# mihikamd/DP-GSAT

Measured on AMD Instinct MI355X. Metric: million edges/s (attn+sample+aggregate fwd+bwd), higher is better.
Workload: dtype f32

## Files before the change

dp_gsat_amd/_lib.py:

```python
from __future__ import annotations

import ctypes
import os
from ctypes import c_char_p, c_double, c_float, c_int, c_int32, c_int64, c_size_t, c_uint64, c_void_p

import torch

_HERE = os.path.dirname(os.path.abspath(__file__))
LIB_PATH = os.path.join(_HERE, "libgsat_hip.so")

P, I64, I32, F32, F64, SZ, INT, U64 = c_void_p, c_int64, c_int32, c_float, c_double, c_size_t, c_int, c_uint64

SIGNATURES = {
    "gsat_abi_version": (INT, []),
    "gsat_seed_next": (INT, [P, P, P]),
    "gsat_last_error": (c_char_p, []),
    "gsat_csr_workspace_bytes": (SZ, [I64, I64]),
    "gsat_rev_workspace_bytes": (SZ, [I64]),
    "gsat_build_csr": (INT, [P, P, I64, I64, P, P, P, P, P, SZ, P]),
    "gsat_reverse_edge_perm": (INT, [P, I64, I64, P, P, P, SZ, P]),
    "gsat_reverse_edge_perm_csr": (INT, [P, P, P, P, P, P, P, P, I64, I64, P, P, P]),
    "gsat_segment_ptr": (INT, [P, I64, I64, P, P, P]),
    "gsat_gather_i64": (INT, [P, I64, P, I64, P, P]),
    "gsat_row_chunks_workspace_bytes": (SZ, [I64]),
    "gsat_row_chunks": (INT, [P, I64, P, P, SZ, P]),
    "gsat_long_row_partial_floats": (SZ, [I64, I64]),
    "gsat_aggr_sum_fwd": (INT, [P, P, P, P, P, P, P, I64, I64, I64, F32, P, P, P, P]),
    "gsat_aggr_sum_bwd": (INT, [P, P, P, P, P, P, P, I64, I64, I64, F32, P, P, P, P, P, P]),
    "gsat_pna_fwd": (INT, [P, P, P, P, P, P, I64, I64, P, INT, P, INT, F32, F32, P, P]),
    "gsat_pna_bwd": (INT, [P, P, P, P, P, P, P, I64, I64, P, INT, P, INT, F32, F32, P, P, P, P, P]),
    "gsat_pna_long_row_floats": (SZ, [I64, I64, INT]),
    "gsat_pna_fwd_long": (INT, [P, P, P, P, P, P, I64, I64, I64, P, INT, P, INT, F32, F32, P, P, P, P]),
    "gsat_pna_bwd_long": (INT, [P, P, P, P, P, P, P, I64, I64, I64, P, INT, P, INT, F32, F32, P, P, P, P, P, P, P]),
    "gsat_pna_tile_plan": (INT, [I64, I64, P, P, P]),
    "gsat_pna_build_tiles": (INT, [P, P, P, P, P, I64, INT, INT, INT, P, P, P, P]),
    "gsat_pna_bwd_tiled": (INT, [P, P, P, P, P, P, P, I64, INT, INT, INT, P, P, I64, I64, I64, P, INT, P, INT, P, P, P, P, P, P, P]),
    "gsat_pna_fwd_compact": (INT, [P, P, P, P, P, I64, I64, P, INT, P, P, P]),
    "gsat_pna_post_fwd": (INT, [P, P, P, I64, I64, INT, P, I64, P, I64, P, P]),
    "gsat_pna_post_dw_workspace_floats": (SZ, [I64, I64, INT, I64]),
    "gsat_pna_post_dw": (INT, [P, P, P, I64, I64, INT, P, I64, P, P, SZ, P]),
    "gsat_pna_fwd_node_att": (INT, [P, P, P, P, I64, I64, P, INT, P, INT, F32, F32, P, P]),
    "gsat_pna_bwd_tiled_node_att": (INT, [P, P, P, P, P, P, I64, INT, INT, INT, P, P, I64, I64, I64, P, INT, P, INT, P, P, P, P, P, P, P, INT, P]),
    "gsat_csr_pair_workspace_bytes": (SZ, [I64, I64]),
    "gsat_build_csr_pair": (INT, [P, I64, I64] + [P] * 12 + [P, SZ, P]),
    "gsat_segment_ptr32": (INT, [P, I64, I64, P, P, P, P]),
    "gsat_bn_workspace_floats": (SZ, [I64, I64]),
    "gsat_bn_fwd": (INT, [P, P, P, P, P, I64, I64, INT, F32, F32, INT, P, P, P, P, P]),
    "gsat_bn_bwd": (INT, [P, P, P, P, P, P, I64, I64, INT, INT, P, P, P, P, P]),
    "gsat_bn_act_fwd": (INT, [P, P, P, P, P, I64, I64, INT, F32, F32, INT, P, F32, U64, P, P, P, P, P, P]),
    "gsat_bn_act_bwd": (INT, [P, P, P, P, P, P, I64, I64, INT, INT, F32, U64, P, P, P, P, P, P, P]),
    "gsat_bn_act_fwd_valid": (INT, [P, P, P, P, P, I64, I64, INT, F32, F32, INT, P, F32, U64, P, P, P, P, P, P, P]),
    "gsat_bn_act_bwd_valid": (INT, [P, P, P, P, P, P, I64, I64, INT, INT, F32, U64, P, P, P, P, P, P, P, P]),
    "gsat_bn_local_sum": (INT, [P, P, I64, I64, P, P, P]),
    "gsat_bn_apply_fwd": (INT, [P, P, P, P, P, I64, I64, INT, P, F32, U64, P, P, P]),
    "gsat_bn_local_bwd_sums": (INT, [P, P, P, P, P, P, I64, I64, INT, F32, U64, P, P, P, P, P]),
    "gsat_bn_apply_bwd": (INT, [P, P, P, P, P, P, P, P, I64, P, I64, I64, INT, F32, U64, P, P, P, P]),
    "gsat_relu_dropout_fwd": (INT, [P, I64, I64, F32, U64, P, P, P]),
    "gsat_relu_dropout_bwd": (INT, [P, P, I64, I64, F32, P, P]),
    "gsat_colsum_workspace_floats": (SZ, [I64]),
    "gsat_colsum": (INT, [P, I64, I64, P, P, P]),
    "gsat_embsum_fwd": (INT, [P, P, INT, P, I64, I64, P, P]),
    "gsat_onehot_rows": (INT, [P, P, INT, I64, I64, P, P]),
    "gsat_gemm_workspace_floats": (SZ, [INT, I64, I64, I64]),
    "gsat_gemm_plan": (INT, [INT, INT, INT, I64, I64, I64, INT, INT, I64, P]),
    "gsat_gemm_f32": (INT, [INT, INT, I64, I64, I64, P, I64, P, I64, P, I64, P, INT, P, SZ, P]),
    "gsat_gemm_bf16x3": (INT, [INT, INT, I64, I64, I64, P, I64, P, I64, P, I64, P, INT, P, SZ, P]),
    "gsat_attn_fwd_workspace_bytes": (SZ, [P]),
    "gsat_attn_fwd_kind": (I32, [P]),
    "gsat_attn_bwd_workspace_bytes": (SZ, [P]),
    "gsat_attn_fwd": (INT, [P, P]),
    "gsat_attn_bwd": (INT, [P, P, P]),
    "gsat_instance_norm_fwd": (INT, [P, P, P, P, I64, I64, I64, P, P, P]),
    "gsat_instance_norm_bwd": (INT, [P, P, P, P, P, P, I64, I64, I64, P, P, P]),
    "gsat_philox_keep_mask": (INT, [U64, I32, I64, I64, F32, P, P]),
    "gsat_philox_noise": (INT, [U64, I64, P, P]),
    "gsat_sample_fwd": (INT, [P, P, INT, F32, F32, I64, P, P]),
    "gsat_sample_bwd": (INT, [P, P, F32, I64, P, P]),
    "gsat_lift_fwd": (INT, [P, P, P, I64, P, P]),
    "gsat_lift_bwd": (INT, [P, P, P, P, P, P, P, P, I64, P, P]),
    "gsat_symmetrise": (INT, [P, P, P, I64, P, P]),
    "gsat_info_loss_fwd": (INT, [P, P, F32, I64, P, P, P]),
    "gsat_info_loss_bwd": (INT, [P, P, F32, P, I64, P, P]),
    "gsat_info_loss_valid_fwd": (INT, [P, P, F32, P, I64, P, P, P, P]),
    "gsat_info_loss_valid_bwd": (INT, [P, P, F32, P, P, I64, P, P, P]),
    "gsat_f1_sparsity_fwd": (INT, [P, P, I64, P, P, P, P, P]),
    "gsat_f1_sparsity_bwd": (INT, [P, P, P, P, I64, P, P, P]),
    "gsat_f1_sparsity_block_entries": (I64, []),
    "gsat_f1_sparsity_max_blocks": (I64, []),
    "gsat_collate_padded": (INT, [P, I64, P, P, P, I64, P, P, I64, I64, P, P, P, P, P, P]),
    "gsat_collate": (INT, [P, I64, P, P, P, I64, P, P, I64, I64, P, P, P, P, P]),
    "gsat_line_graph_pair_counts": (INT, [P, I64, P, P]),
    "gsat_line_graph": (INT, [P, P, P, I64, I64, P, P]),
    "gsat_narrow_i64": (INT, [P, I64, P, P]),
    "gsat_und_edges_workspace_bytes": (SZ, [I64]),
    "gsat_und_edges": (INT, [P, I64, I64, P, P, P, P, P, P, P, P, SZ, P]),
    "gsat_und_line_graph_counts": (INT, [P, P, P, P, I64, P, P]),
    "gsat_und_line_graph": (INT, [P, P, P, P, P, I64, I64, P, P]),
    "gsat_segment_pool_fwd": (INT, [P, P, I64, I64, INT, P, P]),
    "gsat_segment_pool_bwd": (INT, [P, P, I64, I64, INT, P, P]),
    "gsat_rank_edges_lds_cap": (I64, []),
    "gsat_rank_edges_workspace_bytes": (SZ, [I64]),
    "gsat_rank_edges": (INT, [P, P, P, P, I64, I64, I64, I64, INT, P, P, P, P, P, SZ, P]),
    "gsat_auroc_workspace_bytes": (SZ, [I64]),
    "gsat_auroc": (INT, [P, P, I64, P, P, SZ, P]),
    "gsat_delta_kl_workspace_bytes": (SZ, [I64]),
    "gsat_delta_kl": (INT, [P, P, I64, F64, P, P, SZ, P]),
    "gsat_auroc_tasks_workspace_bytes": (SZ, [I64, I64]),
    "gsat_auroc_tasks": (INT, [P, P, I64, I64, P, P, SZ, P]),
    "gsat_att_histogram": (INT, [P, P, I64, I64, F64, F64, P, P, P]),
    "gsat_subgraph_block_items": (I64, []),
    "gsat_subgraph_workspace_bytes": (SZ, [I64, I64]),
    "gsat_subgraph_index": (INT, [P, I64, I64, P, P, I64, P, INT, INT, INT, I64, I64, INT, P, P, P, P, P, P, P, P, SZ, P]),
    "gsat_gather_rows": (INT, [P, P, I64, I64, P, P]),
    "gsat_eval_log_append": (INT, [P] * 8 + [I64] * 4 + [P] * 8 + [I64] * 3 + [P]),
    "gsat_delta_kl_segments_chunk": (I64, []),
    "gsat_delta_kl_segments_workspace_bytes": (SZ, [I64, I64]),
    "gsat_delta_kl_segments": (INT, [P, P, P, I64, I64, I64, F64, P, P, SZ, P]),
}



class AttnArgs(ctypes.Structure):
    _fields_ = [("M", I64), ("N", I64), ("G", I64), ("H", I32), ("C1", I32), ("C2", I32), ("edge_mode", I32),
                ("training", I32), ("p_drop", F32), ("seed", U64),
                ("src", P), ("dst", P), ("seg_ptr", P), ("seg_order", P), ("row_seg", P),
                ("W1", P), ("b1", P), ("W2", P), ("b2", P), ("W3", P), ("b3", P),
                ("emb", P), ("mask1", P), ("mask2", P), ("u", P),
                ("P", P), ("Q", P), ("a1", P), ("h2", P), ("stats", P), ("logits", P), ("att", P),
                ("fwd_workspace", P), ("fwd_workspace_bytes", SZ), ("seed_dev", P), ("noise_philox", I32), ("fused", I32),
                ("node_ptr", P)]


class AttnGrads(ctypes.Structure):
    _fields_ = [("dlogits", P), ("datt", P), ("rowptr_src", P), ("eid_by_src", P), ("rowptr_dst", P), ("eid_by_dst", P),
                ("chunk_ptr_src", P), ("chunk_ptr_dst", P),
                ("demb", P), ("dW1", P), ("db1", P), ("dW2", P), ("db2", P), ("dW3", P), ("db3", P),
                ("workspace", P), ("workspace_bytes", SZ)]


_lib = None


class GsatHipError(RuntimeError):
    pass


def load():
    global _lib
    if _lib is not None:
        return _lib
    if not os.path.exists(LIB_PATH):
        raise GsatHipError(
            f"{LIB_PATH} not found: the HIP extension is required (no CPU fallback). "
            "Build it with `python -c 'import __graft_entry__ as g; g.build()'` or `make -C dp_gsat_amd/csrc`.")
    lib = ctypes.CDLL(LIB_PATH)
    for name, (res, args) in SIGNATURES.items():
        fn = getattr(lib, name)
        fn.restype = res
        fn.argtypes = args
    _lib = lib
    return lib


def ptr(t):
    if t is None:
        return None
    if not t.is_cuda:
        raise GsatHipError("dp_gsat_amd operators need ROCm (cuda) tensors: the HIP path has no CPU fallback")
    if not t.is_contiguous():
        raise GsatHipError("dp_gsat_amd operators need contiguous tensors")
    return t.data_ptr()


_raw_stream = getattr(torch._C, "_cuda_getCurrentRawStream", None)


def stream():
    if _raw_stream is not None:
        return _raw_stream(torch.cuda.current_device())
    return torch.cuda.current_stream().cuda_stream


def call(name, *args):
    lib = _lib if _lib is not None else load()
    rc = getattr(lib, name)(*args)
    if rc != 0:
        msg = lib.gsat_last_error()
        raise GsatHipError(f"{name} failed (code {rc}): {msg.decode() if msg else ''}")
    return rc
```

dp_gsat_amd/csrc/attn.hip:

```cpp
#include "common.h"
#include "attn_fused.h"
#include <cstdlib>

namespace gsat {

constexpr float IN_EPS = 1e-5f;
constexpr int SB = 256;
#ifndef GSAT_SB_LANES
#define GSAT_SB_LANES 16
#endif
constexpr int SB_LANES = GSAT_SB_LANES;
constexpr int SB_SLOTS = SB / SB_LANES;
constexpr int SB_RC = 2;

struct GemmWs { float* ptr; size_t floats; };
static int gemm_rm(hipStream_t stream, bool ta, bool tb, int64_t M, int64_t N, int64_t K, const float* A, int64_t lda, const float* B,
                   int64_t ldb, float beta, float* C, int64_t ldc, GemmWs ws = {nullptr, 0}, bool split_ok = false, SlabJob* defer = nullptr) {
    const char* env = getenv("GSAT_ATTN_BWD_SPLIT");
    const bool bwd_split = !(env && atoi(env) == 0);
    return gemm_f32(stream, ta, tb, M, N, K, A, lda, B, ldb, C, ldc, nullptr, beta != 0.f, ws.ptr, ws.floats, split_ok && bwd_split, defer);
}

template <bool EDGE>
struct PreAct {
    const float* P; const float* Q; const float* bias; const int32_t* src; const int32_t* dst; int C;
    __device__ __forceinline__ float4 load(int row, int c) const {
        float4 b = bias ? ld4(bias + c) : f4zero();
        float4 v;
        if (EDGE) {
            float4 p = ld4(P + (size_t)src[row] * C + c);
            float4 q = ld4(Q + (size_t)dst[row] * C + c);
            v = make_float4(p.x + q.x, p.y + q.y, p.z + q.z, p.w + q.w);
        } else {
            v = ld4(P + (size_t)row * C + c);
        }
        return make_float4(v.x + b.x, v.y + b.y, v.z + b.z, v.w + b.w);
    }
};

__device__ __forceinline__ float4 keep4(const float* mask, SeedRef sref, int layer, int row, int c, int C, float p, bool training) {
    if (!training || p <= 0.f) return make_float4(1.f, 1.f, 1.f, 1.f);
    if (mask) return ld4(mask + (size_t)row * C + c);
    return philox_keep4(sref.get(), layer, row, c, p);
}

__device__ __forceinline__ float4 slot_reduce(float4 v, float4 (*sm)[SB_LANES], int slot, int lane) {
    __syncthreads();
    sm[slot][lane] = v;
    __syncthreads();
    float4 r = f4zero();
    if (slot == 0) {
#pragma unroll
        for (int s = 0; s < SB_SLOTS; ++s) {
            float4 t = sm[s][lane];
            r.x += t.x; r.y += t.y; r.z += t.z; r.w += t.w;
        }
    }
    return r;
}

__device__ __forceinline__ void seg_slice(const int32_t* __restrict__ seg_ptr, int g, int* beg, int* end, float* inv_n) {
    const int b = seg_ptr[g], e = seg_ptr[g + 1];
    *inv_n = 1.f / (float)max(e - b, 1);
    const int Z = gridDim.z, z = blockIdx.z;
    if (Z > 1) {
        const int per = (e - b + Z - 1) / Z;
        *beg = min(e, b + z * per);
        *end = min(e, *beg + per);
    } else {
        *beg = b; *end = e;
    }
}

template <bool EDGE>
__global__ __launch_bounds__(SB) void k_seg_partial(PreAct<EDGE> pre, const int32_t* __restrict__ seg_ptr, const int32_t* __restrict__ order,
                                                    const float* __restrict__ mean , float* __restrict__ part) {
    __shared__ float4 sm[SB_SLOTS][SB_LANES];
    const int g = blockIdx.x;
    const int lane = threadIdx.x % SB_LANES, slot = threadIdx.x / SB_LANES;
    const int c = (blockIdx.y * SB_LANES + lane) * 4;
    const int C = pre.C;
    const bool on = c < C;
    int beg, end; float inv_n;
    seg_slice(seg_ptr, g, &beg, &end, &inv_n);
    float4 acc = f4zero();
    if (on) {
        const float4 mu = mean ? ld4(mean + (size_t)g * C + c) : f4zero();
        for (int r = beg + slot; r < end; r += SB_SLOTS) {
            float4 h = pre.load(order ? order[r] : r, c);
            if (mean) {
                float dx = h.x - mu.x, dy = h.y - mu.y, dz = h.z - mu.z, dw = h.w - mu.w;
                acc.x = fmaf(dx, dx, acc.x); acc.y = fmaf(dy, dy, acc.y); acc.z = fmaf(dz, dz, acc.z); acc.w = fmaf(dw, dw, acc.w);
            } else {
                acc.x += h.x; acc.y += h.y; acc.z += h.z; acc.w += h.w;
            }
        }
    }
    float4 tot = slot_reduce(acc, sm, slot, lane);
    if (slot == 0 && on) st4(part + ((size_t)g * gridDim.z + blockIdx.z) * C + c, tot);
}

__global__ void k_zcombine(const float* __restrict__ part, const int32_t* __restrict__ seg_ptr, int G, int Z, int C, int mode,
                           float* __restrict__ out) {
    const int64_t i = (int64_t)blockIdx.x * blockDim.x + threadIdx.x;
    if (i >= (int64_t)G * C) return;
    const int g = (int)(i / C), c = (int)(i % C);
    float acc = 0.f;
    for (int z = 0; z < Z; ++z) acc += part[((size_t)g * Z + z) * C + c];
    const float inv_n = 1.f / (float)max(seg_ptr[g + 1] - seg_ptr[g], 1);
    out[i] = mode == 0 ? acc : mode == 1 ? acc * inv_n : 1.f / sqrtf(acc * inv_n + IN_EPS);
}

template <bool EDGE, bool APPLY>
__global__ __launch_bounds__(SB) void k_seg_stats(PreAct<EDGE> pre, const int32_t* __restrict__ seg_ptr,
                                                  const int32_t* __restrict__ order, float* __restrict__ mean_out,
                                                  float* __restrict__ rstd_out, const float* __restrict__ mask = nullptr,
                                                  SeedRef seed = SeedRef{0, nullptr}, int layer = 0, float p = 0.f, int training = 0,
                                                  float* __restrict__ act_out = nullptr) {
    __shared__ float4 sm[SB_SLOTS][SB_LANES];
    __shared__ float4 bc[SB_LANES];
    const int g = blockIdx.x;
    const int lane = threadIdx.x % SB_LANES, slot = threadIdx.x / SB_LANES;
    const int c = (blockIdx.y * SB_LANES + lane) * 4;
    const int C = pre.C;
    const bool on = c < C;
    const int beg = seg_ptr[g], end = seg_ptr[g + 1];
    const float inv_n = 1.f / (float)max(end - beg, 1);
    float4 hc[SB_RC];
    int mc[SB_RC];
#pragma unroll
    for (int i = 0; i < SB_RC; ++i) {
        const int r = beg + slot + i * SB_SLOTS;
        mc[i] = (r < end) ? (order ? order[r] : r) : -1;
    }
#pragma unroll
    for (int i = 0; i < SB_RC; ++i) hc[i] = (on && mc[i] >= 0) ? pre.load(mc[i], c) : f4zero();
    const int rest = beg + slot + SB_RC * SB_SLOTS;
    float4 acc = f4zero();
    if (on) {
#pragma unroll
        for (int i = 0; i < SB_RC; ++i)
            if (mc[i] >= 0) { acc.x += hc[i].x; acc.y += hc[i].y; acc.z += hc[i].z; acc.w += hc[i].w; }
        for (int r = rest; r < end; r += SB_SLOTS) {
            float4 h = pre.load(order ? order[r] : r, c);
            acc.x += h.x; acc.y += h.y; acc.z += h.z; acc.w += h.w;
        }
    }
    float4 tot = slot_reduce(acc, sm, slot, lane);
    if (slot == 0) bc[lane] = make_float4(tot.x * inv_n, tot.y * inv_n, tot.z * inv_n, tot.w * inv_n);
    __syncthreads();
    const float4 mu = bc[lane];
    acc = f4zero();
    if (on) {
#pragma unroll
        for (int i = 0; i < SB_RC; ++i)
            if (mc[i] >= 0) {
                float dx = hc[i].x - mu.x, dy = hc[i].y - mu.y, dz = hc[i].z - mu.z, dw = hc[i].w - mu.w;
                acc.x = fmaf(dx, dx, acc.x); acc.y = fmaf(dy, dy, acc.y); acc.z = fmaf(dz, dz, acc.z); acc.w = fmaf(dw, dw, acc.w);
            }
        for (int r = rest; r < end; r += SB_SLOTS) {
            float4 h = pre.load(order ? order[r] : r, c);
            float dx = h.x - mu.x, dy = h.y - mu.y, dz = h.z - mu.z, dw = h.w - mu.w;
            acc.x = fmaf(dx, dx, acc.x); acc.y = fmaf(dy, dy, acc.y); acc.z = fmaf(dz, dz, acc.z); acc.w = fmaf(dw, dw, acc.w);
        }
    }
    tot = slot_reduce(acc, sm, slot, lane);
    float4 rs = make_float4(1.f / sqrtf(tot.x * inv_n + IN_EPS), 1.f / sqrtf(tot.y * inv_n + IN_EPS),
                            1.f / sqrtf(tot.z * inv_n + IN_EPS), 1.f / sqrtf(tot.w * inv_n + IN_EPS));
    if (slot == 0 && on) {
        st4(mean_out + (size_t)g * C + c, mu);
        st4(rstd_out + (size_t)g * C + c, rs);
    }
    if (APPLY) {
        if (slot == 0) bc[lane] = rs;
        __syncthreads();
        rs = bc[lane];
        const float sc = (training && p > 0.f) ? 1.f / (1.f - p) : 1.f;
        if (on) {
#pragma unroll
            for (int i = 0; i < SB_RC; ++i)
                if (mc[i] >= 0) {
                    const int m = mc[i];
                    const float4 h = hc[i];
                    const float4 k = keep4(mask, seed, layer, m, c, C, p, training != 0);
                    st4(act_out + (size_t)m * C + c,
                        make_float4(fmaxf((h.x - mu.x) * rs.x, 0.f) * k.x * sc, fmaxf((h.y - mu.y) * rs.y, 0.f) * k.y * sc,
                                    fmaxf((h.z - mu.z) * rs.z, 0.f) * k.z * sc, fmaxf((h.w - mu.w) * rs.w, 0.f) * k.w * sc));
                }
            for (int r = rest; r < end; r += SB_SLOTS) {
                const int m = order ? order[r] : r;
                const float4 h = pre.load(m, c);
                const float4 k = keep4(mask, seed, layer, m, c, C, p, training != 0);
                st4(act_out + (size_t)m * C + c,
                    make_float4(fmaxf((h.x - mu.x) * rs.x, 0.f) * k.x * sc, fmaxf((h.y - mu.y) * rs.y, 0.f) * k.y * sc,
                                fmaxf((h.z - mu.z) * rs.z, 0.f) * k.z * sc, fmaxf((h.w - mu.w) * rs.w, 0.f) * k.w * sc));
            }
        }
    }
}

template <bool EDGE, bool RELU>
__global__ void k_norm_apply(PreAct<EDGE> pre, const int32_t* __restrict__ row_seg, const float* __restrict__ mean,
                             const float* __restrict__ rstd, const float* __restrict__ mask, SeedRef seed, int layer,
                             float p, int training, int64_t M, float* __restrict__ out) {
    const int C = pre.C, C4 = C >> 2;
    const float sc = (training && p > 0.f) ? 1.f / (1.f - p) : 1.f;
    for (int64_t i = (int64_t)blockIdx.x * blockDim.x + threadIdx.x; i < M * C4; i += (int64_t)gridDim.x * blockDim.x) {
        const int m = (int)(i / C4), c = (int)(i % C4) * 4;
        const int g = row_seg[m];
        float4 h = pre.load(m, c);
        float4 mu = ld4(mean + (size_t)g * C + c), rs = ld4(rstd + (size_t)g * C + c);
        float4 y = make_float4((h.x - mu.x) * rs.x, (h.y - mu.y) * rs.y, (h.z - mu.z) * rs.z, (h.w - mu.w) * rs.w);
        if (RELU) {
            float4 k = keep4(mask, seed, layer, m, c, C, p, training != 0);
            y = make_float4(fmaxf(y.x, 0.f) * k.x * sc, fmaxf(y.y, 0.f) * k.y * sc, fmaxf(y.z, 0.f) * k.z * sc, fmaxf(y.w, 0.f) * k.w * sc);
        }
        st4(out + (size_t)m * C + c, y);
    }
}

template <int LPR>
__global__ __launch_bounds__(256) void k_head_fwd(const float* __restrict__ h2, const float* __restrict__ b2,
                                                  const int32_t* __restrict__ row_seg, const float* __restrict__ mean,
                                                  const float* __restrict__ rstd, const float* __restrict__ mask, SeedRef seed,
                                                  float p, int training, const float* __restrict__ w3, const float* __restrict__ b3,
                                                  const float* __restrict__ u, int noise_philox, int64_t M, int C, float* __restrict__ logits,
                                                  float* __restrict__ att) {
    const int lane = threadIdx.x % LPR;
    const float sc = (training && p > 0.f) ? 1.f / (1.f - p) : 1.f;
    PreAct<false> pre{h2, nullptr, b2, nullptr, nullptr, C};
    for (int64_t m = ((int64_t)blockIdx.x * blockDim.x + threadIdx.x) / LPR; m < M; m += (int64_t)gridDim.x * blockDim.x / LPR) {
        const int g = row_seg[m];
        float acc = 0.f;
        for (int c = lane * 4; c < C; c += LPR * 4) {
            float4 h = pre.load((int)m, c);
            float4 mu = ld4(mean + (size_t)g * C + c), rs = ld4(rstd + (size_t)g * C + c);
            float4 k = keep4(mask, seed, 2, (int)m, c, C, p, training != 0);
            float4 w = ld4(w3 + c);
            acc = fmaf(fmaxf((h.x - mu.x) * rs.x, 0.f) * k.x * sc, w.x, acc);
            acc = fmaf(fmaxf((h.y - mu.y) * rs.y, 0.f) * k.y * sc, w.y, acc);
            acc = fmaf(fmaxf((h.z - mu.z) * rs.z, 0.f) * k.z * sc, w.z, acc);
            acc = fmaf(fmaxf((h.w - mu.w) * rs.w, 0.f) * k.w * sc, w.w, acc);
        }
        acc = group_sum<LPR>(acc);
        if (lane == 0) {
            const float z = acc + b3[0];
            logits[m] = z;
            if (att) {
                float t = z;
                if (training && (u || noise_philox)) {
                    const float uu = u ? u[m] : philox_noise_u(seed.get(), (int)m);
                    t = z + (logf(uu) - logf(1.0f - uu));
                }
                att[m] = 1.f / (1.f + expf(-t));
            }
        }
    }
}

__global__ __launch_bounds__(256) void k_dz(const float* __restrict__ dlogits, const float* __restrict__ datt, const float* __restrict__ att,
                                            int64_t M, float* __restrict__ dz, float* __restrict__ zero_a, int na, float* __restrict__ zero_b, int nb,
                                            float* __restrict__ block_sum = nullptr ) {
    int64_t m = (int64_t)blockIdx.x * blockDim.x + threadIdx.x;
    const int64_t total = (int64_t)gridDim.x * blockDim.x;
    for (int64_t i = m; i < na; i += total) zero_a[i] = 0.f;
    for (int64_t i = m; i < nb; i += total) zero_b[i] = 0.f;
    float v = 0.f;
    if (m < M) {
        v = dlogits ? dlogits[m] : 0.f;
        if (datt) { float a = att[m]; v = fmaf(datt[m], a * (1.f - a), v); }
        dz[m] = v;
    }
    if (block_sum) {
        __shared__ float ws[4];
        const float w = group_sum<64>(v);
        if ((threadIdx.x & 63) == 0) ws[threadIdx.x >> 6] = w;
        __syncthreads();
        if (threadIdx.x == 0) block_sum[blockIdx.x] = ((ws[0] + ws[1]) + ws[2]) + ws[3];
    }
}

struct DzSrc {
    const float* dz;
    const float *dlogits, *datt, *att;
    __device__ __forceinline__ float get(int m) const {
        if (dz) return dz[m];
        float v = dlogits ? dlogits[m] : 0.f;
        if (datt) { const float a = att[m]; v = fmaf(datt[m], a * (1.f - a), v); }
        return v;
    }
};

template <bool APPLY>
__global__ __launch_bounds__(SB) void k_head_bwd_stats(const float* __restrict__ h2, const float* __restrict__ b2,
                                                       const int32_t* __restrict__ seg_ptr, const int32_t* __restrict__ order,
                                                       const float* __restrict__ mean, const float* __restrict__ rstd,
                                                       const float* __restrict__ mask, SeedRef seed, float p, int training,
                                                       const float* __restrict__ w3, const DzSrc dzs, int C,
                                                       float* __restrict__ S1, float* __restrict__ S2, float* __restrict__ dw3p,
                                                       float* __restrict__ dh2 = nullptr) {
    __shared__ float4 sm[SB_SLOTS][SB_LANES];
    __shared__ float4 bc1[SB_LANES], bc2[SB_LANES];
    const int g = blockIdx.x;
    const int lane = threadIdx.x % SB_LANES, slot = threadIdx.x / SB_LANES;
    const int c = (blockIdx.y * SB_LANES + lane) * 4;
    const bool on = c < C;
    int beg, end; float inv_n;
    seg_slice(seg_ptr, g, &beg, &end, &inv_n);
    if (gridDim.z > 1) inv_n = 1.f;
    const size_t orow = gridDim.z > 1 ? (size_t)g * gridDim.z + blockIdx.z : (size_t)g;
    const float sc = (training && p > 0.f) ? 1.f / (1.f - p) : 1.f;
    PreAct<false> pre{h2, nullptr, b2, nullptr, nullptr, C};
    float4 a1 = f4zero(), a2 = f4zero(), a3 = f4zero();
    if (on) {
        const float4 mu = ld4(mean + (size_t)g * C + c), rs = ld4(rstd + (size_t)g * C + c), w = ld4(w3 + c);
        for (int r = beg + slot; r < end; r += SB_SLOTS) {
            const int m = order ? order[r] : r;
            const float d = dzs.get(m);
            float4 h = pre.load(m, c);
            float4 k = keep4(mask, seed, 2, m, c, C, p, training != 0);
            float4 y = make_float4((h.x - mu.x) * rs.x, (h.y - mu.y) * rs.y, (h.z - mu.z) * rs.z, (h.w - mu.w) * rs.w);
            float4 dy = make_float4(y.x > 0.f ? d * w.x * k.x * sc : 0.f, y.y > 0.f ? d * w.y * k.y * sc : 0.f,
                                    y.z > 0.f ? d * w.z * k.z * sc : 0.f, y.w > 0.f ? d * w.w * k.w * sc : 0.f);
            a1.x += dy.x; a1.y += dy.y; a1.z += dy.z; a1.w += dy.w;
            a2.x = fmaf(dy.x, y.x, a2.x); a2.y = fmaf(dy.y, y.y, a2.y); a2.z = fmaf(dy.z, y.z, a2.z); a2.w = fmaf(dy.w, y.w, a2.w);
            a3.x = fmaf(d, fmaxf(y.x, 0.f) * k.x * sc, a3.x); a3.y = fmaf(d, fmaxf(y.y, 0.f) * k.y * sc, a3.y);
            a3.z = fmaf(d, fmaxf(y.z, 0.f) * k.z * sc, a3.z); a3.w = fmaf(d, fmaxf(y.w, 0.f) * k.w * sc, a3.w);
        }
    }
    float4 t1 = slot_reduce(a1, sm, slot, lane);
    float4 t2 = slot_reduce(a2, sm, slot, lane);
    float4 t3 = slot_reduce(a3, sm, slot, lane);
    t1 = make_float4(t1.x * inv_n, t1.y * inv_n, t1.z * inv_n, t1.w * inv_n);
    t2 = make_float4(t2.x * inv_n, t2.y * inv_n, t2.z * inv_n, t2.w * inv_n);
    if (slot == 0 && on) {
        st4(S1 + orow * C + c, t1);
        st4(S2 + orow * C + c, t2);
        st4(dw3p + orow * C + c, t3);
    }
    if (APPLY) {
        if (slot == 0) { bc1[lane] = t1; bc2[lane] = t2; }
        __syncthreads();
        if (!on) return;
        const float4 s1 = bc1[lane], s2 = bc2[lane];
        const float4 mu = ld4(mean + (size_t)g * C + c), rs = ld4(rstd + (size_t)g * C + c), w = ld4(w3 + c);
        for (int r = beg + slot; r < end; r += SB_SLOTS) {
            const int m = order ? order[r] : r;
            const float d = dzs.get(m);
            const float4 h = pre.load(m, c);
            const float4 k = keep4(mask, seed, 2, m, c, C, p, training != 0);
            const float4 y = make_float4((h.x - mu.x) * rs.x, (h.y - mu.y) * rs.y, (h.z - mu.z) * rs.z, (h.w - mu.w) * rs.w);
            const float4 dy = make_float4(y.x > 0.f ? d * w.x * k.x * sc : 0.f, y.y > 0.f ? d * w.y * k.y * sc : 0.f,
                                          y.z > 0.f ? d * w.z * k.z * sc : 0.f, y.w > 0.f ? d * w.w * k.w * sc : 0.f);
            st4(dh2 + (size_t)m * C + c, make_float4(rs.x * (dy.x - s1.x - y.x * s2.x), rs.y * (dy.y - s1.y - y.y * s2.y),
                                                      rs.z * (dy.z - s1.z - y.z * s2.z), rs.w * (dy.w - s1.w - y.w * s2.w)));
        }
    }
}

__global__ void k_dh2(const float* __restrict__ h2, const float* __restrict__ b2, const int32_t* __restrict__ row_seg,
                      const float* __restrict__ mean, const float* __restrict__ rstd, const float* __restrict__ mask, SeedRef seed,
                      float p, int training, const float* __restrict__ w3, const float* __restrict__ dz,
                      const float* __restrict__ S1, const float* __restrict__ S2, int64_t M, int C, float* __restrict__ dh2) {
    const int C4 = C >> 2;
    const float sc = (training && p > 0.f) ? 1.f / (1.f - p) : 1.f;
    PreAct<false> pre{h2, nullptr, b2, nullptr, nullptr, C};
    for (int64_t i = (int64_t)blockIdx.x * blockDim.x + threadIdx.x; i < M * C4; i += (int64_t)gridDim.x * blockDim.x) {
        const int m = (int)(i / C4), c = (int)(i % C4) * 4;
        const int g = row_seg[m];
        const float d = dz[m];
        float4 h = pre.load(m, c);
        float4 mu = ld4(mean + (size_t)g * C + c), rs = ld4(rstd + (size_t)g * C + c), w = ld4(w3 + c);
        float4 k = keep4(mask, seed, 2, m, c, C, p, training != 0);
        float4 s1 = ld4(S1 + (size_t)g * C + c), s2 = ld4(S2 + (size_t)g * C + c);
        float4 y = make_float4((h.x - mu.x) * rs.x, (h.y - mu.y) * rs.y, (h.z - mu.z) * rs.z, (h.w - mu.w) * rs.w);
        float4 dy = make_float4(y.x > 0.f ? d * w.x * k.x * sc : 0.f, y.y > 0.f ? d * w.y * k.y * sc : 0.f,
                                y.z > 0.f ? d * w.z * k.z * sc : 0.f, y.w > 0.f ? d * w.w * k.w * sc : 0.f);
        st4(dh2 + (size_t)m * C + c, make_float4(rs.x * (dy.x - s1.x - y.x * s2.x), rs.y * (dy.y - s1.y - y.y * s2.y),
                                                  rs.z * (dy.z - s1.z - y.z * s2.z), rs.w * (dy.w - s1.w - y.w * s2.w)));
    }
}

template <bool APPLY, bool EDGE>
__global__ __launch_bounds__(SB) void k_l1_bwd_stats(float* __restrict__ da1, const float* __restrict__ a1,
                                                     const int32_t* __restrict__ seg_ptr, const int32_t* __restrict__ order,
                                                     float sc, int C, float* __restrict__ S1, float* __restrict__ S2,
                                                     PreAct<EDGE> pre = PreAct<EDGE>{}, const float* __restrict__ mean = nullptr,
                                                     const float* __restrict__ rstd = nullptr) {
    __shared__ float4 sm[SB_SLOTS][SB_LANES];
    __shared__ float4 bc1[SB_LANES], bc2[SB_LANES];
    const int g = blockIdx.x;
    const int lane = threadIdx.x % SB_LANES, slot = threadIdx.x / SB_LANES;
    const int c = (blockIdx.y * SB_LANES + lane) * 4;
    const bool on = c < C;
    int beg, end; float inv_n;
    seg_slice(seg_ptr, g, &beg, &end, &inv_n);
    if (gridDim.z > 1) inv_n = 1.f;
    const size_t orow = gridDim.z > 1 ? (size_t)g * gridDim.z + blockIdx.z : (size_t)g;
    const float inv_sc = 1.f / sc;
    float4 s1 = f4zero(), s2 = f4zero();
    float4 dcache[SB_RC], acache[SB_RC], hcache[SB_RC];
    int mc[SB_RC];
#pragma unroll
    for (int i = 0; i < SB_RC; ++i) {
        const int r = beg + slot + i * SB_SLOTS;
        mc[i] = (r < end && on) ? (order ? order[r] : r) : -1;
    }
#pragma unroll
    for (int i = 0; i < SB_RC; ++i) {
        dcache[i] = mc[i] >= 0 ? ld4(da1 + (size_t)mc[i] * C + c) : f4zero();
        acache[i] = mc[i] >= 0 ? ld4(a1 + (size_t)mc[i] * C + c) : f4zero();
        if (APPLY) hcache[i] = mc[i] >= 0 ? pre.load(mc[i], c) : f4zero();
    }
    const int rest = beg + slot + SB_RC * SB_SLOTS;
#define GSAT_L1_DY(D4, A4)                                                                                                         \
    const float4 dy = make_float4((A4).x > 0.f ? (D4).x * sc : 0.f, (A4).y > 0.f ? (D4).y * sc : 0.f,                                \
                                  (A4).z > 0.f ? (D4).z * sc : 0.f, (A4).w > 0.f ? (D4).w * sc : 0.f);
#define GSAT_L1_ACC(D4, A4)                                                                                                        \
    {                                                                                                                              \
        GSAT_L1_DY(D4, A4)                                                                                                         \
        s1.x += dy.x; s1.y += dy.y; s1.z += dy.z; s1.w += dy.w;                                                                    \
        s2.x = fmaf(dy.x, (A4).x * inv_sc, s2.x); s2.y = fmaf(dy.y, (A4).y * inv_sc, s2.y);                                          \
        s2.z = fmaf(dy.z, (A4).z * inv_sc, s2.z); s2.w = fmaf(dy.w, (A4).w * inv_sc, s2.w);                                          \
    }
    if (on) {
#pragma unroll
        for (int i = 0; i < SB_RC; ++i)
            if (mc[i] >= 0) GSAT_L1_ACC(dcache[i], acache[i])
        for (int r = rest; r < end; r += SB_SLOTS) {
            const int m = order ? order[r] : r;
            const float4 d = ld4(da1 + (size_t)m * C + c), a = ld4(a1 + (size_t)m * C + c);
            GSAT_L1_ACC(d, a)
        }
    }
#undef GSAT_L1_ACC
    float4 t1 = slot_reduce(s1, sm, slot, lane);
    float4 t2 = slot_reduce(s2, sm, slot, lane);
    t1 = make_float4(t1.x * inv_n, t1.y * inv_n, t1.z * inv_n, t1.w * inv_n);
    t2 = make_float4(t2.x * inv_n, t2.y * inv_n, t2.z * inv_n, t2.w * inv_n);
    if (slot == 0 && on) {
        st4(S1 + orow * C + c, t1);
        st4(S2 + orow * C + c, t2);
    }
    if (APPLY) {
        if (slot == 0) { bc1[lane] = t1; bc2[lane] = t2; }
        __syncthreads();
        if (!on) return;
        const float4 q1 = bc1[lane], q2 = bc2[lane];
        const float4 mu = ld4(mean + (size_t)g * C + c), rs = ld4(rstd + (size_t)g * C + c);
#define GSAT_L1_OUT(M_, H4, D4, A4)                                                                                                \
        {                                                                                                                          \
            const float4 y = make_float4(((H4).x - mu.x) * rs.x, ((H4).y - mu.y) * rs.y, ((H4).z - mu.z) * rs.z, ((H4).w - mu.w) * rs.w); \
            GSAT_L1_DY(D4, A4)                                                                                                     \
            st4(da1 + (size_t)(M_) * C + c, make_float4(rs.x * (dy.x - q1.x - y.x * q2.x), rs.y * (dy.y - q1.y - y.y * q2.y),        \
                                                         rs.z * (dy.z - q1.z - y.z * q2.z), rs.w * (dy.w - q1.w - y.w * q2.w)));     \
        }
#pragma unroll
        for (int i = 0; i < SB_RC; ++i)
            if (mc[i] >= 0) GSAT_L1_OUT(mc[i], hcache[i], dcache[i], acache[i])
        for (int r = rest; r < end; r += SB_SLOTS) {
            const int m = order ? order[r] : r;
            const float4 h = pre.load(m, c);
            const float4 d = ld4(da1 + (size_t)m * C + c), a = ld4(a1 + (size_t)m * C + c);
            GSAT_L1_OUT(m, h, d, a)
        }
#undef GSAT_L1_OUT
    }
#undef GSAT_L1_DY
}

template <bool EDGE>
__global__ void k_dh1(PreAct<EDGE> pre, const int32_t* __restrict__ row_seg, const float* __restrict__ mean,
                      const float* __restrict__ rstd, const float* __restrict__ a1, float sc, const float* __restrict__ S1,
                      const float* __restrict__ S2, int64_t M, float* __restrict__ da1_inout) {
    const int C = pre.C, C4 = C >> 2;
    for (int64_t i = (int64_t)blockIdx.x * blockDim.x + threadIdx.x; i < M * C4; i += (int64_t)gridDim.x * blockDim.x) {
        const int m = (int)(i / C4), c = (int)(i % C4) * 4;
        const int g = row_seg[m];
        float4 h = pre.load(m, c);
        float4 mu = ld4(mean + (size_t)g * C + c), rs = ld4(rstd + (size_t)g * C + c);
        float4 y = make_float4((h.x - mu.x) * rs.x, (h.y - mu.y) * rs.y, (h.z - mu.z) * rs.z, (h.w - mu.w) * rs.w);
        float4 d = ld4(da1_inout + (size_t)m * C + c), a = ld4(a1 + (size_t)m * C + c);
        float4 dy = make_float4(a.x > 0.f ? d.x * sc : 0.f, a.y > 0.f ? d.y * sc : 0.f, a.z > 0.f ? d.z * sc : 0.f, a.w > 0.f ? d.w * sc : 0.f);
        float4 s1 = ld4(S1 + (size_t)g * C + c), s2 = ld4(S2 + (size_t)g * C + c);
        st4(da1_inout + (size_t)m * C + c, make_float4(rs.x * (dy.x - s1.x - y.x * s2.x), rs.y * (dy.y - s1.y - y.y * s2.y),
                                                        rs.z * (dy.z - s1.z - y.z * s2.z), rs.w * (dy.w - s1.w - y.w * s2.w)));
    }
}

__global__ __launch_bounds__(SB) void k_in_bwd_stats(const float* __restrict__ y, const float* __restrict__ dy,
                                                     const int32_t* __restrict__ seg_ptr, const int32_t* __restrict__ order, int C,
                                                     float* __restrict__ S1, float* __restrict__ S2) {
    __shared__ float4 sm[SB_SLOTS][SB_LANES];
    const int g = blockIdx.x;
    const int lane = threadIdx.x % SB_LANES, slot = threadIdx.x / SB_LANES;
    const int c = (blockIdx.y * SB_LANES + lane) * 4;
    const bool on = c < C;
    int beg, end; float inv_n;
    seg_slice(seg_ptr, g, &beg, &end, &inv_n);
    if (gridDim.z > 1) inv_n = 1.f;
    const size_t orow = gridDim.z > 1 ? (size_t)g * gridDim.z + blockIdx.z : (size_t)g;
    float4 s1 = f4zero(), s2 = f4zero();
    if (on)
        for (int r = beg + slot; r < end; r += SB_SLOTS) {
            const int m = order ? order[r] : r;
            float4 d = ld4(dy + (size_t)m * C + c), v = ld4(y + (size_t)m * C + c);
            s1.x += d.x; s1.y += d.y; s1.z += d.z; s1.w += d.w;
            s2.x = fmaf(d.x, v.x, s2.x); s2.y = fmaf(d.y, v.y, s2.y); s2.z = fmaf(d.z, v.z, s2.z); s2.w = fmaf(d.w, v.w, s2.w);
        }
    float4 t1 = slot_reduce(s1, sm, slot, lane);
    float4 t2 = slot_reduce(s2, sm, slot, lane);
    if (slot == 0 && on) {
        st4(S1 + orow * C + c, make_float4(t1.x * inv_n, t1.y * inv_n, t1.z * inv_n, t1.w * inv_n));
        st4(S2 + orow * C + c, make_float4(t2.x * inv_n, t2.y * inv_n, t2.z * inv_n, t2.w * inv_n));
    }
}

__global__ void k_in_bwd_apply(const float* __restrict__ y, const float* __restrict__ dy, const int32_t* __restrict__ row_seg,
                               const float* __restrict__ rstd, const float* __restrict__ S1, const float* __restrict__ S2,
                               int64_t M, int C, float* __restrict__ dx) {
    const int C4 = C >> 2;
    for (int64_t i = (int64_t)blockIdx.x * blockDim.x + threadIdx.x; i < M * C4; i += (int64_t)gridDim.x * blockDim.x) {
        const int m = (int)(i / C4), c = (int)(i % C4) * 4;
        const int g = row_seg[m];
        float4 v = ld4(y + (size_t)m * C + c), d = ld4(dy + (size_t)m * C + c);
        float4 rs = ld4(rstd + (size_t)g * C + c), s1 = ld4(S1 + (size_t)g * C + c), s2 = ld4(S2 + (size_t)g * C + c);
        st4(dx + (size_t)m * C + c, make_float4(rs.x * (d.x - s1.x - v.x * s2.x), rs.y * (d.y - s1.y - v.y * s2.y),
                                                 rs.z * (d.z - s1.z - v.z * s2.z), rs.w * (d.w - s1.w - v.w * s2.w)));
    }
}

__global__ __launch_bounds__(SB) void k_colsum(const float* __restrict__ x, int64_t R, int C, int64_t rows_per_block,
                                               float* __restrict__ out) {
    __shared__ float4 sm[SB_SLOTS][SB_LANES];
    const int lane = threadIdx.x % SB_LANES, slot = threadIdx.x / SB_LANES;
    const int c = (blockIdx.x * SB_LANES + lane) * 4;
    const int64_t beg = (int64_t)blockIdx.y * rows_per_block, end = min(R, beg + rows_per_block);
    float4 acc = f4zero();
    if (c + 3 < C) {
        for (int64_t r = beg + slot; r < end; r += SB_SLOTS) {
            float4 v = ld4(x + (size_t)r * C + c);
            acc.x += v.x; acc.y += v.y; acc.z += v.z; acc.w += v.w;
        }
    } else if (c < C) {
        for (int64_t r = beg + slot; r < end; r += SB_SLOTS) {
            const float* p = x + (size_t)r * C + c;
            acc.x += p[0];
            if (c + 1 < C) acc.y += p[1];
            if (c + 2 < C) acc.z += p[2];
        }
    }
    float4 t = slot_reduce(acc, sm, slot, lane);
    if (slot == 0 && c < C) {
        float* o = out + (size_t)blockIdx.y * C + c;
        o[0] = t.x;
        if (c + 1 < C) o[1] = t.y;
        if (c + 2 < C) o[2] = t.z;
        if (c + 3 < C) o[3] = t.w;
    }
}

constexpr int FIN_T = 1024, FIN_SLOTS = FIN_T / SB_LANES;
__global__ __launch_bounds__(FIN_T) void k_head_bwd_finish(const float* __restrict__ dw3p, const float* __restrict__ dz_part, int64_t G, int ndz, int C,
                                                           float* __restrict__ dW3, float* __restrict__ db3) {
    __shared__ float4 sm[FIN_SLOTS][SB_LANES];
    const int lane = threadIdx.x % SB_LANES, slot = threadIdx.x / SB_LANES;
    const int ctiles = (C + 4 * SB_LANES - 1) / (4 * SB_LANES);
    float4 acc = f4zero();
    if ((int)blockIdx.x < ctiles) {
        const int c = (blockIdx.x * SB_LANES + lane) * 4;
        if (c < C) {
            int64_t g = slot;
            for (; g + 7 * FIN_SLOTS < G; g += 8 * FIN_SLOTS) {
                float4 v[8];
#pragma unroll
                for (int j = 0; j < 8; ++j) v[j] = ld4(dw3p + (size_t)(g + j * FIN_SLOTS) * C + c);
#pragma unroll
                for (int j = 0; j < 8; ++j) { acc.x += v[j].x; acc.y += v[j].y; acc.z += v[j].z; acc.w += v[j].w; }
            }
            for (; g < G; g += FIN_SLOTS) { const float4 v = ld4(dw3p + (size_t)g * C + c); acc.x += v.x; acc.y += v.y; acc.z += v.z; acc.w += v.w; }
        }
    } else {
        for (int i = threadIdx.x; i < ndz; i += FIN_T) acc.x += dz_part[i];
    }
    sm[slot][lane] = acc;
    __syncthreads();
    if (slot == 0) {
        float4 r = f4zero();
        for (int s_ = 0; s_ < FIN_SLOTS; ++s_) { const float4 t = sm[s_][lane]; r.x += t.x; r.y += t.y; r.z += t.z; r.w += t.w; }
        if ((int)blockIdx.x < ctiles) {
            const int c = (blockIdx.x * SB_LANES + lane) * 4;
            if (c < C) st4(dW3 + c, r);
        } else {
            sm[0][lane] = r;
        }
    }
    if ((int)blockIdx.x >= ctiles) {
        __syncthreads();
        if (threadIdx.x == 0) {
            float r = 0.f;
            for (int l = 0; l < SB_LANES; ++l) r += sm[0][l].x;
            db3[0] = r;
        }
    }
}

__global__ void k_philox_noise(uint64_t seed, int64_t M, float* __restrict__ u) {
    const int64_t m = (int64_t)blockIdx.x * blockDim.x + threadIdx.x;
    if (m < M) u[m] = philox_noise_u(seed, (int)m);
}

__global__ void k_philox_mask(uint64_t seed, int layer, int64_t M, int C, float p, float* __restrict__ keep) {
    const int C4 = C >> 2;
    for (int64_t i = (int64_t)blockIdx.x * blockDim.x + threadIdx.x; i < M * C4; i += (int64_t)gridDim.x * blockDim.x) {
        const int m = (int)(i / C4), c = (int)(i % C4) * 4;
        st4(keep + (size_t)m * C + c, keep4(nullptr, SeedRef{seed, nullptr}, layer, m, c, C, p, true));
    }
}

static inline int ew_blocks(int64_t work_items) {
    int64_t nb = ceil_div(work_items, 256);
    if (nb > 256 * 32) nb = 256 * 32;
    return (int)std::max<int64_t>(nb, 1);
}

static int colsum(hipStream_t stream, const float* x, int64_t R, int C, float* out, float* scratch ) {
    if (C <= 0) return GSAT_OK;
    const int ctiles = (int)ceil_div(C, 4 * SB_LANES);
    if (R <= 0) { GSAT_CHECK_HIP(gsat::zero_async(out, sizeof(float) * C, stream)); return GSAT_OK; }
    int64_t RB = std::min<int64_t>(256, ceil_div(R, 64));
    if (RB <= 1) {
        k_colsum<<<dim3(ctiles, 1), SB, 0, stream>>>(x, R, C, R, out);
    } else {
        int64_t rpb = ceil_div(R, RB);
        RB = ceil_div(R, rpb);
        k_colsum<<<dim3(ctiles, (unsigned)RB), SB, 0, stream>>>(x, R, C, rpb, scratch);
        k_colsum<<<dim3(ctiles, 1), SB, 0, stream>>>(scratch, RB, C, RB, out);
    }
    GSAT_LAUNCH_CHECK();
    return GSAT_OK;
}

static inline int seg_slices(int64_t rows, int64_t G) {
    const int64_t avg = rows / std::max<int64_t>(G, 1);
    return (int)std::max<int64_t>(1, std::min<int64_t>(64, ceil_div(avg, 4096)));
}

template <bool EDGE>
static int launch_seg_stats(hipStream_t stream, PreAct<EDGE> pre, const int32_t* seg_ptr, const int32_t* order, int64_t G, int Z,
                            float* mean, float* rstd, float* part) {
    if (G <= 0) return GSAT_OK;
    const int C = pre.C;
    const dim3 grid((unsigned)G, (unsigned)ceil_div(C, 4 * SB_LANES), (unsigned)Z);
    if (Z == 1) {
        k_seg_stats<EDGE, false><<<grid, SB, 0, stream>>>(pre, seg_ptr, order, mean, rstd);
    } else {
        GSAT_REQUIRE(part, GSAT_ERR_WORKSPACE, "segmented statistics need a workspace for sliced segments");
        const unsigned cb = (unsigned)ceil_div(G * C, 256);
        k_seg_partial<EDGE><<<grid, SB, 0, stream>>>(pre, seg_ptr, order, nullptr, part);
        k_zcombine<<<cb, 256, 0, stream>>>(part, seg_ptr, (int)G, Z, C, 1, mean);
        k_seg_partial<EDGE><<<grid, SB, 0, stream>>>(pre, seg_ptr, order, mean, part);
        k_zcombine<<<cb, 256, 0, stream>>>(part, seg_ptr, (int)G, Z, C, 2, rstd);
    }
    GSAT_LAUNCH_CHECK();
    return GSAT_OK;
}

static size_t attn_gemm_ws_w2(const gsat_attn_args* a) { return align_up(gemm_workspace_floats(a->C2, a->C1, a->M, true), 64); }
static size_t attn_gemm_ws_w1(const gsat_attn_args* a) { return align_up(gemm_workspace_floats(a->C1, a->H, a->N, true), 64); }
static size_t attn_gemm_ws_floats(const gsat_attn_args* a) { return attn_gemm_ws_w2(a) + (a->edge_mode ? 2 : 1) * attn_gemm_ws_w1(a); }

static int check_args(const gsat_attn_args* a, const char* who) {
    GSAT_REQUIRE(a, GSAT_ERR_ARG, "%s: null args", who);
    GSAT_REQUIRE(a->M >= 0 && a->N >= 0 && a->G >= 0 && a->M < (1ll << 31) && a->N < (1ll << 31), GSAT_ERR_ARG, "%s: bad extents", who);
    GSAT_REQUIRE(a->H > 0 && a->C1 > 0 && a->C2 > 0 && a->H % 4 == 0 && a->C1 % 4 == 0 && a->C2 % 4 == 0, GSAT_ERR_UNSUPPORTED,
                 "%s: H, C1, C2 must be positive multiples of 4 (got %d, %d, %d)", who, a->H, a->C1, a->C2);
    GSAT_REQUIRE(a->p_drop >= 0.f && a->p_drop < 1.f, GSAT_ERR_ARG, "%s: dropout p must be in [0,1)", who);
    if (a->M == 0) return GSAT_OK;
    GSAT_REQUIRE(a->emb && a->W1 && a->b1 && a->W2 && a->b2 && a->W3 && a->b3 && a->seg_ptr && a->row_seg, GSAT_ERR_ARG, "%s: null input", who);
    GSAT_REQUIRE(a->P && a->h2 && a->stats && a->logits, GSAT_ERR_ARG, "%s: null output/saved buffer", who);
    if (a->edge_mode) GSAT_REQUIRE(a->src && a->dst && a->Q, GSAT_ERR_ARG, "%s: edge mode needs src, dst, Q", who);
    else GSAT_REQUIRE(a->M == a->N, GSAT_ERR_ARG, "%s: node mode needs M == N", who);
    return GSAT_OK;
}

}

using namespace gsat;

extern "C" {

size_t gsat_colsum_workspace_floats(int64_t C) { return (size_t)256 * (size_t)(C > 0 ? C : 0); }

int gsat_colsum(const float* x, int64_t R, int64_t C, float* out, float* workspace, void* stream) {
    GSAT_REQUIRE(R >= 0 && C >= 0 && C < (1ll << 31), GSAT_ERR_ARG, "gsat_colsum: bad extents");
    if (C == 0) return GSAT_OK;
    GSAT_REQUIRE(out && (x || R == 0) && workspace, GSAT_ERR_ARG, "gsat_colsum: null pointer");
    return colsum((hipStream_t)stream, x, R, (int)C, out, workspace);
}


int gsat_attn_fwd(const gsat_attn_args* a, void* stream_) {
    hipStream_t stream = (hipStream_t)stream_;
    int rc = check_args(a, "gsat_attn_fwd");
    if (rc) return rc;
    if (a->M == 0) return GSAT_OK;
    {
        FusedGeom fg;
        if (attn_fused_eligible(a, &fg)) return attn_fused_fwd(stream, a, fg);
    }
    GSAT_REQUIRE(a->a1, GSAT_ERR_ARG, "gsat_attn_fwd: the staged pipeline needs the a1 buffer");
    const int64_t M = a->M, N = a->N, G = a->G;
    const int H = a->H, C1 = a->C1, C2 = a->C2;
    float* mean1 = a->stats;
    float* rstd1 = mean1 + (size_t)G * C1;
    float* mean2 = rstd1 + (size_t)G * C1;
    float* rstd2 = mean2 + (size_t)G * C2;
    if (a->edge_mode) {
        if ((rc = gemm_rm(stream, false, true, N, C1, H, a->emb, H, a->W1, 2 * H, 0.f, a->P, C1))) return rc;
        if ((rc = gemm_rm(stream, false, true, N, C1, H, a->emb, H, a->W1 + H, 2 * H, 0.f, a->Q, C1))) return rc;
    } else {
        if ((rc = gemm_rm(stream, false, true, N, C1, H, a->emb, H, a->W1, H, 0.f, a->P, C1))) return rc;
    }
    const int Z = seg_slices(M, G);
    float* part = nullptr;
    if (Z > 1) {
        const size_t need = (size_t)G * Z * std::max(C1, C2) * sizeof(float);
        GSAT_REQUIRE(a->fwd_workspace && a->fwd_workspace_bytes >= need, GSAT_ERR_WORKSPACE, "gsat_attn_fwd: workspace %zu < %zu", a->fwd_workspace_bytes, need);
        part = static_cast<float*>(a->fwd_workspace);
    }
    const dim3 sgrid((unsigned)G, (unsigned)ceil_div(C1, 4 * SB_LANES), 1);
    const SeedRef sref{a->seed, a->seed_dev};
    if (a->edge_mode) {
        PreAct<true> pre{a->P, a->Q, a->b1, a->src, a->dst, C1};
        if (Z == 1 && G > 0) {
            k_seg_stats<true, true><<<sgrid, SB, 0, stream>>>(pre, a->seg_ptr, a->seg_order, mean1, rstd1, a->mask1, sref, 1, a->p_drop, a->training, a->a1);
        } else {
            if ((rc = launch_seg_stats<true>(stream, pre, a->seg_ptr, a->seg_order, G, Z, mean1, rstd1, part))) return rc;
            k_norm_apply<true, true><<<ew_blocks(M * (C1 / 4)), 256, 0, stream>>>(pre, a->row_seg, mean1, rstd1, a->mask1, sref, 1, a->p_drop, a->training, M, a->a1);
        }
    } else {
        PreAct<false> pre{a->P, nullptr, a->b1, nullptr, nullptr, C1};
        if (Z == 1 && G > 0) {
            k_seg_stats<false, true><<<sgrid, SB, 0, stream>>>(pre, a->seg_ptr, a->seg_order, mean1, rstd1, a->mask1, sref, 1, a->p_drop, a->training, a->a1);
        } else {
            if ((rc = launch_seg_stats<false>(stream, pre, a->seg_ptr, a->seg_order, G, Z, mean1, rstd1, part))) return rc;
            k_norm_apply<false, true><<<ew_blocks(M * (C1 / 4)), 256, 0, stream>>>(pre, a->row_seg, mean1, rstd1, a->mask1, sref, 1, a->p_drop, a->training, M, a->a1);
        }
    }
    GSAT_LAUNCH_CHECK();
    if ((rc = gemm_rm(stream, false, true, M, C2, C1, a->a1, C1, a->W2, C1, 0.f, a->h2, C2))) return rc;
    {
        PreAct<false> pre{a->h2, nullptr, a->b2, nullptr, nullptr, C2};
        if ((rc = launch_seg_stats<false>(stream, pre, a->seg_ptr, a->seg_order, G, Z, mean2, rstd2, part))) return rc;
    }
    const int q = C2 / 4;
    const int lpr = q <= 4 ? 4 : q <= 8 ? 8 : q <= 16 ? 16 : q <= 32 ? 32 : 64;
    const int nb = (int)std::min<int64_t>(ceil_div(M, 256 / lpr), 256 * 32);
#define HEAD(L) k_head_fwd<L><<<nb, 256, 0, stream>>>(a->h2, a->b2, a->row_seg, mean2, rstd2, a->mask2, SeedRef{a->seed, a->seed_dev}, a->p_drop, a->training, a->W3, a->b3, a->u, a->noise_philox, M, C2, a->logits, a->att)
    switch (lpr) { case 4: HEAD(4); break; case 8: HEAD(8); break; case 16: HEAD(16); break; case 32: HEAD(32); break; default: HEAD(64); break; }
#undef HEAD
    GSAT_LAUNCH_CHECK();
    return GSAT_OK;
}

size_t gsat_attn_fwd_workspace_bytes(const gsat_attn_args* a) {
    if (!a) return 0;
    FusedGeom fg;
    if (attn_fused_eligible(a, &fg)) return fused_ws_bytes(fg, a->G);
    const int Z = seg_slices(a->M, a->G);
    return Z > 1 ? (size_t)a->G * Z * std::max(a->C1, a->C2) * sizeof(float) : 0;
}

int gsat_attn_fwd_kind(const gsat_attn_args* a) {
    if (!a) return 0;
    FusedGeom fg;
    if (!attn_fused_eligible(a, &fg)) return 0;
    return fg.x6 ? 2 : 1;
}

size_t gsat_attn_bwd_workspace_bytes(const gsat_attn_args* a) {
    if (!a) return 0;
    const size_t M = (size_t)a->M, N = (size_t)a->N, G = (size_t)a->G, C1 = a->C1, C2 = a->C2;
    const size_t cmax = C1 > C2 ? C1 : C2;
    size_t b = 0;
    b += align_up((M > G ? M : G) * 4, 256);
    b += align_up(M * C2 * 4, 256);
    b += align_up(M * C1 * 4, 256);
    b += 2 * align_up(G * C1 * 4, 256);
    b += 3 * align_up(G * C2 * 4, 256);
    b += align_up(256 * cmax * 4, 256);
    { const size_t Z = seg_slices(a->M, a->G); if (Z > 1) b += 3 * align_up(G * Z * cmax * 4, 256); }
    if (a->edge_mode) b += 2 * align_up(N * C1 * 4, 256) + align_up(gsat_long_row_partial_floats(a->M, a->C1) * 4, 256);
    b += align_up(attn_gemm_ws_floats(a) * 4, 256);
    if (attn_fused_bwd_eligible(a)) b += align_up(attn_fused_bwd_ws_bytes(a), 256);
    b += align_up(std::max(dual_gemm_ws_bytes(1, a->C2, a->C1, a->C1), dual_gemm_ws_bytes(2, a->C1, a->H, a->H)), 256);
    return b + 1024;
}

int gsat_attn_bwd(const gsat_attn_args* a, const gsat_attn_grads* gr, void* stream_) {
    hipStream_t stream = (hipStream_t)stream_;
    int rc = check_args(a, "gsat_attn_bwd");
    if (rc) return rc;
    GSAT_REQUIRE(gr && gr->demb && gr->dW1 && gr->db1 && gr->dW2 && gr->db2 && gr->dW3 && gr->db3, GSAT_ERR_ARG, "gsat_attn_bwd: null gradient output");
    const int64_t M = a->M, N = a->N, G = a->G;
    const int H = a->H, C1 = a->C1, C2 = a->C2;
    const int C0 = a->edge_mode ? 2 * H : H;
    if (M == 0) {
        GSAT_CHECK_HIP(gsat::zero_async(gr->demb, sizeof(float) * N * H, stream));
        GSAT_CHECK_HIP(gsat::zero_async(gr->dW1, sizeof(float) * C1 * C0, stream));
        GSAT_CHECK_HIP(gsat::zero_async(gr->db1, sizeof(float) * C1, stream));
        GSAT_CHECK_HIP(gsat::zero_async(gr->dW2, sizeof(float) * C2 * C1, stream));
        GSAT_CHECK_HIP(gsat::zero_async(gr->db2, sizeof(float) * C2, stream));
        GSAT_CHECK_HIP(gsat::zero_async(gr->dW3, sizeof(float) * C2, stream));
        GSAT_CHECK_HIP(gsat::zero_async(gr->db3, sizeof(float), stream));
        return GSAT_OK;
    }
    GSAT_REQUIRE(gr->dlogits || gr->datt, GSAT_ERR_ARG, "gsat_attn_bwd: need dlogits and/or datt");
    GSAT_REQUIRE(!gr->datt || a->att, GSAT_ERR_ARG, "gsat_attn_bwd: datt given but att was not saved");
    if (a->edge_mode) GSAT_REQUIRE(gr->rowptr_src && gr->eid_by_src && gr->rowptr_dst && gr->eid_by_dst, GSAT_ERR_ARG, "gsat_attn_bwd: edge mode needs both CSRs");
    Arena ar(gr->workspace, gr->workspace_bytes);
    float* dz = ar.take<float>(std::max<int64_t>(M, G));
    float* dh2 = ar.take<float>((size_t)M * C2);
    float* da1 = ar.take<float>((size_t)M * C1);
    float* S1p = ar.take<float>((size_t)G * C1);
    float* S2p = ar.take<float>((size_t)G * C1);
    float* S1 = ar.take<float>((size_t)G * C2);
    float* S2 = ar.take<float>((size_t)G * C2);
    float* dw3p = ar.take<float>((size_t)G * C2);
    float* scratch = ar.take<float>((size_t)256 * std::max(C1, C2));
    const int Z = seg_slices(M, G);
    float *zp1 = nullptr, *zp2 = nullptr, *zp3 = nullptr;
    if (Z > 1) {
        const size_t n = (size_t)G * Z * std::max(C1, C2);
        zp1 = ar.take<float>(n); zp2 = ar.take<float>(n); zp3 = ar.take<float>(n);
    }
    float *dP = nullptr, *dQ = nullptr;
    float* lpart = nullptr;
    if (a->edge_mode) {
        dP = ar.take<float>((size_t)N * C1);
        dQ = ar.take<float>((size_t)N * C1);
        lpart = ar.take<float>(gsat_long_row_partial_floats(M, C1));
    }
    GemmWs gws{nullptr, attn_gemm_ws_w2(a)}, gws1{nullptr, attn_gemm_ws_w1(a)}, gws1b{nullptr, a->edge_mode ? attn_gemm_ws_w1(a) : 0};
    gws.ptr = ar.take<float>(gws.floats);
    gws1.ptr = ar.take<float>(gws1.floats);
    gws1b.ptr = ar.take<float>(gws1b.floats);
    SlabJob jobs[3] = {};
    const size_t dws_bytes = std::max(dual_gemm_ws_bytes(1, C2, C1, C1), dual_gemm_ws_bytes(2, C1, H, H));
    char* dws = ar.take<char>(dws_bytes);
    const bool fused_bwd = attn_fused_bwd_eligible(a) && seg_slices(M, G) == 1;
    const size_t fws_bytes = fused_bwd ? attn_fused_bwd_ws_bytes(a) : 0;
    char* fws = fused_bwd ? ar.take<char>(fws_bytes) : nullptr;
    GSAT_REQUIRE(ar.ok(), GSAT_ERR_WORKSPACE, "gsat_attn_bwd: workspace %zu < %zu", gr->workspace_bytes, ar.off);
    float* mean1 = a->stats;
    float* rstd1 = mean1 + (size_t)G * C1;
    float* mean2 = rstd1 + (size_t)G * C1;
    float* rstd2 = mean2 + (size_t)G * C2;
    const float sc = (a->training && a->p_drop > 0.f) ? 1.f / (1.f - a->p_drop) : 1.f;

    const dim3 g2((unsigned)G, (unsigned)ceil_div(C2, 4 * SB_LANES), (unsigned)Z), g1((unsigned)G, (unsigned)ceil_div(C1, 4 * SB_LANES), (unsigned)Z);
    if (fused_bwd) {
        if ((rc = attn_fused_bwd(stream, a, gr, da1, fws, fws_bytes))) return rc;
    } else {
    const char* env_m = getenv("GSAT_ATTN_BWD_MERGED");
    const bool merged = Z == 1 && G > 0 && !(env_m && atoi(env_m) == 0);
    const unsigned dzb = (unsigned)ceil_div(M, 256);
    float* dzpart = scratch;
    const bool part_ok = (size_t)dzb <= (size_t)256 * std::max(C1, C2);
    k_dz<<<dzb, 256, 0, stream>>>(gr->dlogits, gr->datt, a->att, M, dz, gr->db1, (int)C1, gr->db2, (int)C2, (merged && part_ok) ? dzpart : nullptr);
    GSAT_LAUNCH_CHECK();
    if (!(merged && part_ok) && (rc = colsum(stream, dz, M, 1, gr->db3, scratch))) return rc;
    if (Z == 1)
        k_head_bwd_stats<true><<<g2, SB, 0, stream>>>(a->h2, a->b2, a->seg_ptr, a->seg_order, mean2, rstd2, a->mask2, SeedRef{a->seed, a->seed_dev}, a->p_drop,
                                                      a->training, a->W3, DzSrc{dz, nullptr, nullptr, nullptr}, C2, S1, S2, dw3p, dh2);
    else
        k_head_bwd_stats<false><<<g2, SB, 0, stream>>>(a->h2, a->b2, a->seg_ptr, a->seg_order, mean2, rstd2, a->mask2, SeedRef{a->seed, a->seed_dev}, a->p_drop,
                                                       a->training, a->W3, DzSrc{dz, nullptr, nullptr, nullptr}, C2, zp1, zp2, zp3);
    if (merged && part_ok)
        k_head_bwd_finish<<<(unsigned)ceil_div(C2, 4 * SB_LANES) + 1, FIN_T, 0, stream>>>(dw3p, dzpart, G, (int)dzb, C2, gr->dW3, gr->db3);
    if (Z > 1) {
        const unsigned cb = (unsigned)ceil_div(G * C2, 256);
        k_zcombine<<<cb, 256, 0, stream>>>(zp1, a->seg_ptr, (int)G, Z, C2, 1, S1);
        k_zcombine<<<cb, 256, 0, stream>>>(zp2, a->seg_ptr, (int)G, Z, C2, 1, S2);
        k_zcombine<<<cb, 256, 0, stream>>>(zp3, a->seg_ptr, (int)G, Z, C2, 0, dw3p);
    }
    GSAT_LAUNCH_CHECK();
    if (!(merged && part_ok) && (rc = colsum(stream, dw3p, G, C2, gr->dW3, scratch))) return rc;
    if (Z > 1) {
        k_dh2<<<ew_blocks(M * (C2 / 4)), 256, 0, stream>>>(a->h2, a->b2, a->row_seg, mean2, rstd2, a->mask2, SeedRef{a->seed, a->seed_dev}, a->p_drop, a->training,
                                                           a->W3, dz, S1, S2, M, C2, dh2);
        GSAT_LAUNCH_CHECK();
    }
    if (dual_gemm_ok(1, M, C2, C1, C1)) {
        if ((rc = dual_gemm(stream, 1, M, C2, C1, C1, dh2, C2, a->a1, C1, a->W2, C1, da1, C1, 0, gr->dW2, C1, dws, dws_bytes))) return rc;
    } else {
        if ((rc = gemm_rm(stream, true, false, C2, C1, M, dh2, C2, a->a1, C1, 0.f, gr->dW2, C1, gws, true, &jobs[0]))) return rc;
        if ((rc = gemm_rm(stream, false, false, M, C1, C2, dh2, C2, a->W2, C1, 0.f, da1, C1, GemmWs{nullptr, 0}, true))) return rc;
    }
    if (Z == 1) {
        if (a->edge_mode) {
            PreAct<true> pre1{a->P, a->Q, a->b1, a->src, a->dst, C1};
            k_l1_bwd_stats<true, true><<<g1, SB, 0, stream>>>(da1, a->a1, a->seg_ptr, a->seg_order, sc, C1, S1p, S2p, pre1, mean1, rstd1);
        } else {
            PreAct<false> pre1{a->P, nullptr, a->b1, nullptr, nullptr, C1};
            k_l1_bwd_stats<true, false><<<g1, SB, 0, stream>>>(da1, a->a1, a->seg_ptr, a->seg_order, sc, C1, S1p, S2p, pre1, mean1, rstd1);
        }
    } else {
        k_l1_bwd_stats<false, false><<<g1, SB, 0, stream>>>(da1, a->a1, a->seg_ptr, a->seg_order, sc, C1, zp1, zp2);
    }
    if (Z > 1) {
        const unsigned cb = (unsigned)ceil_div(G * C1, 256);
        k_zcombine<<<cb, 256, 0, stream>>>(zp1, a->seg_ptr, (int)G, Z, C1, 1, S1p);
        k_zcombine<<<cb, 256, 0, stream>>>(zp2, a->seg_ptr, (int)G, Z, C1, 1, S2p);
    }
    GSAT_LAUNCH_CHECK();
    }
    if (a->edge_mode) {
        if (Z > 1) {
            PreAct<true> pre{a->P, a->Q, a->b1, a->src, a->dst, C1};
            k_dh1<true><<<ew_blocks(M * (C1 / 4)), 256, 0, stream>>>(pre, a->row_seg, mean1, rstd1, a->a1, sc, S1p, S2p, M, da1);
            GSAT_LAUNCH_CHECK();
        }
        if ((rc = aggr_sum_fwd_impl(stream, da1, nullptr, nullptr, nullptr, gr->rowptr_src, gr->eid_by_src, nullptr, N, M, C1, 0.f, dP,
                                    gr->chunk_ptr_src, lpart))) return rc;
        if ((rc = aggr_sum_fwd_impl(stream, da1, nullptr, nullptr, nullptr, gr->rowptr_dst, gr->eid_by_dst, nullptr, N, M, C1, 0.f, dQ,
                                    gr->chunk_ptr_dst, lpart))) return rc;
        if (dual_gemm_ok(2, N, C1, H, H)) {
            if ((rc = dual_gemm(stream, 2, N, C1, H, H, dP, C1, a->emb, H, a->W1, 2 * H, gr->demb, H, 0, gr->dW1, 2 * H, dws, dws_bytes))) return rc;
            if ((rc = dual_gemm(stream, 2, N, C1, H, H, dQ, C1, a->emb, H, a->W1 + H, 2 * H, gr->demb, H, 1, gr->dW1 + H, 2 * H, dws, dws_bytes))) return rc;
        } else {
        if ((rc = gemm_rm(stream, false, false, N, H, C1, dP, C1, a->W1, 2 * H, 0.f, gr->demb, H, GemmWs{nullptr, 0}, true))) return rc;
        if ((rc = gemm_rm(stream, false, false, N, H, C1, dQ, C1, a->W1 + H, 2 * H, 1.f, gr->demb, H, GemmWs{nullptr, 0}, true))) return rc;
        if ((rc = gemm_rm(stream, true, false, C1, H, N, dP, C1, a->emb, H, 0.f, gr->dW1, 2 * H, gws1, true, &jobs[1]))) return rc;
        if ((rc = gemm_rm(stream, true, false, C1, H, N, dQ, C1, a->emb, H, 0.f, gr->dW1 + H, 2 * H, gws1b, true, &jobs[2]))) return rc;
        }
    } else {
        if (Z > 1) {
            PreAct<false> pre{a->P, nullptr, a->b1, nullptr, nullptr, C1};
            k_dh1<false><<<ew_blocks(M * (C1 / 4)), 256, 0, stream>>>(pre, a->row_seg, mean1, rstd1, a->a1, sc, S1p, S2p, M, da1);
            GSAT_LAUNCH_CHECK();
        }
        if (dual_gemm_ok(2, N, C1, H, H)) {
            if ((rc = dual_gemm(stream, 2, N, C1, H, H, da1, C1, a->emb, H, a->W1, H, gr->demb, H, 0, gr->dW1, H, dws, dws_bytes))) return rc;
        } else {
        if ((rc = gemm_rm(stream, false, false, N, H, C1, da1, C1, a->W1, H, 0.f, gr->demb, H, GemmWs{nullptr, 0}, true))) return rc;
        if ((rc = gemm_rm(stream, true, false, C1, H, N, da1, C1, a->emb, H, 0.f, gr->dW1, H, gws1, true, &jobs[1]))) return rc;
        }
    }
    return slab_reduce_jobs(stream, jobs, 3);
}

int gsat_instance_norm_fwd(const float* x, const int32_t* seg_ptr, const int32_t* seg_order, const int32_t* row_seg, int64_t M,
                           int64_t G, int64_t C, float* y, float* stats, void* stream_) {
    hipStream_t stream = (hipStream_t)stream_;
    GSAT_REQUIRE(M >= 0 && G >= 0 && C > 0 && C % 4 == 0 && M < (1ll << 31), GSAT_ERR_UNSUPPORTED, "gsat_instance_norm_fwd: C must be a positive multiple of 4");
    if (M == 0 || G == 0) return GSAT_OK;
    GSAT_REQUIRE(x && seg_ptr && row_seg && y && stats, GSAT_ERR_ARG, "gsat_instance_norm_fwd: null pointer");
    float* mean = stats;
    float* rstd = stats + (size_t)G * C;
    PreAct<false> pre{x, nullptr, nullptr, nullptr, nullptr, (int)C};
    k_seg_stats<false, false><<<dim3((unsigned)G, (unsigned)ceil_div(C, 4 * SB_LANES), 1), SB, 0, stream>>>(pre, seg_ptr, seg_order, mean, rstd);
    k_norm_apply<false, false><<<ew_blocks(M * (C / 4)), 256, 0, stream>>>(pre, row_seg, mean, rstd, nullptr, SeedRef{0, nullptr}, 0, 0.f, 0, M, y);
    GSAT_LAUNCH_CHECK();
    return GSAT_OK;
}

int gsat_instance_norm_bwd(const float* y, const float* dy, const float* stats, const int32_t* seg_ptr, const int32_t* seg_order,
                           const int32_t* row_seg, int64_t M, int64_t G, int64_t C, float* dx, float* workspace, void* stream_) {
    hipStream_t stream = (hipStream_t)stream_;
    GSAT_REQUIRE(M >= 0 && G >= 0 && C > 0 && C % 4 == 0 && M < (1ll << 31), GSAT_ERR_UNSUPPORTED, "gsat_instance_norm_bwd: C must be a positive multiple of 4");
    if (M == 0 || G == 0) return GSAT_OK;
    GSAT_REQUIRE(y && dy && stats && seg_ptr && row_seg && dx && workspace, GSAT_ERR_ARG, "gsat_instance_norm_bwd: null pointer");
    float* S1 = workspace;
    float* S2 = workspace + (size_t)G * C;
    k_in_bwd_stats<<<dim3((unsigned)G, (unsigned)ceil_div(C, 4 * SB_LANES), 1), SB, 0, stream>>>(y, dy, seg_ptr, seg_order, (int)C, S1, S2);
    k_in_bwd_apply<<<ew_blocks(M * (C / 4)), 256, 0, stream>>>(y, dy, row_seg, stats + (size_t)G * C, S1, S2, M, (int)C, dx);
    GSAT_LAUNCH_CHECK();
    return GSAT_OK;
}

int gsat_philox_noise(uint64_t seed, int64_t M, float* u, void* stream_) {
    hipStream_t stream = (hipStream_t)stream_;
    GSAT_REQUIRE(M >= 0 && M < (1ll << 31), GSAT_ERR_ARG, "gsat_philox_noise: bad M");
    if (M == 0) return GSAT_OK;
    GSAT_REQUIRE(u, GSAT_ERR_ARG, "gsat_philox_noise: null pointer");
    k_philox_noise<<<(unsigned)ceil_div(M, 256), 256, 0, stream>>>(seed, M, u);
    GSAT_LAUNCH_CHECK();
    return GSAT_OK;
}

int gsat_philox_keep_mask(uint64_t seed, int32_t layer, int64_t M, int64_t C, float p_drop, float* keep, void* stream_) {
    hipStream_t stream = (hipStream_t)stream_;
    GSAT_REQUIRE(M >= 0 && C > 0 && C % 4 == 0 && M < (1ll << 31), GSAT_ERR_UNSUPPORTED, "gsat_philox_keep_mask: C must be a positive multiple of 4");
    if (M == 0) return GSAT_OK;
    GSAT_REQUIRE(keep, GSAT_ERR_ARG, "gsat_philox_keep_mask: null pointer");
    k_philox_mask<<<ew_blocks(M * (C / 4)), 256, 0, stream>>>(seed, layer, M, (int)C, p_drop, keep);
    GSAT_LAUNCH_CHECK();
    return GSAT_OK;
}

}
```

dp_gsat_amd/csrc/attn_fused.h:

```cpp
#pragma once
#include "common.h"

namespace gsat {

constexpr int F_GT = 16;

struct FusedGeom {
    int H, C1, C2, C2p;
    int CH, NCH;
    int S1, S2;
    int NCB2;
    int NRB, RM, RX;
    int LDX, LDU, LDT, LDH, SW;
    int offU, offT, offS, offMeta;
    int lds_bytes;
    int pqg;
    int x6;
};

struct FTile { int row0, nrows, g0, ng, node0, nnodes, flags, pad; };
size_t attn_plan_bytes(int64_t G);
bool attn_plan_ok(int64_t G);
int attn_plan_launch(hipStream_t stream, const int32_t* seg_ptr, const int32_t* node_ptr, int64_t G, int RM, int RX, FTile* tiles, int* counters);

bool fused_geometry(int H, int C1, int C2, bool edge, FusedGeom* out, bool pqg = false);
size_t fused_ws_bytes(const FusedGeom& g, int64_t G);
bool attn_fused_eligible(const gsat_attn_args* a, FusedGeom* g);
int attn_fused_fwd(hipStream_t stream, const gsat_attn_args* a, const FusedGeom& g);

bool attn_fused_bwd_eligible(const gsat_attn_args* a);
size_t attn_fused_bwd_ws_bytes(const gsat_attn_args* a);
int attn_fused_bwd(hipStream_t stream, const gsat_attn_args* a, const gsat_attn_grads* gr, float* dh1, void* ws, size_t ws_bytes);

bool dual_gemm_ok(int mode, int64_t R, int KA, int KY, int NO);
size_t dual_gemm_ws_bytes(int mode, int KA, int KY, int NO);
int dual_gemm(hipStream_t stream, int mode, int64_t R, int KA, int KY, int NO, const float* A, int lda, const float* Y, int ldy, const float* W,
              int ldw, float* OUT, int ldo, int accumulate, float* DW, int lddw, void* ws, size_t ws_bytes);

#ifdef __HIPCC__
__device__ __forceinline__ float4 keep4f(const float* mask, SeedRef sref, int layer, int row, int c, int C, float p, bool training) {
    if (!training || p <= 0.f) return make_float4(1.f, 1.f, 1.f, 1.f);
    if (mask) return ld4(mask + (size_t)row * C + c);
    return philox_keep4(sref.get(), layer, row, c, p);
}
#endif

}
```

dp_gsat_amd/csrc/attn_fused.hip:

```cpp
#include "common.h"
#include "attn_fused.h"
#include <algorithm>
#include <cstdlib>

namespace gsat {

typedef float f32x16 __attribute__((ext_vector_type(16)));

constexpr int FT = 512;
constexpr int F_RMAX = 128;
constexpr float F_EPS = 1e-5f;


static inline int ceil32(int v) { return (v + 31) / 32 * 32; }

bool fused_geometry(int H, int C1, int C2, bool edge, FusedGeom* out, bool pqg) {
    if (H < 8 || H > 256 || H % 8 || C1 < 4 || C1 % 4 || C2 < 4 || C2 % 4 || C2 > 256 || C1 > 2048) return false;
    for (int nrb = 2; nrb >= 1; --nrb) {
        FusedGeom g{};
        g.H = H; g.C1 = C1; g.C2 = C2; g.C2p = ceil32(C2);
        g.CH = edge ? 64 : 128;
        g.NCH = (C1 + g.CH - 1) / g.CH;
        g.S1 = H / 8; g.S2 = g.CH / 8;
        g.NCB2 = g.C2p / 32;
// ... 197 lines not shown
#pragma unroll
        for (int j = 0; j < 4; ++j) {
            if (s + j < S) {
                b[(j + 3) & 3] = bp[64 * min(s + j + 3, S - 1)];
                const float4 x0 = ld4(a0 + 4 * (s + j));
                float4 x1 = f4zero();
                if (NA > 1) x1 = ld4(a1 + 4 * (s + j));
                const float4 w = b[j];
                acc0 = GSAT_MFMA(x0.x, w.x, acc0);
                if (NA > 1) acc1 = GSAT_MFMA(x1.x, w.x, acc1);
                acc0 = GSAT_MFMA(x0.y, w.y, acc0);
                if (NA > 1) acc1 = GSAT_MFMA(x1.y, w.y, acc1);
                acc0 = GSAT_MFMA(x0.z, w.z, acc0);
                if (NA > 1) acc1 = GSAT_MFMA(x1.z, w.z, acc1);
                acc0 = GSAT_MFMA(x0.w, w.w, acc0);
                if (NA > 1) acc1 = GSAT_MFMA(x1.w, w.w, acc1);
            }
        }
    }
}

typedef __attribute__((ext_vector_type(8))) __bf16 fbf16x8;
typedef __attribute__((ext_vector_type(4))) unsigned fu32x4;
#define GSAT_MFMA_B(a, b, c) __builtin_amdgcn_mfma_f32_32x32x16_bf16((a), (b), (c), 0, 0, 0)

__device__ __forceinline__ void split3(const float4 lo4, const float4 hi4, fbf16x8& p0, fbf16x8& p1, fbf16x8& p2) {
    const float x[8] = {lo4.x, lo4.y, lo4.z, lo4.w, hi4.x, hi4.y, hi4.z, hi4.w};
    fu32x4 a, b, c;
#pragma unroll
    for (int e = 0; e < 4; ++e) {
        const unsigned u0 = __builtin_bit_cast(unsigned, x[2 * e]), u1 = __builtin_bit_cast(unsigned, x[2 * e + 1]);
        const float r0 = x[2 * e] - __builtin_bit_cast(float, u0 & 0xFFFF0000u), r1 = x[2 * e + 1] - __builtin_bit_cast(float, u1 & 0xFFFF0000u);
        const unsigned v0 = __builtin_bit_cast(unsigned, r0), v1 = __builtin_bit_cast(unsigned, r1);
        const float s0 = r0 - __builtin_bit_cast(float, v0 & 0xFFFF0000u), s1 = r1 - __builtin_bit_cast(float, v1 & 0xFFFF0000u);
        a[e] = __builtin_amdgcn_perm(u1, u0, 0x07060302u);
        b[e] = __builtin_amdgcn_perm(v1, v0, 0x07060302u);
        c[e] = __builtin_amdgcn_perm(__builtin_bit_cast(unsigned, s1), __builtin_bit_cast(unsigned, s0), 0x07060302u);
    }
    p0 = __builtin_bit_cast(fbf16x8, a); p1 = __builtin_bit_cast(fbf16x8, b); p2 = __builtin_bit_cast(fbf16x8, c);
}

template <int NA>
__device__ __forceinline__ void mma_run_x6(f32x16& acc0, f32x16& acc1, const float* a0, const float* a1, const uint4* __restrict__ bp, const int S) {
    uint4 b[3][3];
#pragma unroll
    for (int p = 0; p < 3; ++p) { b[0][p] = bp[p * 64]; b[1][p] = bp[(3 * min(1, S - 1) + p) * 64]; }
    for (int s = 0; s < S; s += 3) {
#pragma unroll
        for (int j = 0; j < 3; ++j) {
            if (s + j < S) {
                const int sn = min(s + j + 2, S - 1);
#pragma unroll
                for (int p = 0; p < 3; ++p) b[(j + 2) % 3][p] = bp[(3 * sn + p) * 64];
                const fbf16x8 y0 = __builtin_bit_cast(fbf16x8, b[j][0]), y1 = __builtin_bit_cast(fbf16x8, b[j][1]), y2 = __builtin_bit_cast(fbf16x8, b[j][2]);
                fbf16x8 x0, x1, x2;
                split3(ld4(a0 + 16 * (s + j)), ld4(a0 + 16 * (s + j) + 4), x0, x1, x2);
                acc0 = GSAT_MFMA_B(x2, y0, acc0);
                acc0 = GSAT_MFMA_B(x0, y2, acc0);
                acc0 = GSAT_MFMA_B(x1, y1, acc0);
                acc0 = GSAT_MFMA_B(x1, y0, acc0);
                acc0 = GSAT_MFMA_B(x0, y1, acc0);
                acc0 = GSAT_MFMA_B(x0, y0, acc0);
                if (NA > 1) {
                    split3(ld4(a1 + 16 * (s + j)), ld4(a1 + 16 * (s + j) + 4), x0, x1, x2);
                    acc1 = GSAT_MFMA_B(x2, y0, acc1);
                    acc1 = GSAT_MFMA_B(x0, y2, acc1);
                    acc1 = GSAT_MFMA_B(x1, y1, acc1);
                    acc1 = GSAT_MFMA_B(x1, y0, acc1);
                    acc1 = GSAT_MFMA_B(x0, y1, acc1);
                    acc1 = GSAT_MFMA_B(x0, y0, acc1);
                }
            }
        }
    }
}

__device__ __forceinline__ void acc_zero(f32x16& a) {
#pragma unroll
    for (int r = 0; r < 16; ++r) a[r] = 0.f;
}

__device__ __forceinline__ float4 f4add(float4 a, float4 b) { return make_float4(a.x + b.x, a.y + b.y, a.z + b.z, a.w + b.w); }

__device__ float4 slow_pq4(const float* __restrict__ emb_row, const float* __restrict__ W1, int K1, int koff, int col, int C1, int H) {
    float r[4] = {0.f, 0.f, 0.f, 0.f};
    for (int j = 0; j < 4; ++j) {
        if (col + j >= C1) break;
        const float* w = W1 + (size_t)(col + j) * K1 + koff;
        float acc = 0.f;
        for (int k = 0; k < H; ++k) acc = fmaf(emb_row[k], w[k], acc);
        r[j] = acc;
    }
    return make_float4(r[0], r[1], r[2], r[3]);
}

__device__ __forceinline__ void lds_barrier() { asm volatile("s_waitcnt lgkmcnt(0)\n\ts_barrier" ::: "memory"); }

template <int RC>
__device__ __forceinline__ void column_stats(const float* col, const int LD, float bias, int b, int e, float* mean, float* rstd) {
    const float inv_n = 1.f / (float)max(e - b, 1);
    const float* p = col + b * LD;
    const int lastoff = max(e - 1 - b, 0) * LD;
    float v[RC];
#pragma unroll
    for (int j = 0; j < RC; ++j) v[j] = p[min(j * LD, lastoff)];
#pragma unroll
    for (int j = 0; j < RC; ++j) v[j] = (b + j < e) ? v[j] + bias : 0.f;
    float s0 = 0.f, s1 = 0.f, s2 = 0.f, s3 = 0.f;
#pragma unroll
    for (int j = 0; j < RC; j += 4) { s0 += v[j]; s1 += v[j + 1]; s2 += v[j + 2]; s3 += v[j + 3]; }
    float s;
    const int n = e - b;
    for (int r0 = RC; r0 < n; r0 += 16) {
        float w[16];
#pragma unroll
        for (int j = 0; j < 16; ++j) w[j] = p[min((r0 + j) * LD, lastoff)];
#pragma unroll
        for (int j = 0; j < 16; j += 4) {
            s0 += (r0 + j < n) ? w[j] + bias : 0.f; s1 += (r0 + j + 1 < n) ? w[j + 1] + bias : 0.f;
            s2 += (r0 + j + 2 < n) ? w[j + 2] + bias : 0.f; s3 += (r0 + j + 3 < n) ? w[j + 3] + bias : 0.f;
        }
    }
    s = (s0 + s1) + (s2 + s3);
    const float mu = s * inv_n;
    float q0 = 0.f, q1 = 0.f, q2 = 0.f, q3 = 0.f;
#pragma unroll
    for (int j = 0; j < RC; j += 4) {
        const float d0 = (b + j < e) ? v[j] - mu : 0.f, d1 = (b + j + 1 < e) ? v[j + 1] - mu : 0.f;
        const float d2 = (b + j + 2 < e) ? v[j + 2] - mu : 0.f, d3 = (b + j + 3 < e) ? v[j + 3] - mu : 0.f;
        q0 = fmaf(d0, d0, q0); q1 = fmaf(d1, d1, q1); q2 = fmaf(d2, d2, q2); q3 = fmaf(d3, d3, q3);
    }
    for (int r0 = RC; r0 < n; r0 += 16) {
        float w[16];
#pragma unroll
        for (int j = 0; j < 16; ++j) w[j] = p[min((r0 + j) * LD, lastoff)];
#pragma unroll
        for (int j = 0; j < 16; j += 4) {
            const float d0 = (r0 + j < n) ? (w[j] + bias) - mu : 0.f, d1 = (r0 + j + 1 < n) ? (w[j + 1] + bias) - mu : 0.f;
            const float d2 = (r0 + j + 2 < n) ? (w[j + 2] + bias) - mu : 0.f, d3 = (r0 + j + 3 < n) ? (w[j + 3] + bias) - mu : 0.f;
            q0 = fmaf(d0, d0, q0); q1 = fmaf(d1, d1, q1); q2 = fmaf(d2, d2, q2); q3 = fmaf(d3, d3, q3);
        }
    }
    const float q = (q0 + q1) + (q2 + q3);
    *mean = mu;
    *rstd = 1.f / sqrtf(q * inv_n + F_EPS);
}

struct FusedArgs {
    const float *emb, *W1, *b1, *b2, *w3, *b3;
    const float4 *Wp1, *Wp2;
    const int32_t *src, *dst, *seg_ptr, *order;
    const float *mask1, *mask2, *u;
    float *P, *Q, *a1, *h2, *stats, *logits, *att;
    const FTile* tiles;
    int* counters;
    int64_t M, N, G;
    SeedRef seed;
    float p;
    int training, noise_philox;
    FusedGeom g;
};

template <bool EDGE, int NRB, int NCB2W, bool X6, bool PQG>
__global__ __launch_bounds__(FT, 2) void k_attn_fused_fwd(const FusedArgs A) {
    extern __shared__ __attribute__((aligned(16))) float lds[];
    const FusedGeom& g = A.g;
    constexpr int CH = EDGE ? 64 : 128, LDT = CH + 4, LDU = 2 * CH + 4, S2 = CH / 8;
    const int H = g.H, C1 = g.C1, C2 = g.C2, LDX = g.LDX, LDH = g.LDH, SW = g.SW;
    float* const X = lds;
    float* const U = lds + g.offU;
    float* const T = lds + g.offT;
    float* const H2 = lds;
    float* const sMean = lds + g.offS;
    int* const meta = reinterpret_cast<int*>(lds + g.offMeta);
    int* const sGptr = meta;
    int* const sRowG = meta + 32;
    int* const sRowId = sRowG + F_RMAX;
    int* const sSrcL = sRowId + F_RMAX;
    int* const sDstL = sSrcL + F_RMAX;
    int* const sCtl = sDstL + F_RMAX;
    float* const sB2 = reinterpret_cast<float*>(sCtl + 16);
    float* const sW3 = sB2 + g.C2p;
    float* const sB1 = sW3 + g.C2p;
    const int tid = threadIdx.x, lane = tid & 63, wave = tid >> 6;
    const int cw = wave & 3, rw = wave >> 2, c = lane & 31, h = lane >> 5;
    const int RM = 64 * NRB;
    const int64_t G = A.G;
    float* const mean1 = A.stats;
    float* const rstd1 = mean1 + (size_t)G * C1;
    float* const mean2 = rstd1 + (size_t)G * C1;
    float* const rstd2 = mean2 + (size_t)G * C2;
    const float sc = (A.training && A.p > 0.f) ? 1.f / (1.f - A.p) : 1.f;
    const bool train = A.training != 0;
    const int ntiles = A.counters[0];
    const int K1 = EDGE ? 2 * H : H;
    const int H4 = H >> 2, C24 = C2 >> 2;
    constexpr int CH4 = CH / 4;

    for (int i = tid; i < g.C2p; i += FT) { sB2[i] = i < C2 ? A.b2[i] : 0.f; sW3[i] = i < C2 ? A.w3[i] : 0.f; }
    for (int i = tid; i < g.NCH * g.CH; i += FT) sB1[i] = i < C1 ? A.b1[i] : 0.f;
#ifdef GSAT_FUSED_STAMPS
    long long stamp[14] = {0, 0, 0, 0, 0, 0, 0, 0, 0, 0, 0, 0, 0, 0};
    long long tlast = __builtin_amdgcn_s_memtime();
#define STAMP(i) do { if (tid == 0) { const long long n_ = __builtin_amdgcn_s_memtime(); stamp[i] += n_ - tlast; tlast = n_; } } while (0)
#else
#define STAMP(i)
#endif
    FTile nxt = A.tiles[min((int)blockIdx.x, max(ntiles - 1, 0))];
    for (int t = blockIdx.x; t < ntiles; t += gridDim.x) {
        lds_barrier();
        const FTile tl = nxt;
        nxt = A.tiles[min(t + (int)gridDim.x, ntiles - 1)];
        const bool big = (tl.flags & 1) != 0;
        const int nslab_m = big ? (tl.nrows + RM - 1) / RM : 1;
        if (tid <= tl.ng) sGptr[tid] = A.seg_ptr[tl.g0 + tid] - tl.row0;
        if (tid == 0) sCtl[1] = 0;

        auto load_x = [&](int x0, int nx) {
            const int fill = min((nx + 31) & ~31, EDGE ? g.RX : RM);
            for (int i0 = tid; i0 < fill * H4; i0 += 4 * FT) {
                float4 v[4];
#pragma unroll
                for (int u = 0; u < 4; ++u) {
                    const int i = min(i0 + u * FT, fill * H4 - 1), r = i / H4, q = i - r * H4;
                    v[u] = ld4(A.emb + (size_t)(x0 + min(r, nx - 1)) * H + 4 * q);
                }
#pragma unroll
                for (int u = 0; u < 4; ++u) {
                    const int i = i0 + u * FT, r = i / H4, q = i - r * H4;
                    if (i < fill * H4) st4(X + r * LDX + 4 * q, r < nx ? v[u] : f4zero());
                }
            }
        };
        auto gemm1 = [&](int kc, int nx) {
            f32x16 acc0, acc1;
            acc_zero(acc0); acc_zero(acc1);
            const float4* bp = A.Wp1 + ((size_t)(kc * 4 + cw) * g.S1) * 64 + lane;
            const uint4* bx = reinterpret_cast<const uint4*>(A.Wp1) + ((size_t)(kc * 4 + cw) * (H / 16)) * 192 + lane;
            if (EDGE) {
                const int rb = rw;
                if (rb * 32 < nx) {
                    if (X6) mma_run_x6<1>(acc0, acc1, X + (rb * 32 + c) * LDX + 8 * h, nullptr, bx, H / 16);
                    else mma_run<1>(acc0, acc1, X + (rb * 32 + c) * LDX + h * (H / 2), nullptr, bp, g.S1);
                    float* const o = U + (rb * 32 + 4 * h) * LDU + cw * 32 + c;
#pragma unroll
                    for (int r = 0; r < 16; ++r) o[((r & 3) + 8 * (r >> 2)) * LDU] = acc0[r];
                }
            } else {
                const int rb0 = rw * NRB;
                const int na = min(NRB, (nx - rb0 * 32 + 31) / 32);
                if (na > 0) {
                    if (X6) {
                        const float* a0 = X + (rb0 * 32 + c) * LDX + 8 * h;
                        if (NRB > 1 && na > 1) mma_run_x6<2>(acc0, acc1, a0, a0 + 32 * LDX, bx, H / 16);
                        else mma_run_x6<1>(acc0, acc1, a0, nullptr, bx, H / 16);
                    } else {
                    const float* a0 = X + (rb0 * 32 + c) * LDX + h * (H / 2);
                    if (NRB > 1 && na > 1) mma_run<2>(acc0, acc1, a0, a0 + 32 * LDX, bp, g.S1);
                    else mma_run<1>(acc0, acc1, a0, nullptr, bp, g.S1);
                    }
                    float* const o = T + (rb0 * 32 + 4 * h) * LDT + cw * 32 + c;
#pragma unroll
                    for (int r = 0; r < 16; ++r) o[((r & 3) + 8 * (r >> 2)) * LDT] = acc0[r];
                    if (NRB > 1 && na > 1) {
#pragma unroll
                        for (int r = 0; r < 16; ++r) o[(32 + (r & 3) + 8 * (r >> 2)) * LDT] = acc1[r];
                    }
                }
            }
        };
        auto gemm1_global = [&](int kc, int x0g, int nx) {
            f32x16 acc0, acc1;
            acc_zero(acc0); acc_zero(acc1);
            const float4* bp = A.Wp1 + ((size_t)(kc * 4 + cw) * g.S1) * 64 + lane;
            const uint4* bx = reinterpret_cast<const uint4*>(A.Wp1) + ((size_t)(kc * 4 + cw) * (H / 16)) * 192 + lane;
            const int rbA = rw, rbB = rw + 2;
            const int na = (rbA * 32 < nx ? 1 : 0) + ((NRB > 1 && rbB * 32 < nx) ? 1 : 0);
            if (na <= 0) return;
            if (X6) {
                const float* a0 = X + (rbA * 32 + c) * LDX + 8 * h;
                if (na > 1) mma_run_x6<2>(acc0, acc1, a0, a0 + 64 * LDX, bx, H / 16);
                else mma_run_x6<1>(acc0, acc1, a0, nullptr, bx, H / 16);
            } else {
                const float* a0 = X + (rbA * 32 + c) * LDX + h * (H / 2);
                if (na > 1) mma_run<2>(acc0, acc1, a0, a0 + 64 * LDX, bp, g.S1);
                else mma_run<1>(acc0, acc1, a0, nullptr, bp, g.S1);
            }
            const int col128 = cw * 32 + c, ch = kc * CH + (col128 & (CH - 1));
            if (ch >= C1) return;
            int c1o = C1;
            asm volatile("" : "+s"(c1o));
            float* const pA = (col128 >= CH ? A.Q : A.P) + ch + (size_t)(x0g + rbA * 32 + 4 * h) * C1;
#pragma unroll
            for (int r = 0; r < 16; ++r) {
                const int rr = (r & 3) + 8 * (r >> 2);
                if (rbA * 32 + 4 * h + rr < nx) pA[rr * c1o] = acc0[r];
            }
            if (na > 1) {
                float* const pB = pA + (size_t)64 * C1;
#pragma unroll
                for (int r = 0; r < 16; ++r) {
                    const int rr = (r & 3) + 8 * (r >> 2);
                    if (rbB * 32 + 4 * h + rr < nx) pB[rr * c1o] = acc1[r];
                }
            }
        };
// ... 69 lines not shown
                }, bMean, bRstd, mean1, rstd1);
            } else {
                big_stats(C1, [&](int r, int col) { return A.P[(size_t)(tl.row0 + r) * C1 + col] + A.b1[col]; }, bMean, bRstd, mean1, rstd1);
            }
        }

        for (int sl = 0; sl < nslab_m; ++sl) {
            const int r0 = sl * RM;
            const int nr = big ? min(RM, tl.nrows - r0) : tl.nrows;
            const int nrp = (nr + 31) & ~31;
            lds_barrier();
            if (!big) load_x(EDGE ? tl.node0 : tl.row0, EDGE ? tl.nnodes : tl.nrows);
            for (int r = tid; r < RM; r += FT) {
                if (r < nr) {
                    const int gr = tl.row0 + r0 + r;
                    const int m = EDGE ? (A.order ? A.order[gr] : gr) : gr;
                    sRowId[r] = m;
                    if (EDGE) {
                        const int s = A.src[m], d = A.dst[m];
                        const int sl_ = s - tl.node0, dl_ = d - tl.node0;
                        sSrcL[r] = (!big && (unsigned)sl_ < (unsigned)tl.nnodes) ? sl_ : -(s + 1);
                        sDstL[r] = (!big && (unsigned)dl_ < (unsigned)tl.nnodes) ? dl_ : -(d + 1);
                        if (!big && ((unsigned)sl_ >= (unsigned)tl.nnodes || (unsigned)dl_ >= (unsigned)tl.nnodes)) sCtl[1] = 1;
                    }
                    int gl = 0;
                    if (!big) {
#pragma unroll
                        for (int k = 1; k < F_GT; ++k) gl += (k < tl.ng && sGptr[k] <= r) ? 1 : 0;
                    }
                    sRowG[r] = gl;
                }
            }
            f32x16 acc2[NCB2W][NRB];
#pragma unroll
            for (int j = 0; j < NCB2W; ++j)
#pragma unroll
                for (int i = 0; i < NRB; ++i) acc_zero(acc2[j][i]);
            lds_barrier();
            STAMP(0);
            if (PQG && !big) {
                for (int kc = 0; kc < g.NCH; ++kc) gemm1_global(kc, tl.node0, tl.nnodes);
                __syncthreads();
                STAMP(1);
            }

            for (int kc = 0; kc < g.NCH; ++kc) {
                if (!big && !PQG) {
                    gemm1(kc, EDGE ? tl.nnodes : tl.nrows);
                    lds_barrier();
                    STAMP(1);
                    save_pq(kc, EDGE ? tl.node0 : tl.row0, EDGE ? tl.nnodes : tl.nrows);
                    STAMP(10);
                }
                if (PQG) {
                    constexpr int GB = 2;
                    for (int i0 = tid; i0 < nrp * CH4; i0 += GB * FT) {
                        float4 pv[GB], qv[GB];
#pragma unroll
                        for (int u = 0; u < GB; ++u) {
                            const int i = min(i0 + u * FT, nrp * CH4 - 1), r = min(i / CH4, nr - 1), q = i - (i / CH4) * CH4;
                            const int col = min(kc * CH + 4 * q, C1 - 4);
                            const int sl_ = sSrcL[r], dl_ = sDstL[r];
                            const int sg = sl_ >= 0 ? tl.node0 + sl_ : -sl_ - 1, dg = dl_ >= 0 ? tl.node0 + dl_ : -dl_ - 1;
                            pv[u] = ld4(A.P + (size_t)sg * C1 + col);
                            qv[u] = ld4(A.Q + (size_t)dg * C1 + col);
                        }
#pragma unroll
                        for (int u = 0; u < GB; ++u) {
                            const int i = i0 + u * FT;
                            if (i < nrp * CH4) {
                                const int r = i / CH4, q = i - r * CH4, col = kc * CH + 4 * q;
                                st4(T + r * LDT + 4 * q, (r < nr && col < C1) ? f4add(pv[u], qv[u]) : f4zero());
                            }
                        }
                    }
                    if (!big && sCtl[1] != 0) {
                        for (int i = tid; i < nr * CH4; i += FT) {
                            const int r = i / CH4, q = i - r * CH4, col = kc * CH + 4 * q;
                            const int sl_ = sSrcL[r], dl_ = sDstL[r];
                            if ((sl_ < 0 || dl_ < 0) && col < C1) {
                                const float4 p4 = sl_ >= 0 ? ld4(A.P + (size_t)(tl.node0 + sl_) * C1 + col) : slow_pq4(A.emb + (size_t)(-sl_ - 1) * H, A.W1, K1, 0, col, C1, H);
                                const float4 q4 = dl_ >= 0 ? ld4(A.Q + (size_t)(tl.node0 + dl_) * C1 + col) : slow_pq4(A.emb + (size_t)(-dl_ - 1) * H, A.W1, K1, H, col, C1, H);
                                st4(T + r * LDT + 4 * q, f4add(p4, q4));
                            }
                        }
                    }
                    lds_barrier();
                    STAMP(2);
                } else if (EDGE || big) {
                    for (int i = tid; i < nrp * CH4; i += FT) {
                        const int r = i / CH4, q = i - r * CH4;
                        float4 v = f4zero();
                        const int col = kc * CH + 4 * q;
                        if (r < nr && col < C1) {
                            if (EDGE) {
                                const int s = sSrcL[r], d = sDstL[r];
                                float4 p4, q4;
                                if (big) {
                                    p4 = ld4(A.P + (size_t)(-s - 1) * C1 + col);
                                    q4 = ld4(A.Q + (size_t)(-d - 1) * C1 + col);
                                } else {
                                    p4 = s >= 0 ? ld4(U + s * LDU + 4 * q) : slow_pq4(A.emb + (size_t)(-s - 1) * H, A.W1, K1, 0, col, C1, H);
                                    q4 = d >= 0 ? ld4(U + d * LDU + CH + 4 * q) : slow_pq4(A.emb + (size_t)(-d - 1) * H, A.W1, K1, H, col, C1, H);
                                }
                                v = f4add(p4, q4);
                            } else {
                                v = ld4(A.P + (size_t)sRowId[r] * C1 + col);
                            }
                        }
                        st4(T + r * LDT + 4 * q, v);
                    }
                    lds_barrier();
                    STAMP(2);
                }
                if (!big) {
                    constexpr int nslot = FT / CH;
                    const int cc = tid % CH, slot = tid / CH;
                    const int col = kc * CH + cc;
                    const float bias = sB1[col];
                    for (int gl = slot; gl < tl.ng; gl += nslot) {
                        float mu, rs;
                        column_stats<32>(T + cc, LDT, bias, sGptr[gl], sGptr[gl + 1], &mu, &rs);
                        sMean[gl * SW + cc] = mu;
                        sMean[(F_GT + gl) * SW + cc] = rs;
                        if (col < C1) { mean1[(size_t)(tl.g0 + gl) * C1 + col] = mu; rstd1[(size_t)(tl.g0 + gl) * C1 + col] = rs; }
                    }
                    STAMP(11);
                    lds_barrier();
                    STAMP(3);
                }
                constexpr int AB = (NRB == 2 && NCB2W == 2) ? 2 : 4;
                for (int i0 = tid; i0 < nr * CH4; i0 += AB * FT) {
                    float4 hv[AB], mu[AB], rs[AB], bb[AB];
                    int mm[AB], rr[AB], qq[AB];
#pragma unroll
                    for (int u = 0; u < AB; ++u) {
                        const int i = min(i0 + u * FT, nr * CH4 - 1);
                        rr[u] = i / CH4; qq[u] = i - rr[u] * CH4;
                        hv[u] = ld4(T + rr[u] * LDT + 4 * qq[u]);
                        bb[u] = ld4(sB1 + kc * CH + 4 * qq[u]);
                        mm[u] = sRowId[rr[u]];
                        if (big) { mu[u] = ld4(bMean + min(kc * CH + 4 * qq[u], C1 - 4)); rs[u] = ld4(bRstd + min(kc * CH + 4 * qq[u], C1 - 4)); }
                        else { const int gl = sRowG[rr[u]]; mu[u] = ld4(sMean + gl * SW + 4 * qq[u]); rs[u] = ld4(sMean + (F_GT + gl) * SW + 4 * qq[u]); }
                    }
#pragma unroll
                    for (int u = 0; u < AB; ++u) {
                        const int col = kc * CH + 4 * qq[u];
                        if (i0 + u * FT < nr * CH4 && col < C1) {
                            const float4 x = f4add(hv[u], bb[u]);
                            const float4 k = keep4f(A.mask1, A.seed, 1, mm[u], col, C1, A.p, train);
                            const float4 y = make_float4(fmaxf((x.x - mu[u].x) * rs[u].x, 0.f) * k.x * sc, fmaxf((x.y - mu[u].y) * rs[u].y, 0.f) * k.y * sc,
                                                         fmaxf((x.z - mu[u].z) * rs[u].z, 0.f) * k.z * sc, fmaxf((x.w - mu[u].w) * rs[u].w, 0.f) * k.w * sc);
                            st4(T + rr[u] * LDT + 4 * qq[u], y);
                            if (A.a1) st4(A.a1 + (size_t)mm[u] * C1 + col, y);
                        }
                    }
                }
                lds_barrier();
                STAMP(4);
                {
                    const int rb0 = rw * NRB;
                    const int na = min(NRB, (nr - rb0 * 32 + 31) / 32);
                    if (na > 0) {
                        const float* a0 = T + (rb0 * 32 + c) * LDT + (X6 ? 8 * h : h * (CH / 2));
#pragma unroll
                        for (int j = 0; j < NCB2W; ++j) {
                            const int cb2 = cw + 4 * j;
                            if (cb2 < g.NCB2) {
                                if (X6) {
                                    const uint4* bx = reinterpret_cast<const uint4*>(A.Wp2) + ((size_t)(kc * g.NCB2 + cb2) * (CH / 16)) * 192 + lane;
                                    if (NRB > 1 && na > 1) mma_run_x6<2>(acc2[j][0], acc2[j][NRB - 1], a0, a0 + 32 * LDT, bx, CH / 16);
                                    else mma_run_x6<1>(acc2[j][0], acc2[j][NRB - 1], a0, nullptr, bx, CH / 16);
                                } else {
                                const float4* bp = A.Wp2 + ((size_t)(kc * g.NCB2 + cb2) * S2) * 64 + lane;
                                if (NRB > 1 && na > 1) mma_run<2>(acc2[j][0], acc2[j][NRB - 1], a0, a0 + 32 * LDT, bp, S2);
                                else mma_run<1>(acc2[j][0], acc2[j][NRB - 1], a0, nullptr, bp, S2);
                                }
                            }
                        }
                    }
                }
                lds_barrier();
                STAMP(5);
            }
            {
                const int rb0 = rw * NRB;
#pragma unroll
                for (int j = 0; j < NCB2W; ++j) {
                    const int cb2 = cw + 4 * j;
                    if (cb2 < g.NCB2) {
#pragma unroll
                        for (int i = 0; i < NRB; ++i) {
                            if ((rb0 + i) * 32 < nrp) {
#pragma unroll
                                for (int r = 0; r < 16; ++r) {
                                    const int row = (rb0 + i) * 32 + (r & 3) + 8 * (r >> 2) + 4 * h;
                                    H2[row * LDH + cb2 * 32 + c] = acc2[j][i][r];
                                }
                            }
                        }
                    }
                }
            }
            lds_barrier();
            for (int i = tid; i < nr * C24; i += FT) {
                const int r = i / C24, q = i - r * C24;
                st4(A.h2 + (size_t)sRowId[r] * C2 + 4 * q, ld4(H2 + r * LDH + 4 * q));
            }
            STAMP(6);
            if (big) continue;
            {
                const int cc = tid % g.C2p, slot = tid / g.C2p, nslot = FT / g.C2p;
                if (slot < nslot) {
                    const float bias = sB2[cc];
                    for (int gl = slot; gl < tl.ng; gl += nslot) {
                        float mu, rs;
                        column_stats<32>(H2 + cc, LDH, bias, sGptr[gl], sGptr[gl + 1], &mu, &rs);
                        sMean[gl * SW + cc] = mu;
                        sMean[(F_GT + gl) * SW + cc] = rs;
                        if (cc < C2) { mean2[(size_t)(tl.g0 + gl) * C2 + cc] = mu; rstd2[(size_t)(tl.g0 + gl) * C2 + cc] = rs; }
                    }
                }
            }
            lds_barrier();
            STAMP(7);
            {
                constexpr int TPR = FT / (64 * NRB);
                const int r = tid / TPR, part = tid % TPR;
                float acc = 0.f;
                int m = 0;
                if (r < nr) {
                    m = sRowId[r];
                    const int gl = sRowG[r];
                    for (int q = part; q < C24; q += TPR) {
                        const float4 hv = f4add(ld4(H2 + r * LDH + 4 * q), ld4(sB2 + 4 * q));
                        const float4 mu = ld4(sMean + gl * SW + 4 * q), rs = ld4(sMean + (F_GT + gl) * SW + 4 * q);
                        const float4 k = keep4f(A.mask2, A.seed, 2, m, 4 * q, C2, A.p, train);
                        const float4 w = ld4(sW3 + 4 * q);
                        acc = fmaf(fmaxf((hv.x - mu.x) * rs.x, 0.f) * k.x * sc, w.x, acc);
                        acc = fmaf(fmaxf((hv.y - mu.y) * rs.y, 0.f) * k.y * sc, w.y, acc);
                        acc = fmaf(fmaxf((hv.z - mu.z) * rs.z, 0.f) * k.z * sc, w.z, acc);
                        acc = fmaf(fmaxf((hv.w - mu.w) * rs.w, 0.f) * k.w * sc, w.w, acc);
                    }
                }
                acc = group_sum<TPR>(acc);
                if (part == 0 && r < nr) {
                    const float z = acc + A.b3[0];
                    A.logits[m] = z;
                    if (A.att) {
                        float tt = z;
                        if (train && (A.u || A.noise_philox)) {
                            const float uu = A.u ? A.u[m] : philox_noise_u(A.seed.get(), m);
                            tt = z + (logf(uu) - logf(1.0f - uu));
                        }
                        A.att[m] = 1.f / (1.f + expf(-tt));
                    }
                }
            }
            STAMP(8);
        }
        if (big) {
            __syncthreads();
            big_stats(C2, [&](int r, int col) {
                const int gr = tl.row0 + r;
                const int m = EDGE ? (A.order ? A.order[gr] : gr) : gr;
                return A.h2[(size_t)m * C2 + col] + A.b2[col];
            }, bMean, bRstd, mean2, rstd2);
            constexpr int TPR = 4;
            for (int rbase = 0; rbase < tl.nrows; rbase += FT / TPR) {
                const int r = rbase + tid / TPR, part = tid % TPR;
                float acc = 0.f;
                int m = 0;
                if (r < tl.nrows) {
                    const int gr = tl.row0 + r;
                    m = EDGE ? (A.order ? A.order[gr] : gr) : gr;
                    for (int q = part; q < C24; q += TPR) {
                        const float4 hv = f4add(ld4(A.h2 + (size_t)m * C2 + 4 * q), ld4(A.b2 + 4 * q));
                        const float4 mu = ld4(bMean + 4 * q), rs = ld4(bRstd + 4 * q);
                        const float4 k = keep4f(A.mask2, A.seed, 2, m, 4 * q, C2, A.p, train);
                        const float4 w = ld4(A.w3 + 4 * q);
                        acc = fmaf(fmaxf((hv.x - mu.x) * rs.x, 0.f) * k.x * sc, w.x, acc);
                        acc = fmaf(fmaxf((hv.y - mu.y) * rs.y, 0.f) * k.y * sc, w.y, acc);
                        acc = fmaf(fmaxf((hv.z - mu.z) * rs.z, 0.f) * k.z * sc, w.z, acc);
                        acc = fmaf(fmaxf((hv.w - mu.w) * rs.w, 0.f) * k.w * sc, w.w, acc);
                    }
                }
                acc = group_sum<TPR>(acc);
                if (part == 0 && r < tl.nrows) {
                    const float z = acc + A.b3[0];
                    A.logits[m] = z;
                    if (A.att) {
                        float tt = z;
                        if (train && (A.u || A.noise_philox)) {
                            const float uu = A.u ? A.u[m] : philox_noise_u(A.seed.get(), m);
                            tt = z + (logf(uu) - logf(1.0f - uu));
                        }
                        A.att[m] = 1.f / (1.f + expf(-tt));
                    }
                }
            }
        }
    }
#ifdef GSAT_FUSED_STAMPS
    STAMP(9);
    if (tid == 0) {
        unsigned long long* o = reinterpret_cast<unsigned long long*>(A.counters + 16);
        for (int i = 0; i < 14; ++i) atomicAdd(o + i, (unsigned long long)stamp[i]);
        atomicAdd(o + 14, 1ull);
    }
#endif
}

template <bool EDGE, int NRB, int NCB2W, bool X6 = false, bool PQG = false>
static int launch_fused(hipStream_t stream, const FusedArgs& fa, int grid) {
    static size_t allowed = 64 * 1024;
    const size_t lds = (size_t)fa.g.lds_bytes;
    if (lds > allowed) {
        GSAT_CHECK_HIP(hipFuncSetAttribute((const void*)k_attn_fused_fwd<EDGE, NRB, NCB2W, X6, PQG>, hipFuncAttributeMaxDynamicSharedMemorySize, (int)lds));
        allowed = lds;
    }
    k_attn_fused_fwd<EDGE, NRB, NCB2W, X6, PQG><<<grid, FT, lds, stream>>>(fa);
    GSAT_LAUNCH_CHECK();
    return GSAT_OK;
}

size_t attn_plan_bytes(int64_t G) { return align_up((size_t)(G + 1 + (G + 63) / 64 * 64) * sizeof(FTile), 256); }
bool attn_plan_ok(int64_t G) { return G > 0 && G <= (int64_t)PLAN_MAX_SB * 64; }
int attn_plan_launch(hipStream_t stream, const int32_t* seg_ptr, const int32_t* node_ptr, int64_t G, int RM, int RX, FTile* tiles, int* counters) {
    k_attn_plan<<<1, PLAN_T, 0, stream>>>(seg_ptr, node_ptr, (int)G, RM, RX, tiles, counters);
    GSAT_LAUNCH_CHECK();
    return GSAT_OK;
}

bool attn_fused_eligible(const gsat_attn_args* a, FusedGeom* g) {
    const char* env = getenv("GSAT_ATTN_FUSED");
    const int want = a->fused != 0 ? a->fused : (env ? (atoi(env) != 0 ? 1 : -1) : 0);
    if (want < 0) return false;
    if (a->M <= 0 || a->G <= 0 || a->G > (int64_t)PLAN_MAX_SB * 64) return false;
    if (!a->edge_mode && a->seg_order) return false;
    if (a->edge_mode && !a->node_ptr) return false;
    {
        const char* ep = getenv("GSAT_ATTN_FUSED_PQG");
        const bool pqg = a->edge_mode && !(ep && atoi(ep) == 0);
        if (!(pqg && fused_geometry(a->H, a->C1, a->C2, true, g, true) && g->NRB == 2) && !fused_geometry(a->H, a->C1, a->C2, a->edge_mode != 0, g, false)) return false;
    }
    {
        const char* ex = getenv("GSAT_ATTN_FUSED_X6");
        g->x6 = (!(ex && atoi(ex) == 0) && a->H % 16 == 0 && g->NRB == 2 && g->NCB2 <= 4) ? 1 : 0;
    }
    if (a->M > a->G * (int64_t)(2 * g->RM)) return false;
    if (want == 0 && (a->edge_mode || !g->x6 || a->M < 32768)) return false;
    return true;
}

int attn_fused_fwd(hipStream_t stream, const gsat_attn_args* a, const FusedGeom& g) {
    const size_t need = fused_ws_bytes(g, a->G);
    GSAT_REQUIRE(a->fwd_workspace && a->fwd_workspace_bytes >= need, GSAT_ERR_WORKSPACE, "gsat_attn_fwd: workspace %zu < %zu (fused path)",
                 a->fwd_workspace_bytes, need);
    char* w = static_cast<char*>(a->fwd_workspace);
    int* counters = reinterpret_cast<int*>(w); w += 256;
    FTile* tiles = reinterpret_cast<FTile*>(w); w += align_up((size_t)(a->G + 1 + (a->G + 63) / 64 * 64) * sizeof(FTile), 256);
    float4* Wp1 = reinterpret_cast<float4*>(w); w += align_up((size_t)g.NCH * 4 * g.S1 * 64 * 24, 256);
    float4* Wp2 = reinterpret_cast<float4*>(w);
    const int64_t nflt4 = (int64_t)g.NCH * 4 * g.S1 * 64 + (int64_t)g.NCH * g.NCB2 * g.S2 * 64;
    const int pack_blocks = (int)std::min<int64_t>(ceil_div(nflt4, PLAN_T), 512);
    const int32_t* node_ptr = a->edge_mode ? a->node_ptr : a->seg_ptr;
    k_attn_prep<<<1 + pack_blocks, PLAN_T, 0, stream>>>(a->W1, a->W2, g, a->edge_mode, a->seg_ptr, node_ptr, (int)a->G, tiles, counters, Wp1, Wp2);
    GSAT_LAUNCH_CHECK();
    FusedArgs fa{};
    fa.emb = a->emb; fa.W1 = a->W1; fa.b1 = a->b1; fa.b2 = a->b2; fa.w3 = a->W3; fa.b3 = a->b3;
    fa.Wp1 = Wp1; fa.Wp2 = Wp2;
    fa.src = a->src; fa.dst = a->dst; fa.seg_ptr = a->seg_ptr; fa.order = a->seg_order;
    fa.mask1 = a->mask1; fa.mask2 = a->mask2; fa.u = a->u;
    fa.P = a->P; fa.Q = a->Q; fa.a1 = a->a1; fa.h2 = a->h2; fa.stats = a->stats; fa.logits = a->logits; fa.att = a->att;
    fa.tiles = tiles; fa.counters = counters;
    fa.M = a->M; fa.N = a->N; fa.G = a->G;
    fa.seed = SeedRef{a->seed, a->seed_dev};
    fa.p = a->p_drop; fa.training = a->training; fa.noise_philox = a->noise_philox;
    fa.g = g;
    static int cus = 0;
    if (!cus) {
        int dev = 0;
        hipDeviceProp_t prop;
        GSAT_CHECK_HIP(hipGetDevice(&dev));
        GSAT_CHECK_HIP(hipGetDeviceProperties(&prop, dev));
        cus = prop.multiProcessorCount > 0 ? prop.multiProcessorCount : 256;
    }
    const int grid = (int)std::min<int64_t>(cus, a->G);
    const bool e = a->edge_mode != 0;
    const int ncbw = g.NCB2 > 4 ? 2 : 1;
#define GO(E, R, W) return launch_fused<E, R, W>(stream, fa, grid)
    if (e && g.pqg) {
        if (g.x6) return launch_fused<true, 2, 1, true, true>(stream, fa, grid);
        if (ncbw == 2) return launch_fused<true, 2, 2, false, true>(stream, fa, grid);
        return launch_fused<true, 2, 1, false, true>(stream, fa, grid);
    }
    if (g.x6) { if (e) return launch_fused<true, 2, 1, true>(stream, fa, grid); return launch_fused<false, 2, 1, true>(stream, fa, grid); }
    if (e) { if (g.NRB == 2) { if (ncbw == 2) GO(true, 2, 2); GO(true, 2, 1); } if (ncbw == 2) GO(true, 1, 2); GO(true, 1, 1); }
    if (g.NRB == 2) { if (ncbw == 2) GO(false, 2, 2); GO(false, 2, 1); }
    if (ncbw == 2) GO(false, 1, 2);
    GO(false, 1, 1);
#undef GO
}

}
```

dp_gsat_amd/ops.py:

```python
from __future__ import annotations

import os
from typing import Optional

import torch

from ._lib import call, ptr, stream
from .graph_index import BatchIndex


def _f32c(t: Optional[torch.Tensor]) -> Optional[torch.Tensor]:
    if t is None:
        return None
    if isinstance(t, LiftedAttention):
        raise TypeError("LiftedAttention reached an autograd Function: pass dp_gsat_amd.ops.edge_tensor(att) instead")
    if t.dtype != torch.float32:
        raise TypeError("dp_gsat_amd kernels compute in fp32; got " + str(t.dtype))
    return t.contiguous()


def _flat_att(att: Optional[torch.Tensor], E: int) -> Optional[torch.Tensor]:
    if att is None:
        return None
    if isinstance(att, LiftedAttention):
# ... 187 lines not shown
        out = torch.empty(N, S * A * F, dtype=torch.float32, device=x.device)
        hubs = index.long_rows_nowait[0]
        if hubs is not None:
            call("gsat_pna_fwd_long", ptr(x), ptr(attf), ptr(edge_emb), ptr(index.rowptr_dst), ptr(index.src_by_dst), ptr(index.eid_by_dst),
                 N, index.E, H, a_arr, A, s_arr, S, float(avg_lin), float(avg_log), ptr(out), ptr(hubs),
                 ptr(index.pna_partial(H, edge_emb is not None)), stream())
        else:
            call("gsat_pna_fwd", ptr(x), ptr(attf), ptr(edge_emb), ptr(index.rowptr_dst), ptr(index.src_by_dst),
                 ptr(index.eid_by_dst), N, H, a_arr, A, s_arr, S, float(avg_lin), float(avg_log), ptr(out), stream())
        ctx.save_for_backward(x, attf, edge_emb)
        ctx.index = index
        ctx.cfg = (tuple(aggr_codes), tuple(scaler_codes), float(avg_lin), float(avg_log))
        ctx.att_shape = None if att is None else att.shape
        return (out, x_in) if passthrough else out

    @staticmethod
    def _forward_node_att(ctx, x, node_att, index, aggr_codes, scaler_codes, avg_lin, avg_log):
        import ctypes
        N, H = x.shape
        if N != index.N or node_att.numel() != N:
            raise ValueError(f"x / node attention have {N} / {node_att.numel()} rows but the index was built for {index.N} nodes")
        na = _f32c(node_att).view(-1)
        A, S = len(aggr_codes), len(scaler_codes)
        a_arr = (ctypes.c_int32 * A)(*aggr_codes)
        s_arr = (ctypes.c_int32 * S)(*scaler_codes)
        out = torch.empty(N, S * A * 2 * H, dtype=torch.float32, device=x.device)
        call("gsat_pna_fwd_node_att", ptr(x), ptr(na), ptr(index.rowptr_dst), ptr(index.src_by_dst), N, H, a_arr, A, s_arr, S,
             float(avg_lin), float(avg_log), ptr(out), stream())
        ctx.save_for_backward(x, na)
        ctx.index, ctx.node_att = index, True
        ctx.cfg = (tuple(aggr_codes), tuple(scaler_codes), float(avg_lin), float(avg_log))
        ctx.att_shape = node_att.shape
        return out

    @staticmethod
    def _backward_node_att(ctx, dout, dx_add=None):
        import ctypes
        x, na = ctx.saved_tensors
        index = ctx.index
        aggr_codes, scaler_codes, _, _ = ctx.cfg
        dout = _f32c(dout)
        N, H = x.shape
        A, S = len(aggr_codes), len(scaler_codes)
        a_arr = (ctypes.c_int32 * A)(*aggr_codes)
        s_arr = (ctypes.c_int32 * S)(*scaler_codes)
        dev = x.device
        need_att = ctx.needs_input_grad[8]
        tile_ptr, T, rows_nominal, rows_cap, edges_cap, spill = index.pna_tiles(H)
        dmsg = torch.empty(max(index.E, 1), H, dtype=torch.float32, device=dev)[: index.E]
        dw = torch.empty(max(index.E, 1), dtype=torch.float32, device=dev) if need_att else None
        dna, acc, ret = None, 0, None
        if need_att:
            if ctx.lifted is not None:
                dna, acc, ret = ctx.lifted._shared_dna(N, dev)
            else:
                dna = ret = torch.empty(N, dtype=torch.float32, device=dev)
        dx = torch.empty_like(x)
        call("gsat_pna_bwd_tiled_node_att", ptr(x), ptr(na), ptr(dout), ptr(index.rowptr_dst), ptr(index.src_by_dst), ptr(tile_ptr), T,
             rows_nominal, rows_cap, edges_cap, ptr(index.rowptr_src), ptr(index.slot_dst_of_srcslot), N, index.E, H, a_arr, A, s_arr, S,
             ptr(spill[1:]), ptr(spill[:1]), ptr(dx), ptr(dmsg), ptr(dna), ptr(dw), ptr(dx_add), acc, stream())
        return dx, None, None, None, None, None, None, None, (ret.view(ctx.att_shape) if ret is not None else None), None, None

    @staticmethod
    def backward(ctx, dout, dx_add=None):
        import ctypes
        dx_add = None if dx_add is None else _f32c(dx_add)
        if dout is None:
            return dx_add, None, None, None, None, None, None, None, None, None, None
        if ctx.node_att:
            return PnaAggregate._backward_node_att(ctx, dout, dx_add)
        x, attf, edge_emb = ctx.saved_tensors
        index = ctx.index
        aggr_codes, scaler_codes, avg_lin, avg_log = ctx.cfg
        dout = _f32c(dout)
        N, H = x.shape
        A, S = len(aggr_codes), len(scaler_codes)
        a_arr = (ctypes.c_int32 * A)(*aggr_codes)
        s_arr = (ctypes.c_int32 * S)(*scaler_codes)
        need_att = attf is not None and ctx.needs_input_grad[1]
        need_ee = edge_emb is not None and ctx.needs_input_grad[2]
        dev = x.device
        dmsg = torch.empty(max(index.E, 1), H, dtype=torch.float32, device=dev)[: index.E]
        datt = torch.empty(index.E, dtype=torch.float32, device=dev) if need_att else None
        tiles = None
        hubs = index.long_rows_nowait[0]
        from .graph_index import sync_free
        if (edge_emb is None and _FIXED_PNA.get((aggr_codes, scaler_codes)) and os.environ.get("GSAT_PNA_TILED", "1") != "0"
                and (hubs is None or sync_free())):
            tiles = index.pna_tiles(H) or None
        if tiles is not None:
            tile_ptr, T, rows_nominal, rows_cap, edges_cap, spill = tiles
            dx = torch.empty_like(x)
            call("gsat_pna_bwd_tiled", ptr(x), ptr(attf), ptr(dout), ptr(index.rowptr_dst), ptr(index.src_by_dst), ptr(index.eid_by_dst),
                 ptr(tile_ptr), T, rows_nominal, rows_cap, edges_cap, ptr(index.rowptr_src), ptr(index.slot_dst_of_srcslot), N, index.E, H,
                 a_arr, A, s_arr, S, ptr(spill[1:]), ptr(spill[:1]), ptr(dx), ptr(dmsg), ptr(datt), ptr(dx_add), stream())
            return dx, (datt.view(ctx.att_shape) if need_att else None), None, None, None, None, None, None, None, None, None
        dx_self = torch.empty_like(x)
        dee = torch.empty_like(edge_emb) if need_ee else None
        if hubs is not None:
            call("gsat_pna_bwd_long", ptr(x), ptr(attf), ptr(edge_emb), ptr(dout), ptr(index.rowptr_dst), ptr(index.src_by_dst),
                 ptr(index.eid_by_dst), N, index.E, H, a_arr, A, s_arr, S, avg_lin, avg_log, ptr(dx_self), ptr(dmsg), ptr(datt),
                 ptr(dee), ptr(hubs), ptr(index.pna_partial(H, edge_emb is not None)), stream())
        else:
            call("gsat_pna_bwd", ptr(x), ptr(attf), ptr(edge_emb), ptr(dout), ptr(index.rowptr_dst), ptr(index.src_by_dst),
                 ptr(index.eid_by_dst), N, H, a_arr, A, s_arr, S, avg_lin, avg_log, ptr(dx_self), ptr(dmsg), ptr(datt),
                 ptr(dee), stream())
        dx = torch.empty_like(x)
        call("gsat_aggr_sum_fwd", ptr(dmsg), ptr(dx_self), None, None, ptr(index.rowptr_src),
             ptr(index.slot_dst_of_srcslot), None, N, index.E, H, 1.0, ptr(dx),
             ptr(index.long_rows[1]), ptr(index.partial(H)) if index.long_rows[1] is not None else None, stream())
        if dx_add is not None:
            dx = dx + dx_add
        return dx, (datt.view(ctx.att_shape) if need_att else None), dee, None, None, None, None, None, None, None, None


def pna_aggregate(x, index, att, edge_emb, aggregators, scalers, avg_deg, passthrough: bool = False):
    a = [AGGREGATOR_CODES[k] for k in aggregators]
    s = [SCALER_CODES[k] for k in scalers]
    if isinstance(att, LiftedAttention):
        if (edge_emb is None and att.index is index and _FIXED_PNA.get((tuple(a), tuple(s))) and index.long_rows_nowait[0] is None
                and os.environ.get("GSAT_PNA_TILED", "1") != "0" and os.environ.get("GSAT_NODE_ATT_LIFT", "0") != "1"
                and att._edge is None and index.pna_tiles(x.shape[1])):
            return PnaAggregate.apply(x, None, None, index, a, s, avg_deg["lin"], avg_deg["log"], att.shared_node_att, passthrough, att)
        att = att.edge()
    return PnaAggregate.apply(x, att, edge_emb, index, a, s, avg_deg["lin"], avg_deg["log"], None, passthrough)


def _attn_args(emb, params, index, segments, edge_mode, training, p, seed, mask1, mask2, u, bufs, seed_dev=None, noise_philox=False):
    from ._lib import AttnArgs
    W1, b1, W2, b2, W3, b3 = params
    N, H = emb.shape
    C1, C2 = W1.shape[0], W2.shape[0]
    a = AttnArgs()
    if edge_mode:
        eptr, order, _, eg32 = segments.edge_segments
        a.M, a.seg_ptr, a.seg_order, a.row_seg = index.E, ptr(eptr), ptr(order), ptr(eg32)
        a.src, a.dst = ptr(index.src32), ptr(index.dst32)
    else:
        a.M, a.seg_ptr, a.seg_order, a.row_seg = N, ptr(segments.node_ptr), None, ptr(segments.node_seg32)
        a.src, a.dst = None, None
    a.N, a.G, a.H, a.C1, a.C2 = N, segments.G, H, C1, C2
    a.edge_mode, a.training, a.p_drop, a.seed = int(edge_mode), int(training), float(p), int(seed) & ((1 << 64) - 1)
    a.W1, a.b1, a.W2, a.b2, a.W3, a.b3 = ptr(W1), ptr(b1), ptr(W2), ptr(b2), ptr(W3), ptr(b3)
    a.emb, a.mask1, a.mask2, a.u = ptr(emb), ptr(mask1), ptr(mask2), ptr(u)
    P, Q, a1, h2, stats, logits, att = bufs
    a.P, a.Q, a.a1, a.h2, a.stats, a.logits, a.att = ptr(P), ptr(Q), ptr(a1), ptr(h2), ptr(stats), ptr(logits), ptr(att)
    a.seed_dev = ptr(seed_dev)
    a.noise_philox = int(bool(noise_philox) and u is None)
    a.fused = 0
    a.node_ptr = ptr(segments.node_ptr)
    return a


class ExtractorAttention(torch.autograd.Function):

    last_forward_kind = 0

    @staticmethod
    def forward(ctx, emb, W1, b1, W2, b2, W3, b3, index, segments, edge_mode, training, p, seed, mask1, mask2, u, seed_dev=None, noise_philox=False):
        import ctypes
        ctx.set_materialize_grads(False)
        emb = _f32c(emb)
        params = tuple(_f32c(t) for t in (W1, b1, W2, b2, W3, b3))
        mask1, mask2 = _f32c(mask1), _f32c(mask2)
        u = None if u is None else _f32c(u).view(-1)
        N, H = emb.shape
        C1, C2 = params[0].shape[0], params[2].shape[0]
        C0 = 2 * H if edge_mode else H
        if params[0].shape[1] != C0 or params[2].shape[1] != C1 or tuple(params[4].shape) != (1, C2):
            raise ValueError("extractor weight shapes do not match the embedding width")
        if N != index.N:
            raise ValueError(f"emb has {N} rows but the index was built for {index.N} nodes")
        M = index.E if edge_mode else N
        for m_, c_ in ((mask1, C1), (mask2, C2)):
            if m_ is not None and tuple(m_.shape) != (M, c_):
                raise ValueError("dropout keep-mask has the wrong shape")
        if u is not None and u.numel() != M:
            raise ValueError("noise tensor has the wrong number of entries")
        dev, f32 = emb.device, torch.float32
        G = segments.G
        P = torch.empty(N, C1, dtype=f32, device=dev)
        Q = torch.empty(N, C1, dtype=f32, device=dev) if edge_mode else None
        a1 = torch.empty(M, C1, dtype=f32, device=dev)
        h2 = torch.empty(M, C2, dtype=f32, device=dev)
        stats = torch.empty(max(G, 1) * (2 * C1 + 2 * C2), dtype=f32, device=dev)
        logits = torch.empty(M, 1, dtype=f32, device=dev)
        att = torch.empty(M, 1, dtype=f32, device=dev)
        bufs = (P, Q, a1, h2, stats, logits, att)
        args = _attn_args(emb, params, index, segments, edge_mode, training, p, seed, mask1, mask2, u, bufs, seed_dev, noise_philox)
        from ._lib import load
        fws_bytes = int(load().gsat_attn_fwd_workspace_bytes(ctypes.byref(args)))
        ExtractorAttention.last_forward_kind = int(load().gsat_attn_fwd_kind(ctypes.byref(args)))
        if fws_bytes:
            fws = torch.empty(fws_bytes, dtype=torch.uint8, device=dev)
            args.fwd_workspace, args.fwd_workspace_bytes = ptr(fws), fws_bytes
        call("gsat_attn_fwd", ctypes.byref(args), stream())
        ctx.save_for_backward(emb, *params, P, Q if Q is not None else emb.new_empty(0), a1, h2, stats, att,
                              mask1 if mask1 is not None else emb.new_empty(0),
                              mask2 if mask2 is not None else emb.new_empty(0),
                              u if u is not None else emb.new_empty(0))
        ctx.meta = (index, segments, bool(edge_mode), bool(training), float(p), int(seed),
                    mask1 is not None, mask2 is not None, u is not None)
        ctx.seed_dev = seed_dev
        return logits, att

    @staticmethod
    def backward(ctx, dlogits, datt):
        import ctypes
        from ._lib import AttnGrads, load
        (emb, W1, b1, W2, b2, W3, b3, P, Q, a1, h2, stats, att, mask1, mask2, u) = ctx.saved_tensors
        index, segments, edge_mode, training, p, seed, has_m1, has_m2, has_u = ctx.meta
        params = (W1, b1, W2, b2, W3, b3)
        logits_dummy = att
        bufs = (P, Q if edge_mode else None, a1, h2, stats, logits_dummy, att)
        args = _attn_args(emb, params, index, segments, edge_mode, training, p, seed, mask1 if has_m1 else None,
                          mask2 if has_m2 else None, u if has_u else None, bufs, ctx.seed_dev)
        g = AttnGrads()
        dlogits = None if dlogits is None else _f32c(dlogits)
        datt = None if datt is None else _f32c(datt)
        g.dlogits, g.datt = ptr(dlogits), ptr(datt)
        if edge_mode:
            g.rowptr_src, g.eid_by_src = ptr(index.rowptr_src), ptr(index.eid_by_src)
            g.rowptr_dst, g.eid_by_dst = ptr(index.rowptr_dst), ptr(index.eid_by_dst)
            g.chunk_ptr_dst, g.chunk_ptr_src = (ptr(t) for t in index.long_rows)
        demb = torch.empty_like(emb)
        grads = [torch.empty_like(t) for t in params]
        g.demb = ptr(demb)
        g.dW1, g.db1, g.dW2, g.db2, g.dW3, g.db3 = (ptr(t) for t in grads)
        ws_bytes = int(load().gsat_attn_bwd_workspace_bytes(ctypes.byref(args)))
        ws = torch.empty(ws_bytes, dtype=torch.uint8, device=emb.device)
        g.workspace, g.workspace_bytes = ptr(ws), ws_bytes
        call("gsat_attn_bwd", ctypes.byref(args), ctypes.byref(g), stream())
        return (demb, *grads, None, None, None, None, None, None, None, None, None, None, None)


def new_seed() -> int:
    return int(torch.empty((), dtype=torch.int64).random_().item())


_DEVICE_SEEDS = {}


def device_seed(device) -> torch.Tensor:
    if os.environ.get("GSAT_DEVICE_SEEDS", "1") == "0":
        return torch.empty(1, dtype=torch.int64, device=device).random_()
    capturing = torch.cuda.is_current_stream_capturing()
    ent = _DEVICE_SEEDS.get(str(device))
    if ent is None:
        if capturing:
            return torch.empty(1, dtype=torch.int64, device=device).random_()
        ent = [torch.tensor([new_seed(), 0], dtype=torch.int64, device=device), torch.initial_seed()]
        _DEVICE_SEEDS[str(device)] = ent
    elif ent[1] != torch.initial_seed() and not capturing:
        ent[0].copy_(torch.tensor([new_seed(), 0], dtype=torch.int64))
        ent[1] = torch.initial_seed()
    out = torch.empty(1, dtype=torch.int64, device=device)
    call("gsat_seed_next", ptr(ent[0]), ptr(out), stream())
    return out


def device_seed_state(device) -> Optional[torch.Tensor]:
    ent = _DEVICE_SEEDS.get(str(device))
    return None if ent is None else ent[0]


class Sample(torch.autograd.Function):

    @staticmethod
    def forward(ctx, logits, noise, mode: int, temp: float, eps: float):
        z = _f32c(logits)
        nz = None if noise is None else _f32c(noise)
        att = torch.empty_like(z)
        call("gsat_sample_fwd", ptr(z), ptr(nz), int(mode), float(temp), float(eps), z.numel(), ptr(att), stream())
        ctx.save_for_backward(att)
        ctx.temp = float(temp)
        return att

    @staticmethod
    def backward(ctx, datt):
        (att,) = ctx.saved_tensors
        datt = _f32c(datt)
        dz = torch.empty_like(att)
        call("gsat_sample_bwd", ptr(att), ptr(datt), ctx.temp, att.numel(), ptr(dz), stream())
        return dz, None, None, None, None


class Lift(torch.autograd.Function):

    @staticmethod
    def forward(ctx, node_att, index: BatchIndex):
        a = _f32c(node_att)
        if a.numel() != index.N:
            raise ValueError("node attention must have one entry per node")
        out = torch.empty(index.E, 1, dtype=torch.float32, device=a.device)
        call("gsat_lift_fwd", ptr(a), ptr(index.src32), ptr(index.dst32), index.E, ptr(out), stream())
        ctx.save_for_backward(a)
        ctx.index = index
        return out

    @staticmethod
    def backward(ctx, dout):
        (a,) = ctx.saved_tensors
        ix = ctx.index
        dout = _f32c(dout)
        da = torch.empty_like(a)
        call("gsat_lift_bwd", ptr(a), ptr(dout), ptr(ix.rowptr_src), ptr(ix.dst_by_src), ptr(ix.eid_by_src),
             ptr(ix.rowptr_dst), ptr(ix.src_by_dst), ptr(ix.eid_by_dst), ix.N, ptr(da), stream())
        return da, None


class Symmetrise(torch.autograd.Function):

    @staticmethod
    def forward(ctx, att, rev, flag=None):
        a = _f32c(att)
        out = torch.empty_like(a)
        call("gsat_symmetrise", ptr(a), ptr(rev), ptr(flag), a.numel(), ptr(out), stream())
        ctx.save_for_backward(rev, flag if flag is not None else rev.new_empty(0))
        ctx.has_flag = flag is not None
        return out

    @staticmethod
    def backward(ctx, dout):
        rev, flag = ctx.saved_tensors
        d = _f32c(dout)
        da = torch.empty_like(d)
        call("gsat_symmetrise", ptr(d), ptr(rev), ptr(flag if ctx.has_flag else None), d.numel(), ptr(da), stream())
        return da, None, None


class InfoLoss(torch.autograd.Function):

    @staticmethod
    def forward(ctx, att, r, m_valid=None, r_dev=None):
        a = _f32c(att)
        r_vec = _f32c(r.detach()) if isinstance(r, torch.Tensor) else None
        r_scalar = 0.0 if r_vec is not None else float(r)
        if r_vec is not None and r_vec.numel() != a.numel():
            raise ValueError("tensor prior must have one entry per attention value")
        out = torch.empty((), dtype=torch.float32, device=a.device)
        partial = torch.empty(1024, dtype=torch.float32, device=a.device)
        if m_valid is None:
            if r_dev is not None:
                raise ValueError("a device r needs the count-aware info loss (m_valid)")
            call("gsat_info_loss_fwd", ptr(a), ptr(r_vec), r_scalar, a.numel(), ptr(partial), ptr(out), stream())
        else:
            if r_dev is not None and (r_vec is not None or r_dev.dtype != torch.float32 or r_dev.numel() != 1):
                raise ValueError("r_dev must be one float32 on the device, without a tensor prior")
            call("gsat_info_loss_valid_fwd", ptr(a), ptr(r_vec), r_scalar, ptr(r_dev), a.numel(), ptr(m_valid), ptr(partial), ptr(out), stream())
        ctx.save_for_backward(a, r_vec if r_vec is not None else a.new_empty(0))
        ctx.r_scalar, ctx.has_vec = r_scalar, r_vec is not None
        ctx.m_valid, ctx.r_dev = m_valid, r_dev
        return out

    @staticmethod
    def backward(ctx, gout):
        a, r_vec = ctx.saved_tensors
        gout = _f32c(gout)
        da = torch.empty_like(a)
        if ctx.m_valid is None:
            call("gsat_info_loss_bwd", ptr(a), ptr(r_vec if ctx.has_vec else None), ctx.r_scalar, ptr(gout), a.numel(), ptr(da), stream())
        else:
            call("gsat_info_loss_valid_bwd", ptr(a), ptr(r_vec if ctx.has_vec else None), ctx.r_scalar, ptr(ctx.r_dev), ptr(gout), a.numel(),
                 ptr(ctx.m_valid), ptr(da), stream())
        return da, None, None, None


class F1SparsityLoss(torch.autograd.Function):

    @staticmethod
    def forward(ctx, p, y, m_valid=None):
        a, b = _f32c(p), _f32c(y.detach())
        if a.numel() != b.numel() or a.numel() == 0:
            raise ValueError("f1 sparsity loss: p and y need the same, non-zero number of entries")
        if m_valid is not None and (m_valid.dtype != torch.int32 or m_valid.numel() != 1 or not m_valid.is_cuda):
            raise ValueError("m_valid must be one int32 on the device")
        out = torch.empty((), dtype=torch.float32, device=a.device)
        stats = torch.empty(8, dtype=torch.float32, device=a.device)
        partial = torch.empty(1024, dtype=torch.float32, device=a.device)
        call("gsat_f1_sparsity_fwd", ptr(a), ptr(b), a.numel(), ptr(m_valid), ptr(partial), ptr(out), ptr(stats), stream())
        ctx.save_for_backward(a, b, stats)
        ctx.m_valid = m_valid
        return out

    @staticmethod
# ... 387 lines not shown
```

include/gsat_hip.h:

```cpp
#ifndef GSAT_HIP_H
#define GSAT_HIP_H

#include <stddef.h>
#include <stdint.h>

#ifdef __cplusplus
extern "C" {
#endif

#define GSAT_ABI_VERSION 4

#define GSAT_OK 0
#define GSAT_ERR_HIP (-1)
#define GSAT_ERR_ARG (-2)
#define GSAT_ERR_WORKSPACE (-3)
#define GSAT_ERR_UNSUPPORTED (-4)
#define GSAT_ERR_BLAS (-5)

int gsat_abi_version(void);

int gsat_seed_next(uint64_t* state, uint64_t* out, void* stream);
const char* gsat_last_error(void);


// ... 68 lines not shown
                 float* dedge_emb, void* stream);

size_t gsat_pna_long_row_floats(int64_t num_edges, int64_t H, int has_edge_emb);
int gsat_pna_fwd_long(const float* x, const float* att, const float* edge_emb, const int32_t* rowptr,
                      const int32_t* col, const int32_t* eid, int64_t num_rows, int64_t num_edges, int64_t H,
                      const int32_t* aggregators, int num_aggregators, const int32_t* scalers, int num_scalers,
                      float avg_deg_lin, float avg_deg_log, float* out, const int32_t* chunk_ptr, float* workspace, void* stream);
int gsat_pna_bwd_long(const float* x, const float* att, const float* edge_emb, const float* dout,
                      const int32_t* rowptr, const int32_t* col, const int32_t* eid, int64_t num_rows, int64_t num_edges, int64_t H,
                      const int32_t* aggregators, int num_aggregators, const int32_t* scalers, int num_scalers,
                      float avg_deg_lin, float avg_deg_log, float* dx_self, float* dmsg, float* datt,
                      float* dedge_emb, const int32_t* chunk_ptr, float* workspace, void* stream);

int gsat_pna_tile_plan(int64_t H, int64_t lds_budget_bytes, int32_t* rows_nominal, int32_t* rows_slack, int32_t* edges_cap);
int gsat_pna_build_tiles(const int32_t* node_ptr, const int32_t* node_seg, const int32_t* rowptr, const int32_t* rowptr_src,
                         const int32_t* slot_dst_of_srcslot, int64_t num_rows, int rows_nominal, int rows_slack, int edges_cap,
                         int32_t* tile_desc, int32_t* spill_rows , int32_t* spill_count , void* stream);
int gsat_pna_bwd_tiled(const float* x, const float* att, const float* dout, const int32_t* rowptr, const int32_t* col,
                       const int32_t* eid, const int32_t* tile_desc, int64_t num_tiles, int rows_nominal, int rows_cap, int edges_cap,
                       const int32_t* rowptr_src, const int32_t* slot_dst_of_srcslot, int64_t num_rows, int64_t num_edges, int64_t H,
                       const int32_t* aggregators, int num_aggregators, const int32_t* scalers, int num_scalers,
                       const int32_t* spill_rows, const int32_t* spill_count, float* dx, float* dmsg, float* datt,
                       const float* dx_add ,
                       void* stream);

int gsat_pna_fwd_compact(const float* x, const float* att, const int32_t* rowptr, const int32_t* col, const int32_t* eid, int64_t num_rows,
                         int64_t H, const int32_t* aggregators, int num_aggregators, float* aggj, float* scal, void* stream);
int gsat_pna_post_fwd(const float* x, const float* aggj, const float* scal, int64_t num_rows, int64_t H,
                      int num_aggregators, const float* W, int64_t ldw, const float* bias, int64_t Ho, float* out, void* stream);
size_t gsat_pna_post_dw_workspace_floats(int64_t num_rows, int64_t H, int num_aggregators, int64_t Ho);
int gsat_pna_post_dw(const float* x, const float* aggj, const float* scal, int64_t num_rows, int64_t H,
                     int num_aggregators, const float* dout, int64_t Ho, float* dW, float* workspace, size_t workspace_floats, void* stream);

int gsat_pna_fwd_node_att(const float* x, const float* node_att, const int32_t* rowptr, const int32_t* col, int64_t num_rows, int64_t H,
                          const int32_t* aggregators, int num_aggregators, const int32_t* scalers, int num_scalers, float avg_deg_lin,
                          float avg_deg_log, float* out, void* stream);
int gsat_pna_bwd_tiled_node_att(const float* x, const float* node_att, const float* dout, const int32_t* rowptr, const int32_t* col,
                                const int32_t* tile_desc, int64_t num_tiles, int rows_nominal, int rows_cap, int edges_cap,
                                const int32_t* rowptr_src, const int32_t* slot_dst_of_srcslot, int64_t num_rows, int64_t num_edges, int64_t H,
                                const int32_t* aggregators, int num_aggregators, const int32_t* scalers, int num_scalers,
                                const int32_t* spill_rows, const int32_t* spill_count, float* dx, float* dmsg, float* dnode_att, float* dw,
                                const float* dx_add, int accumulate_dnode_att ,
                                void* stream);


size_t gsat_bn_workspace_floats(int64_t N, int64_t C);
int gsat_bn_fwd(const float* x, const float* gamma, const float* beta, float* running_mean, float* running_var,
                int64_t N, int64_t C, int training, float momentum, float eps, int relu, float* y,
                float* save_mean, float* save_rstd, float* workspace, void* stream);
int gsat_bn_bwd(const float* x, const float* dy, const float* gamma, const float* beta, const float* save_mean,
                const float* save_rstd, int64_t N, int64_t C, int training, int relu, float* dx, float* dgamma,
                float* dbeta, float* workspace, void* stream);

int gsat_bn_act_fwd(const float* x, const float* gamma, const float* beta, float* running_mean, float* running_var,
                    int64_t N, int64_t C, int training, float momentum, float eps, int relu, const float* residual,
                    float dropout_p, uint64_t seed, const uint64_t* seed_dev, float* y, float* save_mean,
                    float* save_rstd, float* workspace, void* stream);
int gsat_bn_act_bwd(const float* x, const float* dy, const float* gamma, const float* beta, const float* save_mean,
                    const float* save_rstd, int64_t N, int64_t C, int training, int relu, float dropout_p,
                    uint64_t seed, const uint64_t* seed_dev, float* dx, float* dresidual, float* dgamma,
                    float* dbeta, float* workspace, void* stream);

int gsat_bn_act_fwd_valid(const float* x, const float* gamma, const float* beta, float* running_mean, float* running_var,
                          int64_t N, int64_t C, int training, float momentum, float eps, int relu, const float* residual,
                          float dropout_p, uint64_t seed, const uint64_t* seed_dev, float* y, float* save_mean,
                          float* save_rstd, float* workspace, const int32_t* n_valid_dev, void* stream);
int gsat_bn_act_bwd_valid(const float* x, const float* dy, const float* gamma, const float* beta, const float* save_mean,
                          const float* save_rstd, int64_t N, int64_t C, int training, int relu, float dropout_p,
                          uint64_t seed, const uint64_t* seed_dev, float* dx, float* dresidual, float* dgamma,
                          float* dbeta, float* workspace, const int32_t* n_valid_dev, void* stream);

int gsat_bn_local_sum(const float* x, const float* centre, int64_t N, int64_t C, float* out, float* workspace, void* stream);
int gsat_bn_apply_fwd(const float* x, const float* gamma, const float* beta, const float* mean, const float* rstd, int64_t N, int64_t C,
                      int relu, const float* residual, float dropout_p, uint64_t seed, const uint64_t* seed_dev, float* y, void* stream);
int gsat_bn_local_bwd_sums(const float* x, const float* dy, const float* gamma, const float* beta, const float* mean, const float* rstd,
                           int64_t N, int64_t C, int relu, float dropout_p, uint64_t seed, const uint64_t* seed_dev, float* sum_dy,
                           float* sum_dy_xhat, float* workspace, void* stream);
int gsat_bn_apply_bwd(const float* x, const float* dy, const float* gamma, const float* beta, const float* mean, const float* rstd,
                      const float* sum_dy, const float* sum_dy_xhat, int64_t global_rows, const float* global_rows_dev , int64_t N, int64_t C,
                      int relu, float dropout_p, uint64_t seed, const uint64_t* seed_dev, float* dx, float* dresidual, void* stream);

size_t gsat_colsum_workspace_floats(int64_t C);
int gsat_colsum(const float* x, int64_t R, int64_t C, float* out, float* workspace, void* stream);


int gsat_embsum_fwd(const int64_t* x, const int32_t* dims, int ncol, const float* W, int64_t N, int64_t H,
                    float* out, void* stream);
int gsat_onehot_rows(const int64_t* x, const int32_t* dims, int ncol, int64_t N, int64_t R_padded, float* O,
                     void* stream);


size_t gsat_gemm_workspace_floats(int a_t, int64_t M, int64_t N, int64_t K);
int gsat_gemm_plan(int allow_split, int a_t, int b_t, int64_t M, int64_t N, int64_t K, int has_bias, int accumulate,
                   int64_t ldb, int32_t* plan);
int gsat_gemm_f32(int a_t, int b_t, int64_t M, int64_t N, int64_t K, const float* A, int64_t lda,
                  const float* B, int64_t ldb, float* C, int64_t ldc, const float* bias, int accumulate,
                  float* workspace, size_t workspace_floats, void* stream);
int gsat_gemm_bf16x3(int a_t, int b_t, int64_t M, int64_t N, int64_t K, const float* A, int64_t lda,
                     const float* B, int64_t ldb, float* C, int64_t ldc, const float* bias, int accumulate,
                     float* workspace, size_t workspace_floats, void* stream);


typedef struct gsat_attn_args {
    int64_t M, N, G;
    int32_t H, C1, C2;
    int32_t edge_mode;
    int32_t training;
    float p_drop;
    uint64_t seed;
    const int32_t* src;
    const int32_t* dst;
    const int32_t* seg_ptr;
    const int32_t* seg_order;
    const int32_t* row_seg;
    const float *W1, *b1, *W2, *b2, *W3, *b3;
    const float* emb;
    const float* mask1;
    const float* mask2;
    const float* u;
    float* P;
    float* Q;
    float* a1;
    float* h2;
    float* stats;
    float* logits;
    float* att;
    void* fwd_workspace;
    size_t fwd_workspace_bytes;
    const uint64_t* seed_dev;
    int32_t noise_philox;
    int32_t fused;
    const int32_t* node_ptr;
} gsat_attn_args;

typedef struct gsat_attn_grads {
    const float* dlogits;
    const float* datt;
    const int32_t* rowptr_src;
    const int32_t* eid_by_src;
    const int32_t* rowptr_dst;
    const int32_t* eid_by_dst;
    const int32_t* chunk_ptr_src;
    const int32_t* chunk_ptr_dst;
    float *demb, *dW1, *db1, *dW2, *db2, *dW3, *db3;
    void* workspace;
    size_t workspace_bytes;
} gsat_attn_grads;

size_t gsat_attn_fwd_workspace_bytes(const gsat_attn_args* args);
int gsat_attn_fwd_kind(const gsat_attn_args* args);
size_t gsat_attn_bwd_workspace_bytes(const gsat_attn_args* args);
int gsat_attn_fwd(const gsat_attn_args* args, void* stream);
int gsat_attn_bwd(const gsat_attn_args* args, const gsat_attn_grads* grads, void* stream);

int gsat_instance_norm_fwd(const float* x, const int32_t* seg_ptr, const int32_t* seg_order,
                           const int32_t* row_seg, int64_t M, int64_t G, int64_t C, float* y,
                           float* stats, void* stream);
int gsat_instance_norm_bwd(const float* y, const float* dy, const float* stats, const int32_t* seg_ptr,
                           const int32_t* seg_order, const int32_t* row_seg, int64_t M, int64_t G,
                           int64_t C, float* dx, float* workspace , void* stream);

int gsat_philox_noise(uint64_t seed, int64_t M, float* u, void* stream);

int gsat_philox_keep_mask(uint64_t seed, int32_t layer, int64_t M, int64_t C, float p_drop, float* keep,
                          void* stream);

int gsat_relu_dropout_fwd(const float* x, int64_t N, int64_t C, float dropout_p, uint64_t seed, const uint64_t* seed_dev, float* y,
                          void* stream);
int gsat_relu_dropout_bwd(const float* y, const float* dy, int64_t N, int64_t C, float dropout_p, float* dx, void* stream);


int gsat_sample_fwd(const float* logits, const float* noise, int mode, float temp, float eps, int64_t M,
                    float* att, void* stream);
int gsat_sample_bwd(const float* att, const float* datt, float temp, int64_t M, float* dlogits, void* stream);

int gsat_lift_fwd(const float* node_att, const int32_t* src, const int32_t* dst, int64_t num_edges,
                  float* edge_att, void* stream);
int gsat_lift_bwd(const float* node_att, const float* dedge_att, const int32_t* rowptr_src,
                  const int32_t* dst_by_src, const int32_t* eid_by_src, const int32_t* rowptr_dst,
                  const int32_t* src_by_dst, const int32_t* eid_by_dst, int64_t num_nodes,
                  float* dnode_att, void* stream);

int gsat_symmetrise(const float* att, const int32_t* rev, const int32_t* undirected_flag ,
                    int64_t num_edges, float* out, void* stream);

int gsat_info_loss_fwd(const float* att, const float* r_vec, float r_scalar, int64_t M, float* partial,
                       float* out, void* stream);
int gsat_info_loss_bwd(const float* att, const float* r_vec, float r_scalar, const float* gout, int64_t M,
                       float* datt, void* stream);

int gsat_info_loss_valid_fwd(const float* att, const float* r_vec, float r_scalar, const float* r_dev, int64_t M,
                             const int32_t* m_valid_dev, float* partial, float* out, void* stream);
int gsat_info_loss_valid_bwd(const float* att, const float* r_vec, float r_scalar, const float* r_dev, const float* gout,
                             int64_t M, const int32_t* m_valid_dev, float* datt, void* stream);

int gsat_f1_sparsity_fwd(const float* p, const float* y, int64_t M, const int32_t* m_valid_dev, float* partial, float* loss,
                         float* stats, void* stream);
int gsat_f1_sparsity_bwd(const float* p, const float* y, const float* stats, const float* gout, int64_t M,
                         const int32_t* m_valid_dev, float* dp, void* stream);
int64_t gsat_f1_sparsity_block_entries(void);
int64_t gsat_f1_sparsity_max_blocks(void);

int gsat_narrow_i64(const int64_t* in, int64_t n, int32_t* out, void* stream);


int gsat_collate(const int64_t* graph_ids, int64_t num_graphs, const int64_t* node_ptr_all, const int64_t* edge_ptr_all,
                 const int64_t* edge_local_all, int64_t num_edges_all, const int64_t* out_node_ptr,
                 const int64_t* out_edge_ptr, int64_t N, int64_t E, int64_t* batch, int64_t* node_src_row,
                 int64_t* edge_index, int64_t* edge_src_slot, void* stream);

int gsat_collate_padded(const int64_t* graph_ids, int64_t num_graphs, const int64_t* node_ptr_all, const int64_t* edge_ptr_all,
                        const int64_t* edge_local_all, int64_t num_edges_all, const int64_t* out_node_ptr,
                        const int64_t* out_edge_ptr, int64_t N_cap, int64_t E_cap, int64_t* batch, int64_t* node_src_row,
                        int64_t* edge_index, int64_t* edge_src_slot, int32_t* valid, void* stream);

int gsat_line_graph_pair_counts(const int32_t* rowptr_src, int64_t num_nodes, int64_t* counts, void* stream);
int gsat_line_graph(const int32_t* rowptr_src, const int32_t* eid_by_src, const int64_t* pair_ptr, int64_t num_nodes,
                    int64_t num_pairs, int64_t* dual_edge_index, void* stream);

size_t gsat_und_edges_workspace_bytes(int64_t num_edges);
int gsat_und_edges(const int64_t* edge_index, int64_t num_edges, int64_t num_nodes, uint64_t* sorted_keys, int32_t* rowptr,
                   int32_t* und_of_slot, int32_t* und_of_edge, int32_t* und_src, int32_t* und_dst, int32_t* status,
                   void* workspace, size_t workspace_bytes, void* stream);
int gsat_und_line_graph_counts(const int32_t* rowptr, const int32_t* und_of_slot, const int32_t* und_src, const int32_t* und_dst,
                               int64_t num_und, int64_t* counts, void* stream);
int gsat_und_line_graph(const int32_t* rowptr, const int32_t* und_of_slot, const int32_t* und_src, const int32_t* und_dst,
                        const int64_t* dual_ptr, int64_t num_und, int64_t total, int64_t* dual_edge_index, void* stream);


int gsat_segment_pool_fwd(const float* x, const int32_t* ptr, int64_t num_segments, int64_t H,
                          int mean, float* out, void* stream);
int gsat_segment_pool_bwd(const float* dout, const int32_t* ptr, int64_t num_segments, int64_t H,
                          int mean, float* dx, void* stream);


int64_t gsat_rank_edges_lds_cap(void);
size_t gsat_rank_edges_workspace_bytes(int64_t num_edges);
int gsat_rank_edges(const float* att, const int32_t* edge_ptr, const int32_t* edge_order, const uint8_t* label, int64_t num_edges,
                    int64_t num_graphs, int64_t k, int64_t max_seg_edges, int path, int32_t* order, int32_t* rank, uint8_t* topk,
                    int32_t* hits, void* workspace, size_t workspace_bytes, void* stream);

size_t gsat_auroc_workspace_bytes(int64_t num_edges);
int gsat_auroc(const float* att, const uint8_t* label, int64_t num_edges, uint64_t* out, void* workspace, size_t workspace_bytes,
               void* stream);

size_t gsat_delta_kl_workspace_bytes(int64_t num_edges);
int gsat_delta_kl(const float* att, const uint8_t* label, int64_t num_edges, double eps, float* out, void* workspace,
                  size_t workspace_bytes, void* stream);


size_t gsat_auroc_tasks_workspace_bytes(int64_t num_rows, int64_t num_tasks);
int gsat_auroc_tasks(const float* score, const float* label, int64_t num_rows, int64_t num_tasks, uint64_t* out, void* workspace,
                     size_t workspace_bytes, void* stream);

int gsat_att_histogram(const float* att, const uint8_t* label, int64_t num_edges, int64_t bins, double lo, double hi, uint64_t* hist,
                       uint64_t* outside, void* stream);


int64_t gsat_subgraph_block_items(void);
size_t gsat_subgraph_workspace_bytes(int64_t num_nodes, int64_t num_edges);
int gsat_subgraph_index(const int64_t* edge_index, int64_t num_edges, int64_t num_nodes, const int64_t* batch, const int32_t* node_ptr,
                        int64_t num_graphs, const uint8_t* keep, int mode, int drop_isolated, int phases, int64_t cap_nodes,
                        int64_t cap_edges, int exact, int64_t* node_id, int64_t* edge_id, int64_t* new_edge_index, int64_t* new_batch,
                        int32_t* new_node_ptr, uint8_t* edge_mask, int64_t* counts, void* workspace, size_t workspace_bytes,
                        void* stream);

int gsat_gather_rows(const void* table, const int64_t* index, int64_t n, int64_t row_bytes, void* out, void* stream);


int gsat_eval_log_append(const float* att, const uint8_t* label, const int32_t* edge_ptr, const int32_t* edge_order, const float* logits,
                         const float* y, const int32_t* valid, const float* losses, int64_t edge_cap, int64_t graph_cap,
                         int64_t logit_cols, int64_t y_cols, float* log_att, uint8_t* log_label, int32_t* log_graph_edge_ptr,
                         float* log_logits, float* log_y, int64_t* log_batch_edge_ptr, double* log_loss_sums, int64_t* log_state,
                         int64_t max_edges, int64_t max_graphs, int64_t max_batches, void* stream);

int64_t gsat_delta_kl_segments_chunk(void);
size_t gsat_delta_kl_segments_workspace_bytes(int64_t num_segments, int64_t max_seg_len);
int gsat_delta_kl_segments(const float* att, const uint8_t* label, const int64_t* seg_ptr, int64_t num_segments, int64_t num_edges,
                           int64_t max_seg_len, double eps, float* out, void* workspace, size_t workspace_bytes, void* stream);

#ifdef __cplusplus
}
#endif
#endif
```

Baseline: 125.4.

## Save packed ReLU/dropout activity bits in attention forward for backward gating

The forward pass now writes a per-element activity nibble (ReLU positive and dropout kept) for the two hidden layers into uint8 buffers. The backward kernels read these bits instead of regenerating philox dropout masks or reading masks, and a new head-backward kernel fuses the statistics and dh2 application while reducing three accumulators in one shared-memory pass. This trades extra forward stores and saved memory for less RNG recomputation and mask traffic in backward. Launch bounds are also adjusted for the bit-gated variant.

```diff
diff --git a/dp_gsat_amd/_lib.py b/dp_gsat_amd/_lib.py
--- a/dp_gsat_amd/_lib.py
+++ b/dp_gsat_amd/_lib.py
@@ -70,6 +70,8 @@
     "gsat_attn_bwd_workspace_bytes": (SZ, [P]),
     "gsat_attn_fwd": (INT, [P, P]),
     "gsat_attn_bwd": (INT, [P, P, P]),
+    "gsat_attn_fwd_bits": (INT, [P, P, P, P]),
+    "gsat_attn_bwd_bits": (INT, [P, P, P, P, P]),
     "gsat_instance_norm_fwd": (INT, [P, P, P, P, I64, I64, I64, P, P, P]),
     "gsat_instance_norm_bwd": (INT, [P, P, P, P, P, P, I64, I64, I64, P, P, P]),
     "gsat_philox_keep_mask": (INT, [U64, I32, I64, I64, F32, P, P]),
diff --git a/dp_gsat_amd/csrc/attn.hip b/dp_gsat_amd/csrc/attn.hip
--- a/dp_gsat_amd/csrc/attn.hip
+++ b/dp_gsat_amd/csrc/attn.hip
@@ -53,6 +53,22 @@
 #pragma unroll
         for (int s = 0; s < SB_SLOTS; ++s) {
             float4 t = sm[s][lane];
+            r.x += t.x; r.y += t.y; r.z += t.z; r.w += t.w;
+        }
+    }
+    return r;
+}
+
+template <int NQ>
+__device__ __forceinline__ float4 slot_reduce_n(const float4* v, float4 (*sm)[SB_SLOTS][SB_LANES], int slot, int lane) {
+#pragma unroll
+    for (int k = 0; k < NQ; ++k) sm[k][slot][lane] = v[k];
+    __syncthreads();
+    float4 r = f4zero();
+    if (slot < NQ) {
+#pragma unroll
+        for (int s = 0; s < SB_SLOTS; ++s) {
+            float4 t = sm[slot][s][lane];
             r.x += t.x; r.y += t.y; r.z += t.z; r.w += t.w;
         }
     }
@@ -116,7 +132,7 @@
                                                   const int32_t* __restrict__ order, float* __restrict__ mean_out,
                                                   float* __restrict__ rstd_out, const float* __restrict__ mask = nullptr,
                                                   SeedRef seed = SeedRef{0, nullptr}, int layer = 0, float p = 0.f, int training = 0,
-                                                  float* __restrict__ act_out = nullptr) {
+                                                  float* __restrict__ act_out = nullptr, uint8_t* __restrict__ act_bits = nullptr) {
     __shared__ float4 sm[SB_SLOTS][SB_LANES];
     __shared__ float4 bc[SB_LANES];
     const int g = blockIdx.x;
@@ -183,17 +199,19 @@
                     const int m = mc[i];
                     const float4 h = hc[i];
                     const float4 k = keep4(mask, seed, layer, m, c, C, p, training != 0);
-                    st4(act_out + (size_t)m * C + c,
-                        make_float4(fmaxf((h.x - mu.x) * rs.x, 0.f) * k.x * sc, fmaxf((h.y - mu.y) * rs.y, 0.f) * k.y * sc,
-                                    fmaxf((h.z - mu.z) * rs.z, 0.f) * k.z * sc, fmaxf((h.w - mu.w) * rs.w, 0.f) * k.w * sc));
+                    const float4 a = make_float4(fmaxf((h.x - mu.x) * rs.x, 0.f) * k.x * sc, fmaxf((h.y - mu.y) * rs.y, 0.f) * k.y * sc,
+                                                 fmaxf((h.z - mu.z) * rs.z, 0.f) * k.z * sc, fmaxf((h.w - mu.w) * rs.w, 0.f) * k.w * sc);
+                    st4(act_out + (size_t)m * C + c, a);
+                    if (act_bits) act_bits[(size_t)m * (C >> 2) + (c >> 2)] = (uint8_t)act_nibble(a);
                 }
             for (int r = rest; r < end; r += SB_SLOTS) {
                 const int m = order ? order[r] : r;
                 const float4 h = pre.load(m, c);
                 const float4 k = keep4(mask, seed, layer, m, c, C, p, training != 0);
-                st4(act_out + (size_t)m * C + c,
-                    make_float4(fmaxf((h.x - mu.x) * rs.x, 0.f) * k.x * sc, fmaxf((h.y - mu.y) * rs.y, 0.f) * k.y * sc,
-                                fmaxf((h.z - mu.z) * rs.z, 0.f) * k.z * sc, fmaxf((h.w - mu.w) * rs.w, 0.f) * k.w * sc));
+                const float4 a = make_float4(fmaxf((h.x - mu.x) * rs.x, 0.f) * k.x * sc, fmaxf((h.y - mu.y) * rs.y, 0.f) * k.y * sc,
+                                             fmaxf((h.z - mu.z) * rs.z, 0.f) * k.z * sc, fmaxf((h.w - mu.w) * rs.w, 0.f) * k.w * sc);
+                st4(act_out + (size_t)m * C + c, a);
+                if (act_bits) act_bits[(size_t)m * (C >> 2) + (c >> 2)] = (uint8_t)act_nibble(a);
             }
         }
     }
@@ -202,7 +220,7 @@
 template <bool EDGE, bool RELU>
 __global__ void k_norm_apply(PreAct<EDGE> pre, const int32_t* __restrict__ row_seg, const float* __restrict__ mean,
                              const float* __restrict__ rstd, const float* __restrict__ mask, SeedRef seed, int layer,
-                             float p, int training, int64_t M, float* __restrict__ out) {
+                             float p, int training, int64_t M, float* __restrict__ out, uint8_t* __restrict__ act_bits = nullptr) {
     const int C = pre.C, C4 = C >> 2;
     const float sc = (training && p > 0.f) ? 1.f / (1.f - p) : 1.f;
     for (int64_t i = (int64_t)blockIdx.x * blockDim.x + threadIdx.x; i < M * C4; i += (int64_t)gridDim.x * blockDim.x) {
@@ -214,6 +232,7 @@
         if (RELU) {
             float4 k = keep4(mask, seed, layer, m, c, C, p, training != 0);
             y = make_float4(fmaxf(y.x, 0.f) * k.x * sc, fmaxf(y.y, 0.f) * k.y * sc, fmaxf(y.z, 0.f) * k.z * sc, fmaxf(y.w, 0.f) * k.w * sc);
+            if (act_bits) act_bits[i] = (uint8_t)act_nibble(y);
         }
         st4(out + (size_t)m * C + c, y);
     }
@@ -225,7 +244,7 @@
                                                   const float* __restrict__ rstd, const float* __restrict__ mask, SeedRef seed,
                                                   float p, int training, const float* __restrict__ w3, const float* __restrict__ b3,
                                                   const float* __restrict__ u, int noise_philox, int64_t M, int C, float* __restrict__ logits,
-                                                  float* __restrict__ att) {
+                                                  float* __restrict__ att, uint8_t* __restrict__ act_bits) {
     const int lane = threadIdx.x % LPR;
     const float sc = (training && p > 0.f) ? 1.f / (1.f - p) : 1.f;
     PreAct<false> pre{h2, nullptr, b2, nullptr, nullptr, C};
@@ -237,10 +256,12 @@
             float4 mu = ld4(mean + (size_t)g * C + c), rs = ld4(rstd + (size_t)g * C + c);
             float4 k = keep4(mask, seed, 2, (int)m, c, C, p, training != 0);
             float4 w = ld4(w3 + c);
-            acc = fmaf(fmaxf((h.x - mu.x) * rs.x, 0.f) * k.x * sc, w.x, acc);
-            acc = fmaf(fmaxf((h.y - mu.y) * rs.y, 0.f) * k.y * sc, w.y, acc);
-            acc = fmaf(fmaxf((h.z - mu.z) * rs.z, 0.f) * k.z * sc, w.z, acc);
-            acc = fmaf(fmaxf((h.w - mu.w) * rs.w, 0.f) * k.w * sc, w.w, acc);
+            const float4 y = make_float4((h.x - mu.x) * rs.x, (h.y - mu.y) * rs.y, (h.z - mu.z) * rs.z, (h.w - mu.w) * rs.w);
+            acc = fmaf(fmaxf(y.x, 0.f) * k.x * sc, w.x, acc);
+            acc = fmaf(fmaxf(y.y, 0.f) * k.y * sc, w.y, acc);
+            acc = fmaf(fmaxf(y.z, 0.f) * k.z * sc, w.z, acc);
+            acc = fmaf(fmaxf(y.w, 0.f) * k.w * sc, w.w, acc);
+            if (act_bits) act_bits[(size_t)m * (C >> 2) + (c >> 2)] = (uint8_t)act_nibble(y, k);
         }
         acc = group_sum<LPR>(acc);
         if (lane == 0) {
@@ -358,10 +379,119 @@
     }
 }
 
+template <bool APPLY>
+__global__ __launch_bounds__(SB) void k_head_bwd_bits(const float* __restrict__ h2, const float* __restrict__ b2,
+                                                      const int32_t* __restrict__ seg_ptr, const int32_t* __restrict__ order,
+                                                      const float* __restrict__ mean, const float* __restrict__ rstd,
+                                                      const uint8_t* __restrict__ act, float sc, const float* __restrict__ w3,
+                                                      const DzSrc dzs, int C, float* __restrict__ S1, float* __restrict__ S2,
+                                                      float* __restrict__ dw3p, float* __restrict__ dzsum = nullptr,
+                                                      float* __restrict__ dh2 = nullptr) {
+    __shared__ float4 sm[3][SB_SLOTS][SB_LANES];
+    __shared__ float4 bc1[SB_LANES], bc2[SB_LANES];
+    __shared__ float sdz[SB_SLOTS];
+    const int g = blockIdx.x;
+    const int lane = threadIdx.x % SB_LANES, slot = threadIdx.x / SB_LANES;
+    const int c = (blockIdx.y * SB_LANES + lane) * 4;
+    const int C4 = C >> 2, q = c >> 2;
+    const bool on = c < C;
+    int beg, end; float inv_n;
+    seg_slice(seg_ptr, g, &beg, &end, &inv_n);
+    if (gridDim.z > 1) inv_n = 1.f;
+    const size_t orow = gridDim.z > 1 ? (size_t)g * gridDim.z + blockIdx.z : (size_t)g;
+    PreAct<false> pre{h2, nullptr, b2, nullptr, nullptr, C};
+    float4 hc[SB_RC];
+    float dc[SB_RC];
+    unsigned bcache[SB_RC];
+    int mc[SB_RC];
+#pragma unroll
+    for (int i = 0; i < SB_RC; ++i) {
+        const int r = beg + slot + i * SB_SLOTS;
+        mc[i] = (r < end && on) ? (order ? order[r] : r) : -1;
+    }
+#pragma unroll
+    for (int i = 0; i < SB_RC; ++i) {
+        hc[i] = mc[i] >= 0 ? pre.load(mc[i], c) : f4zero();
+        dc[i] = mc[i] >= 0 ? dzs.get(mc[i]) : 0.f;
+        bcache[i] = mc[i] >= 0 ? (unsigned)act[(size_t)mc[i] * C4 + q] : 0u;
+    }
+    const int rest = beg + slot + SB_RC * SB_SLOTS;
+    const float4 mu = on ? ld4(mean + (size_t)g * C + c) : f4zero(), rs = on ? ld4(rstd + (size_t)g * C + c) : f4zero();
+    const float4 w = on ? ld4(w3 + c) : f4zero();
+    float4 a1 = f4zero(), a2 = f4zero(), a3 = f4zero();
+    float dsum = 0.f;
+#define GSAT_H2_Y(H4) const float4 y = make_float4(((H4).x - mu.x) * rs.x, ((H4).y - mu.y) * rs.y, ((H4).z - mu.z) * rs.z, ((H4).w - mu.w) * rs.w);
+#define GSAT_H2_DY(D, B)                                                                                                           \
+    const float4 dy = make_float4(((B) & 1u) ? (D) * w.x * sc : 0.f, ((B) & 2u) ? (D) * w.y * sc : 0.f,                              \
+                                  ((B) & 4u) ? (D) * w.z * sc : 0.f, ((B) & 8u) ? (D) * w.w * sc : 0.f);
+#define GSAT_H2_ACC(H4, D, B)                                                                                                      \
+    {                                                                                                                              \
+        GSAT_H2_Y(H4)                                                                                                              \
+        GSAT_H2_DY(D, B)                                                                                                           \
+        a1.x += dy.x; a1.y += dy.y; a1.z += dy.z; a1.w += dy.w;                                                                    \
+        a2.x = fmaf(dy.x, y.x, a2.x); a2.y = fmaf(dy.y, y.y, a2.y); a2.z = fmaf(dy.z, y.z, a2.z); a2.w = fmaf(dy.w, y.w, a2.w);      \
+        a3.x = fmaf((D), ((B) & 1u) ? y.x * sc : 0.f, a3.x); a3.y = fmaf((D), ((B) & 2u) ? y.y * sc : 0.f, a3.y);                    \
+        a3.z = fmaf((D), ((B) & 4u) ? y.z * sc : 0.f, a3.z); a3.w = fmaf((D), ((B) & 8u) ? y.w * sc : 0.f, a3.w);                    \
+        dsum += (D);                                                                                                               \
+    }
+    if (on) {
+#pragma unroll
+        for (int i = 0; i < SB_RC; ++i)
+            if (mc[i] >= 0) GSAT_H2_ACC(hc[i], dc[i], bcache[i])
+        for (int r = rest; r < end; r += SB_SLOTS) {
+            const int m = order ? order[r] : r;
+            const float d = dzs.get(m);
+            const float4 h = pre.load(m, c);
+            const unsigned b = act[(size_t)m * C4 + q];
+            GSAT_H2_ACC(h, d, b)
+        }
+    }
+#undef GSAT_H2_ACC
+    if (lane == 0) sdz[slot] = dsum;
+    const float4 acc3[3] = {a1, a2, a3};
+    float4 t = slot_reduce_n<3>(acc3, sm, slot, lane);
+    if (slot < 2) t = make_float4(t.x * inv_n, t.y * inv_n, t.z * inv_n, t.w * inv_n);
+    if (slot < 3 && on) st4((slot == 0 ? S1 : slot == 1 ? S2 : dw3p) + orow * C + c, t);
+    if (dzsum && blockIdx.y == 0 && slot == 3 && lane == 0) {
+        float d = 0.f;
+#pragma unroll
+        for (int s_ = 0; s_ < SB_SLOTS; ++s_) d += sdz[s_];
+        dzsum[g] = d;
+    }
+    if (APPLY) {
+        if (slot == 0) bc1[lane] = t;
+        if (slot == 1) bc2[lane] = t;
+        __syncthreads();
+        if (!on) return;
+        const float4 s1 = bc1[lane], s2 = bc2[lane];
+#define GSAT_H2_OUT(M_, H4, D, B)                                                                                                  \
+        {                                                                                                                          \
+            GSAT_H2_Y(H4)                                                                                                          \
+            GSAT_H2_DY(D, B)                                                                                                       \
+            st4(dh2 + (size_t)(M_) * C + c, make_float4(rs.x * (dy.x - s1.x - y.x * s2.x), rs.y * (dy.y - s1.y - y.y * s2.y),        \
+                                                         rs.z * (dy.z - s1.z - y.z * s2.z), rs.w * (dy.w - s1.w - y.w * s2.w)));     \
+        }
+#pragma unroll
+        for (int i = 0; i < SB_RC; ++i)
+            if (mc[i] >= 0) GSAT_H2_OUT(mc[i], hc[i], dc[i], bcache[i])
+        for (int r = rest; r < end; r += SB_SLOTS) {
+            const int m = order ? order[r] : r;
+            const float d = dzs.get(m);
+            const float4 h = pre.load(m, c);
+            const unsigned b = act[(size_t)m * C4 + q];
+            GSAT_H2_OUT(m, h, d, b)
+        }
+#undef GSAT_H2_OUT
+    }
+#undef GSAT_H2_DY
+#undef GSAT_H2_Y
+}
+
 __global__ void k_dh2(const float* __restrict__ h2, const float* __restrict__ b2, const int32_t* __restrict__ row_seg,
                       const float* __restrict__ mean, const float* __restrict__ rstd, const float* __restrict__ mask, SeedRef seed,
                       float p, int training, const float* __restrict__ w3, const float* __restrict__ dz,
-                      const float* __restrict__ S1, const float* __restrict__ S2, int64_t M, int C, float* __restrict__ dh2) {
+                      const float* __restrict__ S1, const float* __restrict__ S2, int64_t M, int C, float* __restrict__ dh2,
+                      const uint8_t* __restrict__ act = nullptr ) {
     const int C4 = C >> 2;
     const float sc = (training && p > 0.f) ? 1.f / (1.f - p) : 1.f;
     PreAct<false> pre{h2, nullptr, b2, nullptr, nullptr, C};
@@ -371,27 +501,35 @@
         const float d = dz[m];
         float4 h = pre.load(m, c);
         float4 mu = ld4(mean + (size_t)g * C + c), rs = ld4(rstd + (size_t)g * C + c), w = ld4(w3 + c);
-        float4 k = keep4(mask, seed, 2, m, c, C, p, training != 0);
         float4 s1 = ld4(S1 + (size_t)g * C + c), s2 = ld4(S2 + (size_t)g * C + c);
         float4 y = make_float4((h.x - mu.x) * rs.x, (h.y - mu.y) * rs.y, (h.z - mu.z) * rs.z, (h.w - mu.w) * rs.w);
-        float4 dy = make_float4(y.x > 0.f ? d * w.x * k.x * sc : 0.f, y.y > 0.f ? d * w.y * k.y * sc : 0.f,
-                                y.z > 0.f ? d * w.z * k.z * sc : 0.f, y.w > 0.f ? d * w.w * k.w * sc : 0.f);
+        float4 dy;
+        if (act) {
+            const unsigned b = act[i];
+            dy = make_float4((b & 1u) ? d * w.x * sc : 0.f, (b & 2u) ? d * w.y * sc : 0.f, (b & 4u) ? d * w.z * sc : 0.f, (b & 8u) ? d * w.w * sc : 0.f);
+        } else {
+            float4 k = keep4(mask, seed, 2, m, c, C, p, training != 0);
+            dy = make_float4(y.x > 0.f ? d * w.x * k.x * sc : 0.f, y.y > 0.f ? d * w.y * k.y * sc : 0.f,
+                             y.z > 0.f ? d * w.z * k.z * sc : 0.f, y.w > 0.f ? d * w.w * k.w * sc : 0.f);
+        }
         st4(dh2 + (size_t)m * C + c, make_float4(rs.x * (dy.x - s1.x - y.x * s2.x), rs.y * (dy.y - s1.y - y.y * s2.y),
                                                   rs.z * (dy.z - s1.z - y.z * s2.z), rs.w * (dy.w - s1.w - y.w * s2.w)));
     }
 }
 
-template <bool APPLY, bool EDGE>
-__global__ __launch_bounds__(SB) void k_l1_bwd_stats(float* __restrict__ da1, const float* __restrict__ a1,
+template <bool APPLY, bool EDGE, bool BITS = false>
+__global__ __launch_bounds__(SB, (EDGE && BITS) ? 5 : 6) void k_l1_bwd_stats(float* __restrict__ da1, const float* __restrict__ a1,
                                                      const int32_t* __restrict__ seg_ptr, const int32_t* __restrict__ order,
                                                      float sc, int C, float* __restrict__ S1, float* __restrict__ S2,
                                                      PreAct<EDGE> pre = PreAct<EDGE>{}, const float* __restrict__ mean = nullptr,
-                                                     const float* __restrict__ rstd = nullptr) {
-    __shared__ float4 sm[SB_SLOTS][SB_LANES];
+                                                     const float* __restrict__ rstd = nullptr, const uint8_t* __restrict__ act = nullptr) {
+    static_assert(APPLY || !BITS, "the bit-gated statistics recompute yhat1 from the pre-activation: APPLY only");
+    __shared__ float4 sm[2][SB_SLOTS][SB_LANES];
     __shared__ float4 bc1[SB_LANES], bc2[SB_LANES];
     const int g = blockIdx.x;
     const int lane = threadIdx.x % SB_LANES, slot = threadIdx.x / SB_LANES;
     const int c = (blockIdx.y * SB_LANES + lane) * 4;
+    const int C4 = C >> 2, q = c >> 2;
     const bool on = c < C;
     int beg, end; float inv_n;
     seg_slice(seg_ptr, g, &beg, &end, &inv_n);
@@ -400,6 +538,7 @@
     const float inv_sc = 1.f / sc;
     float4 s1 = f4zero(), s2 = f4zero();
     float4 dcache[SB_RC], acache[SB_RC], hcache[SB_RC];
+    unsigned gcache[SB_RC];
     int mc[SB_RC];
 #pragma unroll
     for (int i = 0; i < SB_RC; ++i) {
@@ -409,70 +548,87 @@
 #pragma unroll
     for (int i = 0; i < SB_RC; ++i) {
         dcache[i] = mc[i] >= 0 ? ld4(da1 + (size_t)mc[i] * C + c) : f4zero();
-        acache[i] = mc[i] >= 0 ? ld4(a1 + (size_t)mc[i] * C + c) : f4zero();
+        if (BITS) gcache[i] = mc[i] >= 0 ? (unsigned)act[(size_t)mc[i] * C4 + q] : 0u;
+        else acache[i] = mc[i] >= 0 ? ld4(a1 + (size_t)mc[i] * C + c) : f4zero();
         if (APPLY) hcache[i] = mc[i] >= 0 ? pre.load(mc[i], c) : f4zero();
     }
+    float4 mu = f4zero(), rs = f4zero();
+    if (APPLY && on) { mu = ld4(mean + (size_t)g * C + c); rs = ld4(rstd + (size_t)g * C + c); }
     const int rest = beg + slot + SB_RC * SB_SLOTS;
-#define GSAT_L1_DY(D4, A4)                                                                                                         \
-    const float4 dy = make_float4((A4).x > 0.f ? (D4).x * sc : 0.f, (A4).y > 0.f ? (D4).y * sc : 0.f,                                \
-                                  (A4).z > 0.f ? (D4).z * sc : 0.f, (A4).w > 0.f ? (D4).w * sc : 0.f);
-#define GSAT_L1_ACC(D4, A4)                                                                                                        \
+#define GSAT_L1_Y(H4) make_float4(((H4).x - mu.x) * rs.x, ((H4).y - mu.y) * rs.y, ((H4).z - mu.z) * rs.z, ((H4).w - mu.w) * rs.w)
+#define GSAT_L1_DY(D4, G)                                                                                                          \
+    const float4 dy = make_float4(((G) & 1u) ? (D4).x * sc : 0.f, ((G) & 2u) ? (D4).y * sc : 0.f,                                    \
+                                  ((G) & 4u) ? (D4).z * sc : 0.f, ((G) & 8u) ? (D4).w * sc : 0.f);
+#define GSAT_L1_ACC(D4, G, Y4)                                                                                                     \
     {                                                                                                                              \
-        GSAT_L1_DY(D4, A4)                                                                                                         \
+        GSAT_L1_DY(D4, G)                                                                                                          \
+        const float4 yv = (Y4);                                                                                                    \
         s1.x += dy.x; s1.y += dy.y; s1.z += dy.z; s1.w += dy.w;                                                                    \
-        s2.x = fmaf(dy.x, (A4).x * inv_sc, s2.x); s2.y = fmaf(dy.y, (A4).y * inv_sc, s2.y);                                          \
-        s2.z = fmaf(dy.z, (A4).z * inv_sc, s2.z); s2.w = fmaf(dy.w, (A4).w * inv_sc, s2.w);                                          \
-    }
+        s2.x = fmaf(dy.x, yv.x, s2.x); s2.y = fmaf(dy.y, yv.y, s2.y);                                                                \
+        s2.z = fmaf(dy.z, yv.z, s2.z); s2.w = fmaf(dy.w, yv.w, s2.w);                                                                \
+    }
+#define GSAT_L1_ASC(A4) make_float4((A4).x * inv_sc, (A4).y * inv_sc, (A4).z * inv_sc, (A4).w * inv_sc)
     if (on) {
 #pragma unroll
         for (int i = 0; i < SB_RC; ++i)
-            if (mc[i] >= 0) GSAT_L1_ACC(dcache[i], acache[i])
+            if (mc[i] >= 0) {
+                if (BITS) GSAT_L1_ACC(dcache[i], gcache[i], GSAT_L1_Y(hcache[i]))
+                else { gcache[i] = act_nibble(acache[i]); GSAT_L1_ACC(dcache[i], gcache[i], GSAT_L1_ASC(acache[i])) }
+            }
         for (int r = rest; r < end; r += SB_SLOTS) {
             const int m = order ? order[r] : r;
-            const float4 d = ld4(da1 + (size_t)m * C + c), a = ld4(a1 + (size_t)m * C + c);
-            GSAT_L1_ACC(d, a)
-        }
-    }
+            const float4 d = ld4(da1 + (size_t)m * C + c);
+            if (BITS) {
+                const unsigned gb = act[(size_t)m * C4 + q];
+                const float4 h = pre.load(m, c);
+                GSAT_L1_ACC(d, gb, GSAT_L1_Y(h))
+            } else {
+                const float4 a = ld4(a1 + (size_t)m * C + c);
+                const unsigned gb = act_nibble(a);
+                GSAT_L1_ACC(d, gb, GSAT_L1_ASC(a))
+            }
+        }
+    }
+#undef GSAT_L1_ASC
 #undef GSAT_L1_ACC
-    float4 t1 = slot_reduce(s1, sm, slot, lane);
-    float4 t2 = slot_reduce(s2, sm, slot, lane);
-    t1 = make_float4(t1.x * inv_n, t1.y * inv_n, t1.z * inv_n, t1.w * inv_n);
-    t2 = make_float4(t2.x * inv_n, t2.y * inv_n, t2.z * inv_n, t2.w * inv_n);
-    if (slot == 0 && on) {
-        st4(S1 + orow * C + c, t1);
-        st4(S2 + orow * C + c, t2);
-    }
+    const float4 acc2[2] = {s1, s2};
+    float4 t = slot_reduce_n<2>(acc2, sm, slot, lane);
+    t = make_float4(t.x * inv_n, t.y * inv_n, t.z * inv_n, t.w * inv_n);
+    if (slot < 2 && on) st4((slot == 0 ? S1 : S2) + orow * C + c, t);
     if (APPLY) {
-        if (slot == 0) { bc1[lane] = t1; bc2[lane] = t2; }
+        if (slot == 0) bc1[lane] = t;
+        if (slot == 1) bc2[lane] = t;
         __syncthreads();
         if (!on) return;
         const float4 q1 = bc1[lane], q2 = bc2[lane];
-        const float4 mu = ld4(mean + (size_t)g * C + c), rs = ld4(rstd + (size_t)g * C + c);
-#define GSAT_L1_OUT(M_, H4, D4, A4)                                                                                                \
+#define GSAT_L1_OUT(M_, H4, D4, G)                                                                                                 \
         {                                                                                                                          \
-            const float4 y = make_float4(((H4).x - mu.x) * rs.x, ((H4).y - mu.y) * rs.y, ((H4).z - mu.z) * rs.z, ((H4).w - mu.w) * rs.w); \
-            GSAT_L1_DY(D4, A4)                                                                                                     \
+            const float4 y = GSAT_L1_Y(H4);                                                                                        \
+            GSAT_L1_DY(D4, G)                                                                                                      \
             st4(da1 + (size_t)(M_) * C + c, make_float4(rs.x * (dy.x - q1.x - y.x * q2.x), rs.y * (dy.y - q1.y - y.y * q2.y),        \
                                                          rs.z * (dy.z - q1.z - y.z * q2.z), rs.w * (dy.w - q1.w - y.w * q2.w)));     \
         }
 #pragma unroll
         for (int i = 0; i < SB_RC; ++i)
-            if (mc[i] >= 0) GSAT_L1_OUT(mc[i], hcache[i], dcache[i], acache[i])
+            if (mc[i] >= 0) GSAT_L1_OUT(mc[i], hcache[i], dcache[i], gcache[i])
         for (int r = rest; r < end; r += SB_SLOTS) {
             const int m = order ? order[r] : r;
             const float4 h = pre.load(m, c);
-            const float4 d = ld4(da1 + (size_t)m * C + c), a = ld4(a1 + (size_t)m * C + c);
-            GSAT_L1_OUT(m, h, d, a)
+            const float4 d = ld4(da1 + (size_t)m * C + c);
+            const unsigned gb = BITS ? (unsigned)act[(size_t)m * C4 + q] : act_nibble(ld4(a1 + (size_t)m * C + c));
+            GSAT_L1_OUT(m, h, d, gb)
         }
 #undef GSAT_L1_OUT
     }
 #undef GSAT_L1_DY
+#undef GSAT_L1_Y
 }
 
 template <bool EDGE>
 __global__ void k_dh1(PreAct<EDGE> pre, const int32_t* __restrict__ row_seg, const float* __restrict__ mean,
                       const float* __restrict__ rstd, const float* __restrict__ a1, float sc, const float* __restrict__ S1,
-                      const float* __restrict__ S2, int64_t M, float* __restrict__ da1_inout) {
+                      const float* __restrict__ S2, int64_t M, float* __restrict__ da1_inout,
+                      const uint8_t* __restrict__ act = nullptr ) {
     const int C = pre.C, C4 = C >> 2;
     for (int64_t i = (int64_t)blockIdx.x * blockDim.x + threadIdx.x; i < M * C4; i += (int64_t)gridDim.x * blockDim.x) {
         const int m = (int)(i / C4), c = (int)(i % C4) * 4;
@@ -480,8 +636,9 @@
         float4 h = pre.load(m, c);
         float4 mu = ld4(mean + (size_t)g * C + c), rs = ld4(rstd + (size_t)g * C + c);
         float4 y = make_float4((h.x - mu.x) * rs.x, (h.y - mu.y) * rs.y, (h.z - mu.z) * rs.z, (h.w - mu.w) * rs.w);
-        float4 d = ld4(da1_inout + (size_t)m * C + c), a = ld4(a1 + (size_t)m * C + c);
-        float4 dy = make_float4(a.x > 0.f ? d.x * sc : 0.f, a.y > 0.f ? d.y * sc : 0.f, a.z > 0.f ? d.z * sc : 0.f, a.w > 0.f ? d.w * sc : 0.f);
+        float4 d = ld4(da1_inout + (size_t)m * C + c);
+        const unsigned b = act ? (unsigned)act[i] : act_nibble(ld4(a1 + (size_t)m * C + c));
+        float4 dy = make_float4((b & 1u) ? d.x * sc : 0.f, (b & 2u) ? d.y * sc : 0.f, (b & 4u) ? d.z * sc : 0.f, (b & 8u) ? d.w * sc : 0.f);
         float4 s1 = ld4(S1 + (size_t)g * C + c), s2 = ld4(S2 + (size_t)g * C + c);
         st4(da1_inout + (size_t)m * C + c, make_float4(rs.x * (dy.x - s1.x - y.x * s2.x), rs.y * (dy.y - s1.y - y.y * s2.y),
                                                         rs.z * (dy.z - s1.z - y.z * s2.z), rs.w * (dy.w - s1.w - y.w * s2.w)));
@@ -562,7 +719,9 @@
 
 constexpr int FIN_T = 1024, FIN_SLOTS = FIN_T / SB_LANES;
 __global__ __launch_bounds__(FIN_T) void k_head_bwd_finish(const float* __restrict__ dw3p, const float* __restrict__ dz_part, int64_t G, int ndz, int C,
-                                                           float* __restrict__ dW3, float* __restrict__ db3) {
+                                                           float* __restrict__ dW3, float* __restrict__ db3,
+                                                           float* __restrict__ zero_a = nullptr, int na = 0, float* __restrict__ zero_b = nullptr,
+                                                           int nb = 0 ) {
     __shared__ float4 sm[FIN_SLOTS][SB_LANES];
     const int lane = threadIdx.x % SB_LANES, slot = threadIdx.x / SB_LANES;
     const int ctiles = (C + 4 * SB_LANES - 1) / (4 * SB_LANES);
@@ -582,6 +741,8 @@
         }
     } else {
         for (int i = threadIdx.x; i < ndz; i += FIN_T) acc.x += dz_part[i];
+        for (int i = threadIdx.x; i < na; i += FIN_T) zero_a[i] = 0.f;
+        for (int i = threadIdx.x; i < nb; i += FIN_T) zero_b[i] = 0.f;
     }
     sm[slot][lane] = acc;
     __syncthreads();
@@ -700,10 +861,14 @@
 }
 
 
-int gsat_attn_fwd(const gsat_attn_args* a, void* stream_) {
+int gsat_attn_fwd(const gsat_attn_args* a, void* stream) { return gsat_attn_fwd_bits(a, nullptr, nullptr, stream); }
+
+int gsat_attn_fwd_bits(const gsat_attn_args* args, uint8_t* act1, uint8_t* act2, void* stream_) {
     hipStream_t stream = (hipStream_t)stream_;
-    int rc = check_args(a, "gsat_attn_fwd");
+    int rc = check_args(args, "gsat_attn_fwd");
     if (rc) return rc;
+    const AttnArgsX ax{*args, act1, act2};
+    const AttnArgsX* const a = &ax;
     if (a->M == 0) return GSAT_OK;
     {
         FusedGeom fg;
@@ -734,18 +899,18 @@
     if (a->edge_mode) {
         PreAct<true> pre{a->P, a->Q, a->b1, a->src, a->dst, C1};
         if (Z == 1 && G > 0) {
-            k_seg_stats<true, true><<<sgrid, SB, 0, stream>>>(pre, a->seg_ptr, a->seg_order, mean1, rstd1, a->mask1, sref, 1, a->p_drop, a->training, a->a1);
+            k_seg_stats<true, true><<<sgrid, SB, 0, stream>>>(pre, a->seg_ptr, a->seg_order, mean1, rstd1, a->mask1, sref, 1, a->p_drop, a->training, a->a1, a->act1);
         } else {
             if ((rc = launch_seg_stats<true>(stream, pre, a->seg_ptr, a->seg_order, G, Z, mean1, rstd1, part))) return rc;
-            k_norm_apply<true, true><<<ew_blocks(M * (C1 / 4)), 256, 0, stream>>>(pre, a->row_seg, mean1, rstd1, a->mask1, sref, 1, a->p_drop, a->training, M, a->a1);
+            k_norm_apply<true, true><<<ew_blocks(M * (C1 / 4)), 256, 0, stream>>>(pre, a->row_seg, mean1, rstd1, a->mask1, sref, 1, a->p_drop, a->training, M, a->a1, a->act1);
         }
     } else {
         PreAct<false> pre{a->P, nullptr, a->b1, nullptr, nullptr, C1};
         if (Z == 1 && G > 0) {
-            k_seg_stats<false, true><<<sgrid, SB, 0, stream>>>(pre, a->seg_ptr, a->seg_order, mean1, rstd1, a->mask1, sref, 1, a->p_drop, a->training, a->a1);
+            k_seg_stats<false, true><<<sgrid, SB, 0, stream>>>(pre, a->seg_ptr, a->seg_order, mean1, rstd1, a->mask1, sref, 1, a->p_drop, a->training, a->a1, a->act1);
         } else {
             if ((rc = launch_seg_stats<false>(stream, pre, a->seg_ptr, a->seg_order, G, Z, mean1, rstd1, part))) return rc;
-            k_norm_apply<false, true><<<ew_blocks(M * (C1 / 4)), 256, 0, stream>>>(pre, a->row_seg, mean1, rstd1, a->mask1, sref, 1, a->p_drop, a->training, M, a->a1);
+            k_norm_apply<false, true><<<ew_blocks(M * (C1 / 4)), 256, 0, stream>>>(pre, a->row_seg, mean1, rstd1, a->mask1, sref, 1, a->p_drop, a->training, M, a->a1, a->act1);
         }
     }
     GSAT_LAUNCH_CHECK();
@@ -757,7 +922,7 @@
     const int q = C2 / 4;
     const int lpr = q <= 4 ? 4 : q <= 8 ? 8 : q <= 16 ? 16 : q <= 32 ? 32 : 64;
     const int nb = (int)std::min<int64_t>(ceil_div(M, 256 / lpr), 256 * 32);
-#define HEAD(L) k_head_fwd<L><<<nb, 256, 0, stream>>>(a->h2, a->b2, a->row_seg, mean2, rstd2, a->mask2, SeedRef{a->seed, a->seed_dev}, a->p_drop, a->training, a->W3, a->b3, a->u, a->noise_philox, M, C2, a->logits, a->att)
+#define HEAD(L) k_head_fwd<L><<<nb, 256, 0, stream>>>(a->h2, a->b2, a->row_seg, mean2, rstd2, a->mask2, SeedRef{a->seed, a->seed_dev}, a->p_drop, a->training, a->W3, a->b3, a->u, a->noise_philox, M, C2, a->logits, a->att, a->act2)
     switch (lpr) { case 4: HEAD(4); break; case 8: HEAD(8); break; case 16: HEAD(16); break; case 32: HEAD(32); break; default: HEAD(64); break; }
 #undef HEAD
     GSAT_LAUNCH_CHECK();
@@ -798,10 +963,14 @@
     return b + 1024;
 }
 
-int gsat_attn_bwd(const gsat_attn_args* a, const gsat_attn_grads* gr, void* stream_) {
+int gsat_attn_bwd(const gsat_attn_args* a, const gsat_attn_grads* gr, void* stream) { return gsat_attn_bwd_bits(a, gr, nullptr, nullptr, stream); }
+
+int gsat_attn_bwd_bits(const gsat_attn_args* args, const gsat_attn_grads* gr, const uint8_t* act1, const uint8_t* act2, void* stream_) {
     hipStream_t stream = (hipStream_t)stream_;
-    int rc = check_args(a, "gsat_attn_bwd");
+    int rc = check_args(args, "gsat_attn_bwd");
     if (rc) return rc;
+    const AttnArgsX ax{*args, const_cast<uint8_t*>(act1), const_cast<uint8_t*>(act2)};
+    const AttnArgsX* const a = &ax;
     GSAT_REQUIRE(gr && gr->demb && gr->dW1 && gr->db1 && gr->dW2 && gr->db2 && gr->dW3 && gr->db3, GSAT_ERR_ARG, "gsat_attn_bwd: null gradient output");
     const int64_t M = a->M, N = a->N, G = a->G;
     const int H = a->H, C1 = a->C1, C2 = a->C2;
@@ -868,16 +1037,31 @@
     const unsigned dzb = (unsigned)ceil_div(M, 256);
     float* dzpart = scratch;
     const bool part_ok = (size_t)dzb <= (size_t)256 * std::max(C1, C2);
+    const bool bits2 = a->act2 != nullptr;
+    const bool inline_dz = bits2 && merged;
+    const bool fin = merged && (inline_dz || part_ok);
+    if (!inline_dz) {
     k_dz<<<dzb, 256, 0, stream>>>(gr->dlogits, gr->datt, a->att, M, dz, gr->db1, (int)C1, gr->db2, (int)C2, (merged && part_ok) ? dzpart : nullptr);
     GSAT_LAUNCH_CHECK();
     if (!(merged && part_ok) && (rc = colsum(stream, dz, M, 1, gr->db3, scratch))) return rc;
-    if (Z == 1)
+    }
+    if (bits2) {
+        const DzSrc dsrc = inline_dz ? DzSrc{nullptr, gr->dlogits, gr->datt, a->att} : DzSrc{dz, nullptr, nullptr, nullptr};
+        if (Z == 1)
+            k_head_bwd_bits<true><<<g2, SB, 0, stream>>>(a->h2, a->b2, a->seg_ptr, a->seg_order, mean2, rstd2, a->act2, sc, a->W3, dsrc, C2, S1, S2, dw3p,
+                                                         inline_dz ? dz : nullptr, dh2);
+        else
+            k_head_bwd_bits<false><<<g2, SB, 0, stream>>>(a->h2, a->b2, a->seg_ptr, a->seg_order, mean2, rstd2, a->act2, sc, a->W3, dsrc, C2, zp1, zp2, zp3);
+    } else if (Z == 1)
         k_head_bwd_stats<true><<<g2, SB, 0, stream>>>(a->h2, a->b2, a->seg_ptr, a->seg_order, mean2, rstd2, a->mask2, SeedRef{a->seed, a->seed_dev}, a->p_drop,
                                                       a->training, a->W3, DzSrc{dz, nullptr, nullptr, nullptr}, C2, S1, S2, dw3p, dh2);
     else
         k_head_bwd_stats<false><<<g2, SB, 0, stream>>>(a->h2, a->b2, a->seg_ptr, a->seg_order, mean2, rstd2, a->mask2, SeedRef{a->seed, a->seed_dev}, a->p_drop,
                                                        a->training, a->W3, DzSrc{dz, nullptr, nullptr, nullptr}, C2, zp1, zp2, zp3);
-    if (merged && part_ok)
+    if (inline_dz)
+        k_head_bwd_finish<<<(unsigned)ceil_div(C2, 4 * SB_LANES) + 1, FIN_T, 0, stream>>>(dw3p, dz, G, (int)G, C2, gr->dW3, gr->db3, gr->db1, (int)C1,
+                                                                                          gr->db2, (int)C2);
+    else if (fin)
         k_head_bwd_finish<<<(unsigned)ceil_div(C2, 4 * SB_LANES) + 1, FIN_T, 0, stream>>>(dw3p, dzpart, G, (int)dzb, C2, gr->dW3, gr->db3);
     if (Z > 1) {
         const unsigned cb = (unsigned)ceil_div(G * C2, 256);
@@ -886,10 +1070,10 @@
         k_zcombine<<<cb, 256, 0, stream>>>(zp3, a->seg_ptr, (int)G, Z, C2, 0, dw3p);
     }
     GSAT_LAUNCH_CHECK();
-    if (!(merged && part_ok) && (rc = colsum(stream, dw3p, G, C2, gr->dW3, scratch))) return rc;
+    if (!fin && (rc = colsum(stream, dw3p, G, C2, gr->dW3, scratch))) return rc;
     if (Z > 1) {
         k_dh2<<<ew_blocks(M * (C2 / 4)), 256, 0, stream>>>(a->h2, a->b2, a->row_seg, mean2, rstd2, a->mask2, SeedRef{a->seed, a->seed_dev}, a->p_drop, a->training,
-                                                           a->W3, dz, S1, S2, M, C2, dh2);
+                                                           a->W3, dz, S1, S2, M, C2, dh2, a->act2);
         GSAT_LAUNCH_CHECK();
     }
     if (dual_gemm_ok(1, M, C2, C1, C1)) {
@@ -901,10 +1085,12 @@
     if (Z == 1) {
         if (a->edge_mode) {
             PreAct<true> pre1{a->P, a->Q, a->b1, a->src, a->dst, C1};
-            k_l1_bwd_stats<true, true><<<g1, SB, 0, stream>>>(da1, a->a1, a->seg_ptr, a->seg_order, sc, C1, S1p, S2p, pre1, mean1, rstd1);
+            if (a->act1) k_l1_bwd_stats<true, true, true><<<g1, SB, 0, stream>>>(da1, a->a1, a->seg_ptr, a->seg_order, sc, C1, S1p, S2p, pre1, mean1, rstd1, a->act1);
+            else k_l1_bwd_stats<true, true><<<g1, SB, 0, stream>>>(da1, a->a1, a->seg_ptr, a->seg_order, sc, C1, S1p, S2p, pre1, mean1, rstd1);
         } else {
             PreAct<false> pre1{a->P, nullptr, a->b1, nullptr, nullptr, C1};
-            k_l1_bwd_stats<true, false><<<g1, SB, 0, stream>>>(da1, a->a1, a->seg_ptr, a->seg_order, sc, C1, S1p, S2p, pre1, mean1, rstd1);
+            if (a->act1) k_l1_bwd_stats<true, false, true><<<g1, SB, 0, stream>>>(da1, a->a1, a->seg_ptr, a->seg_order, sc, C1, S1p, S2p, pre1, mean1, rstd1, a->act1);
+            else k_l1_bwd_stats<true, false><<<g1, SB, 0, stream>>>(da1, a->a1, a->seg_ptr, a->seg_order, sc, C1, S1p, S2p, pre1, mean1, rstd1);
         }
     } else {
         k_l1_bwd_stats<false, false><<<g1, SB, 0, stream>>>(da1, a->a1, a->seg_ptr, a->seg_order, sc, C1, zp1, zp2);
@@ -919,7 +1105,7 @@
     if (a->edge_mode) {
         if (Z > 1) {
             PreAct<true> pre{a->P, a->Q, a->b1, a->src, a->dst, C1};
-            k_dh1<true><<<ew_blocks(M * (C1 / 4)), 256, 0, stream>>>(pre, a->row_seg, mean1, rstd1, a->a1, sc, S1p, S2p, M, da1);
+            k_dh1<true><<<ew_blocks(M * (C1 / 4)), 256, 0, stream>>>(pre, a->row_seg, mean1, rstd1, a->a1, sc, S1p, S2p, M, da1, a->act1);
             GSAT_LAUNCH_CHECK();
         }
         if ((rc = aggr_sum_fwd_impl(stream, da1, nullptr, nullptr, nullptr, gr->rowptr_src, gr->eid_by_src, nullptr, N, M, C1, 0.f, dP,
@@ -938,7 +1124,7 @@
     } else {
         if (Z > 1) {
             PreAct<false> pre{a->P, nullptr, a->b1, nullptr, nullptr, C1};
-            k_dh1<false><<<ew_blocks(M * (C1 / 4)), 256, 0, stream>>>(pre, a->row_seg, mean1, rstd1, a->a1, sc, S1p, S2p, M, da1);
+            k_dh1<false><<<ew_blocks(M * (C1 / 4)), 256, 0, stream>>>(pre, a->row_seg, mean1, rstd1, a->a1, sc, S1p, S2p, M, da1, a->act1);
             GSAT_LAUNCH_CHECK();
         }
         if (dual_gemm_ok(2, N, C1, H, H)) {
diff --git a/dp_gsat_amd/csrc/attn_fused.h b/dp_gsat_amd/csrc/attn_fused.h
--- a/dp_gsat_amd/csrc/attn_fused.h
+++ b/dp_gsat_amd/csrc/attn_fused.h
@@ -25,8 +25,12 @@
 
 bool fused_geometry(int H, int C1, int C2, bool edge, FusedGeom* out, bool pqg = false);
 size_t fused_ws_bytes(const FusedGeom& g, int64_t G);
+struct AttnArgsX : gsat_attn_args {
+    uint8_t* act1;
+    uint8_t* act2;
+};
 bool attn_fused_eligible(const gsat_attn_args* a, FusedGeom* g);
-int attn_fused_fwd(hipStream_t stream, const gsat_attn_args* a, const FusedGeom& g);
+int attn_fused_fwd(hipStream_t stream, const AttnArgsX* a, const FusedGeom& g);
 
 bool attn_fused_bwd_eligible(const gsat_attn_args* a);
 size_t attn_fused_bwd_ws_bytes(const gsat_attn_args* a);
@@ -43,6 +47,14 @@
     if (mask) return ld4(mask + (size_t)row * C + c);
     return philox_keep4(sref.get(), layer, row, c, p);
 }
+
+__device__ __forceinline__ unsigned act_nibble(float4 a) {
+    return (a.x > 0.f ? 1u : 0u) | (a.y > 0.f ? 2u : 0u) | (a.z > 0.f ? 4u : 0u) | (a.w > 0.f ? 8u : 0u);
+}
+__device__ __forceinline__ unsigned act_nibble(float4 y, float4 k) {
+    return ((y.x > 0.f && k.x != 0.f) ? 1u : 0u) | ((y.y > 0.f && k.y != 0.f) ? 2u : 0u) |
+           ((y.z > 0.f && k.z != 0.f) ? 4u : 0u) | ((y.w > 0.f && k.w != 0.f) ? 8u : 0u);
+}
 #endif
 
 }
diff --git a/dp_gsat_amd/csrc/attn_fused.hip b/dp_gsat_amd/csrc/attn_fused.hip
--- a/dp_gsat_amd/csrc/attn_fused.hip
+++ b/dp_gsat_amd/csrc/attn_fused.hip
@@ -373,6 +373,7 @@
     const int32_t *src, *dst, *seg_ptr, *order;
     const float *mask1, *mask2, *u;
     float *P, *Q, *a1, *h2, *stats, *logits, *att;
+    uint8_t *act1, *act2;
     const FTile* tiles;
     int* counters;
     int64_t M, N, G;
@@ -748,7 +749,9 @@
                             const float4 y = make_float4(fmaxf((x.x - mu[u].x) * rs[u].x, 0.f) * k.x * sc, fmaxf((x.y - mu[u].y) * rs[u].y, 0.f) * k.y * sc,
                                                          fmaxf((x.z - mu[u].z) * rs[u].z, 0.f) * k.z * sc, fmaxf((x.w - mu[u].w) * rs[u].w, 0.f) * k.w * sc);
                             st4(T + rr[u] * LDT + 4 * qq[u], y);
-                            if (A.a1) st4(A.a1 + (size_t)mm[u] * C1 + col, y);
+                            const size_t e = (size_t)mm[u] * C1 + col;
+                            if (A.a1) st4(A.a1 + e, y);
+                            if (A.act1) A.act1[e >> 2] = (uint8_t)act_nibble(y);
                         }
                     }
                 }
@@ -833,10 +836,12 @@
                         const float4 mu = ld4(sMean + gl * SW + 4 * q), rs = ld4(sMean + (F_GT + gl) * SW + 4 * q);
                         const float4 k = keep4f(A.mask2, A.seed, 2, m, 4 * q, C2, A.p, train);
                         const float4 w = ld4(sW3 + 4 * q);
-                        acc = fmaf(fmaxf((hv.x - mu.x) * rs.x, 0.f) * k.x * sc, w.x, acc);
-                        acc = fmaf(fmaxf((hv.y - mu.y) * rs.y, 0.f) * k.y * sc, w.y, acc);
-                        acc = fmaf(fmaxf((hv.z - mu.z) * rs.z, 0.f) * k.z * sc, w.z, acc);
-                        acc = fmaf(fmaxf((hv.w - mu.w) * rs.w, 0.f) * k.w * sc, w.w, acc);
+                        const float4 y = make_float4((hv.x - mu.x) * rs.x, (hv.y - mu.y) * rs.y, (hv.z - mu.z) * rs.z, (hv.w - mu.w) * rs.w);
+                        acc = fmaf(fmaxf(y.x, 0.f) * k.x * sc, w.x, acc);
+                        acc = fmaf(fmaxf(y.y, 0.f) * k.y * sc, w.y, acc);
+                        acc = fmaf(fmaxf(y.z, 0.f) * k.z * sc, w.z, acc);
+                        acc = fmaf(fmaxf(y.w, 0.f) * k.w * sc, w.w, acc);
+                        if (A.act2) A.act2[(size_t)m * C24 + q] = (uint8_t)act_nibble(y, k);
                     }
                 }
                 acc = group_sum<TPR>(acc);
@@ -875,10 +880,12 @@
                         const float4 mu = ld4(bMean + 4 * q), rs = ld4(bRstd + 4 * q);
                         const float4 k = keep4f(A.mask2, A.seed, 2, m, 4 * q, C2, A.p, train);
                         const float4 w = ld4(A.w3 + 4 * q);
-                        acc = fmaf(fmaxf((hv.x - mu.x) * rs.x, 0.f) * k.x * sc, w.x, acc);
-                        acc = fmaf(fmaxf((hv.y - mu.y) * rs.y, 0.f) * k.y * sc, w.y, acc);
-                        acc = fmaf(fmaxf((hv.z - mu.z) * rs.z, 0.f) * k.z * sc, w.z, acc);
-                        acc = fmaf(fmaxf((hv.w - mu.w) * rs.w, 0.f) * k.w * sc, w.w, acc);
+                        const float4 y = make_float4((hv.x - mu.x) * rs.x, (hv.y - mu.y) * rs.y, (hv.z - mu.z) * rs.z, (hv.w - mu.w) * rs.w);
+                        acc = fmaf(fmaxf(y.x, 0.f) * k.x * sc, w.x, acc);
+                        acc = fmaf(fmaxf(y.y, 0.f) * k.y * sc, w.y, acc);
+                        acc = fmaf(fmaxf(y.z, 0.f) * k.z * sc, w.z, acc);
+                        acc = fmaf(fmaxf(y.w, 0.f) * k.w * sc, w.w, acc);
+                        if (A.act2) A.act2[(size_t)m * C24 + q] = (uint8_t)act_nibble(y, k);
                     }
                 }
                 acc = group_sum<TPR>(acc);
@@ -949,7 +956,7 @@
     return true;
 }
 
-int attn_fused_fwd(hipStream_t stream, const gsat_attn_args* a, const FusedGeom& g) {
+int attn_fused_fwd(hipStream_t stream, const AttnArgsX* a, const FusedGeom& g) {
     const size_t need = fused_ws_bytes(g, a->G);
     GSAT_REQUIRE(a->fwd_workspace && a->fwd_workspace_bytes >= need, GSAT_ERR_WORKSPACE, "gsat_attn_fwd: workspace %zu < %zu (fused path)",
                  a->fwd_workspace_bytes, need);
@@ -969,6 +976,7 @@
     fa.src = a->src; fa.dst = a->dst; fa.seg_ptr = a->seg_ptr; fa.order = a->seg_order;
     fa.mask1 = a->mask1; fa.mask2 = a->mask2; fa.u = a->u;
     fa.P = a->P; fa.Q = a->Q; fa.a1 = a->a1; fa.h2 = a->h2; fa.stats = a->stats; fa.logits = a->logits; fa.att = a->att;
+    fa.act1 = a->act1; fa.act2 = a->act2;
     fa.tiles = tiles; fa.counters = counters;
     fa.M = a->M; fa.N = a->N; fa.G = a->G;
     fa.seed = SeedRef{a->seed, a->seed_dev};
diff --git a/dp_gsat_amd/ops.py b/dp_gsat_amd/ops.py
--- a/dp_gsat_amd/ops.py
+++ b/dp_gsat_amd/ops.py
@@ -363,6 +363,10 @@
     return a
 
 
+def attn_act_bits_enabled() -> bool:
+    return os.environ.get("GSAT_ATTN_ACT_BITS", "1") != "0"
+
+
 class ExtractorAttention(torch.autograd.Function):
 
     last_forward_kind = 0
@@ -398,6 +402,9 @@
         logits = torch.empty(M, 1, dtype=f32, device=dev)
         att = torch.empty(M, 1, dtype=f32, device=dev)
         bufs = (P, Q, a1, h2, stats, logits, att)
+        act_bits = None
+        if attn_act_bits_enabled():
+            act_bits = (torch.empty(M, C1 // 4, dtype=torch.uint8, device=dev), torch.empty(M, C2 // 4, dtype=torch.uint8, device=dev))
         args = _attn_args(emb, params, index, segments, edge_mode, training, p, seed, mask1, mask2, u, bufs, seed_dev, noise_philox)
         from ._lib import load
         fws_bytes = int(load().gsat_attn_fwd_workspace_bytes(ctypes.byref(args)))
@@ -405,11 +412,14 @@
         if fws_bytes:
             fws = torch.empty(fws_bytes, dtype=torch.uint8, device=dev)
             args.fwd_workspace, args.fwd_workspace_bytes = ptr(fws), fws_bytes
-        call("gsat_attn_fwd", ctypes.byref(args), stream())
+        if act_bits is not None:
+            call("gsat_attn_fwd_bits", ctypes.byref(args), ptr(act_bits[0]), ptr(act_bits[1]), stream())
+        else:
+            call("gsat_attn_fwd", ctypes.byref(args), stream())
         ctx.save_for_backward(emb, *params, P, Q if Q is not None else emb.new_empty(0), a1, h2, stats, att,
                               mask1 if mask1 is not None else emb.new_empty(0),
                               mask2 if mask2 is not None else emb.new_empty(0),
-                              u if u is not None else emb.new_empty(0))
+                              u if u is not None else emb.new_empty(0), *(act_bits or ()))
         ctx.meta = (index, segments, bool(edge_mode), bool(training), float(p), int(seed),
                     mask1 is not None, mask2 is not None, u is not None)
         ctx.seed_dev = seed_dev
@@ -419,7 +429,7 @@
     def backward(ctx, dlogits, datt):
         import ctypes
         from ._lib import AttnGrads, load
-        (emb, W1, b1, W2, b2, W3, b3, P, Q, a1, h2, stats, att, mask1, mask2, u) = ctx.saved_tensors
+        (emb, W1, b1, W2, b2, W3, b3, P, Q, a1, h2, stats, att, mask1, mask2, u, *act_bits) = ctx.saved_tensors
         index, segments, edge_mode, training, p, seed, has_m1, has_m2, has_u = ctx.meta
         params = (W1, b1, W2, b2, W3, b3)
         logits_dummy = att
@@ -441,7 +451,10 @@
         ws_bytes = int(load().gsat_attn_bwd_workspace_bytes(ctypes.byref(args)))
         ws = torch.empty(ws_bytes, dtype=torch.uint8, device=emb.device)
         g.workspace, g.workspace_bytes = ptr(ws), ws_bytes
-        call("gsat_attn_bwd", ctypes.byref(args), ctypes.byref(g), stream())
+        if act_bits:
+            call("gsat_attn_bwd_bits", ctypes.byref(args), ctypes.byref(g), ptr(act_bits[0]), ptr(act_bits[1]), stream())
+        else:
+            call("gsat_attn_bwd", ctypes.byref(args), ctypes.byref(g), stream())
         return (demb, *grads, None, None, None, None, None, None, None, None, None, None, None)
 
 
diff --git a/include/gsat_hip.h b/include/gsat_hip.h
--- a/include/gsat_hip.h
+++ b/include/gsat_hip.h
@@ -244,6 +244,8 @@
 size_t gsat_attn_bwd_workspace_bytes(const gsat_attn_args* args);
 int gsat_attn_fwd(const gsat_attn_args* args, void* stream);
 int gsat_attn_bwd(const gsat_attn_args* args, const gsat_attn_grads* grads, void* stream);
+int gsat_attn_fwd_bits(const gsat_attn_args* args, uint8_t* act1, uint8_t* act2, void* stream);
+int gsat_attn_bwd_bits(const gsat_attn_args* args, const gsat_attn_grads* grads, const uint8_t* act1, const uint8_t* act2, void* stream);
 
 int gsat_instance_norm_fwd(const float* x, const int32_t* seg_ptr, const int32_t* seg_order,
                            const int32_t* row_seg, int64_t M, int64_t G, int64_t C, float* y,
```

Result: no change. 126.2 (median of 6 runs) (+0.6%).
